# linto-ai/whisper-timestamped

Hardware: NVIDIA B200
Metric: audio-sec/s (RTF) large-v3 1h synthetic @1/2/4/8 B200; DTW GB/s vs HBM peak (higher is better)
Workload: dtype bf16x3 tensor-core GEMMs (float32-accurate), f32 elsewhere, f64 DTW accumulate

## Files before the change

include/wts.h:

```cpp
#ifndef WTS_H
#define WTS_H

#include <stdint.h>

#ifdef __cplusplus
extern "C" {
#endif

#define WTS_VERSION 102
#define WTS_SEG_NONPOSITIVE 1
#define WTS_SEG_PITCH16 2

typedef struct WtsSegDesc {
    int32_t window;
    int32_t row0;
    int32_t last_row;
    int32_t T;
    int32_t f0;
    int32_t F;
    int32_t max_dur;
    int32_t flags;
    int64_t cost_off;
    int64_t jumps_off;
    int64_t dir_off;
    int64_t bnd_off;
} WtsSegDesc;

int         wts_version(void);
const char* wts_last_error(void);

int64_t wts_dtw_dir_words(int32_t T, int32_t F);
int64_t wts_dtw_bnd_doubles(int32_t T, int32_t F);

int wts_attn_prep_batch(const float* d_qk, int32_t N, int32_t Tmax, int32_t Fmax,
                        const WtsSegDesc* d_segs, int32_t nseg, int32_t max_T, int32_t max_F,
                        float* d_cost, void* stream);

int wts_dtw_batch(const void* d_cost, int32_t cost_is_f64,
                  const WtsSegDesc* d_segs, int32_t nseg,
                  uint32_t* d_dir_ws, double* d_bnd_ws,
                  int32_t* d_jumps, int32_t* d_path, const int64_t* d_path_off,
                  int32_t* d_path_len, int32_t* d_status, void* stream);

int wts_dtw_batch_sized(const void* d_cost, int32_t cost_is_f64,
                  const WtsSegDesc* d_segs, int32_t nseg,
                  uint32_t* d_dir_ws, double* d_bnd_ws,
                  int32_t* d_jumps, int32_t* d_path, const int64_t* d_path_off,
                  int32_t* d_path_len, int32_t* d_status, int32_t max_T, int32_t max_F, int32_t all_flags,
                  void* stream);

int wts_disfluency_starts(const float* d_cost, const WtsSegDesc* d_segs, int32_t nseg, const int32_t* d_jumps,
                          int32_t* d_out, void* stream);



typedef struct WtsGemm {
    const void* a;  int64_t lda, a_plane, a_bo, a_bi;
    const void* b;  int64_t ldb, b_plane, b_bo, b_bi;
    int32_t M, N, K, batch_outer, batch_inner;
    float alpha;
    const float* bias;
    int32_t bias_on_m;
    int32_t act;
    const float* residual; int64_t ldr, r_bo, r_bi;
    float* out_f32;   int64_t ldc, c_bo, c_bi;
    void*  out_sb16;  int64_t ldo, o_plane, o_bo, o_bi;
    int32_t head_dim; int64_t head_stride;
    int32_t backend;
    int32_t a_is_f32, b_is_f32;
    const int32_t* row_mask;
} WtsGemm;

int wts_gemm(const WtsGemm* g, void* stream);

int wts_to_sb16(const float* d_x, int64_t n, void* d_hi, void* d_lo, void* stream);

int wts_layernorm(const float* d_x, int64_t ldx, const float* d_gamma, const float* d_beta, int32_t M,
                  int32_t D, void* d_out_sb16, int64_t ldo, int64_t o_plane, float* d_out_f32, int64_t ldf,
                  void* stream);

int wts_softmax_rows(const float* d_s, int64_t lds, int64_t rows, int32_t n, void* d_out_sb16, int64_t ldo,
                     int64_t o_plane, void* stream);

int wts_enc_attention(const void* d_qk, int64_t ld_qk, int64_t qk_plane, const void* d_vt, int64_t ld_vt,
                      int64_t vt_plane, int32_t B, int32_t H, int32_t D, int32_t n_ctx, void* d_out, int64_t ldo,
                      int64_t o_plane, void* stream);

int wts_frames(const float* d_audio, int64_t n_samples, int64_t n_total, int64_t n_frames, void* d_out,
               int64_t o_plane, void* stream);
int wts_power(const float* d_y, int64_t ldy, int64_t n_frames, void* d_out, int64_t ldo, int64_t o_plane,
              void* stream);
int wts_logmel_max(const float* d_m, int64_t n, float* d_max, void* stream);
int wts_logmel_finish(const float* d_m, int64_t n_frames, int32_t n_mels, const float* d_max, float* d_out_f32,
                      void* stream);

int wts_window_gather(const int64_t* d_mel_ptr, int32_t n_mels, const int32_t* d_seek, const int32_t* d_size,
                      int32_t B, void* d_out, int64_t o_plane, void* stream);

int wts_embed(const int32_t* d_tokens, const int32_t* d_positions, const float* d_emb, const float* d_pos,
              int32_t rows, int32_t D, float* d_out, void* stream);

int wts_gather_rows(const float* d_x, int64_t ldx, const int32_t* d_idx, int32_t rows, int32_t D, float* d_out,
                    void* stream);

int wts_decoder_attention(int32_t kind, const float* d_q, int64_t ldq, const float* d_k, const float* d_v,
                          int64_t seq_stride, int32_t ctx, const int32_t* d_row_seq, const int32_t* d_row_pos,
                          int32_t rows, int32_t H, void* d_out_sb16, int64_t ldo, int64_t o_plane,
                          float* d_qk_out, const int32_t* d_head_slot, int32_t n_slots, int32_t qk_rows,
                          const int32_t* d_qk_row, const int32_t* d_row_active, void* stream);

int wts_cross_kv_pack(const float* d_src, void* d_dst16, float* d_dst_align, const int32_t* d_head_slot,
                      int32_t n_slots, int32_t B, int32_t H, int32_t ctx, void* stream);
int wts_cross_attention_f16(const float* d_q, int64_t ldq, const void* d_k16, const void* d_v16,
                            const float* d_k_align, const int32_t* d_head_slot, int32_t n_slots, int32_t ctx,
                            const int32_t* d_row_seq, int32_t rows, int32_t H, void* d_out_sb16, int64_t ldo,
                            int64_t o_plane, float* d_qk_out, int32_t qk_rows, const int32_t* d_qk_row,
                            const int32_t* d_row_active, void* stream);

int wts_kv_append(const float* d_k, const float* d_v, int64_t ld, const int32_t* d_row_seq,
                  const int32_t* d_row_pos, int32_t rows, int32_t H, int32_t ctx, float* d_kc, float* d_vc,
                  int64_t seq_stride, void* stream);

typedef struct WtsDecodeCfg {
    int32_t n_vocab, eot, timestamp_begin, no_timestamps, max_initial_ts;
    int32_t sample_len, n_ctx, tokens_ld;
} WtsDecodeCfg;
int wts_decode_select(float* d_logits, int64_t ldl, const WtsDecodeCfg* cfg, const uint8_t* d_suppress,
                      const uint8_t* d_blank, int32_t* d_tokens, int32_t* d_n_tokens, const int32_t* d_n_prompt,
                      int32_t* d_done, float* d_logprobs, int32_t lp_ld, float* d_full_logprobs,
                      float* d_last_full, int32_t B, void* stream);

int wts_filtered_logprobs(const float* d_logits, int64_t ldl, const WtsDecodeCfg* cfg, const uint8_t* d_suppress,
                          const uint8_t* d_blank, int32_t* d_tokens, int32_t* d_n_tokens, const int32_t* d_n_prompt,
                          float* d_out, int32_t B, void* stream);

typedef struct WtsDecLayer {
    const float *ln1_g, *ln1_b, *w_qkv, *b_qkv, *w_o, *b_o;
    const float *ln2_g, *ln2_b, *w_cq, *b_cq, *w_co, *b_co;
    const float *ln3_g, *ln3_b, *w_fc1, *b_fc1, *w_fc2, *b_fc2;
    float *self_k, *self_v;
    const void *cross_k16, *cross_v16;
    const float* cross_k_align;
    const int32_t* head_slot;
    const void *sb_qkv, *sb_o, *sb_cq, *sb_co, *sb_fc1, *sb_fc2;
    int64_t pl_qkv, pl_o, pl_cq, pl_co, pl_fc1, pl_fc2;
} WtsDecLayer;

typedef struct WtsDecodeSteps {
    const WtsDecLayer* layers;
    const float *emb, *pos, *ln_g, *ln_b;
    int32_t *tokens, *n_tokens;
    const int32_t* n_prompt;
    int32_t* done;
    float *logprobs, *full, *last_full, *qk_buf;
    const uint8_t *suppress, *blank;
    float *x, *qkv, *att, *q, *mid, *logits;
    uint32_t* sync;
    uint64_t* prof;
    const void* emb_sb;
    int64_t emb_plane;
    int64_t use_mma;
    WtsDecodeCfg cfg;
    int32_t n_layer, D, H, n_ctx, n_audio_ctx, n_slots, cap, lp_ld, qk_rows, n_steps, max_rows, prof_cap;
} WtsDecodeSteps;

int wts_decode_steps(const WtsDecodeSteps* p, void* stream);

int wts_decode_step_kernels(const WtsDecodeSteps* p, const WtsDecLayer* h_layers, void* stream);

int wts_step_inputs(const int32_t* d_tokens, int32_t tokens_ld, const int32_t* d_n_tokens, const int32_t* d_n_prompt,
                    const int32_t* d_done, int32_t B, int32_t* d_tok, int32_t* d_pos, int32_t* d_qk_row,
                    int32_t* d_active, void* stream);

int wts_softmax_pick(const float* d_logits, int64_t ldl, int32_t n, int32_t index, float* d_out, int32_t rows,
                     void* stream);

int wts_logprob_gather(const float* d_logits, int64_t ldl, int32_t n, const int32_t* d_rows, const int32_t* d_tokens,
                       float* d_out, int32_t count, void* stream);

#ifdef __cplusplus
}
#endif
#endif
```

whisper-timestamped_b200/csrc/gemm.cu:

```cuda
#include <cuda_bf16.h>

#include "common.cuh"

namespace wts {

int gemm_tc_launch(const WtsGemm& g, cudaStream_t st);

__device__ __forceinline__ float ld_operand(const void* p, int64_t idx, int64_t plane, bool is_f32)
{
    if (is_f32) return reinterpret_cast<const float*>(p)[idx];
    const __nv_bfloat16* q = reinterpret_cast<const __nv_bfloat16*>(p);
    return __bfloat162float(q[idx]) + __bfloat162float(q[idx + plane]);
}

__device__ __forceinline__ float gelu_erf(float v) { return 0.5f * v * (1.0f + erff(v * 0.70710678118654752440f)); }

__device__ __forceinline__ void gemm_epilogue_store(const WtsGemm& g, int zo, int zi, int m, int n, float acc)
{
    float v = g.alpha * acc;
    if (g.bias) v += g.bias[g.bias_on_m ? m : n];
    if (g.act == 1) v = gelu_erf(v);
    if (g.residual) v += g.residual[(int64_t)zo * g.r_bo + (int64_t)zi * g.r_bi + (int64_t)m * g.ldr + n];
    if (g.out_f32) {
        const int64_t off = g.head_dim > 0 ? (int64_t)(n / g.head_dim) * g.head_stride + (int64_t)m * g.ldc + (n % g.head_dim)
                                           : (int64_t)m * g.ldc + n;
        g.out_f32[(int64_t)zo * g.c_bo + (int64_t)zi * g.c_bi + off] = v;
    }
    if (g.out_sb16) {
        const int64_t off = g.head_dim > 0 ? (int64_t)(n / g.head_dim) * g.head_stride + (int64_t)m * g.ldo + (n % g.head_dim)
                                           : (int64_t)m * g.ldo + n;
        __nv_bfloat16* o = reinterpret_cast<__nv_bfloat16*>(g.out_sb16) + (int64_t)zo * g.o_bo + (int64_t)zi * g.o_bi + off;
        const __nv_bfloat16 hi = __float2bfloat16_rn(v);
        o[0] = hi;
        o[g.o_plane] = __float2bfloat16_rn(v - __bfloat162float(hi));
    }
}

constexpr int ST = 64, SK = 16;
__global__ void __launch_bounds__(256)
gemm_simt_kernel(const WtsGemm g)
{
    __shared__ float As[SK][ST + 4];
    __shared__ float Bs[SK][ST + 4];
    const int z = blockIdx.z, zo = z / g.batch_inner, zi = z % g.batch_inner;
    const int m0 = blockIdx.y * ST, n0 = blockIdx.x * ST;
    const int tx = threadIdx.x & 15, ty = threadIdx.x >> 4;
    const int64_t abase = (int64_t)zo * g.a_bo + (int64_t)zi * g.a_bi;
    const int64_t bbase = (int64_t)zo * g.b_bo + (int64_t)zi * g.b_bi;
    float acc[4][4] = {};
    for (int k0 = 0; k0 < g.K; k0 += SK) {
#pragma unroll
        for (int i = 0; i < 4; ++i) {
            const int e = threadIdx.x + i * 256;
            const int r = e >> 4, kk = e & 15;
            const int m = m0 + r, n = n0 + r, k = k0 + kk;
            As[kk][r] = (m < g.M && k < g.K) ? ld_operand(g.a, abase + (int64_t)m * g.lda + k, g.a_plane, g.a_is_f32) : 0.f;
            Bs[kk][r] = (n < g.N && k < g.K) ? ld_operand(g.b, bbase + (int64_t)n * g.ldb + k, g.b_plane, g.b_is_f32) : 0.f;
        }
        __syncthreads();
#pragma unroll
        for (int kk = 0; kk < SK; ++kk) {
            float a[4], b[4];
#pragma unroll
            for (int i = 0; i < 4; ++i) { a[i] = As[kk][ty * 4 + i]; b[i] = Bs[kk][tx * 4 + i]; }
#pragma unroll
            for (int i = 0; i < 4; ++i)
#pragma unroll
                for (int j = 0; j < 4; ++j) acc[i][j] = fmaf(a[i], b[j], acc[i][j]);
        }
        __syncthreads();
    }
#pragma unroll
    for (int i = 0; i < 4; ++i)
#pragma unroll
        for (int j = 0; j < 4; ++j) {
            const int m = m0 + ty * 4 + i, n = n0 + tx * 4 + j;
            if (m < g.M && n < g.N) gemm_epilogue_store(g, zo, zi, m, n, acc[i][j]);
        }
}

}

using namespace wts;

extern "C" int wts_gemm(const WtsGemm* gp, void* stream)
{
    if (!gp) { set_error("wts_gemm: null descriptor"); return -2; }
    const WtsGemm g = *gp;
    if (g.M <= 0 || g.N <= 0 || g.batch_outer <= 0 || g.batch_inner <= 0) return 0;
    if (!g.a || !g.b || (!g.out_f32 && !g.out_sb16)) { set_error("wts_gemm: null operand/output"); return -2; }
    cudaStream_t st = (cudaStream_t)stream;
    if (g.backend == 0 && !g.a_is_f32 && !g.b_is_f32) return gemm_tc_launch(g, st);
    dim3 grid((g.N + ST - 1) / ST, (g.M + ST - 1) / ST, g.batch_outer * g.batch_inner);
    gemm_simt_kernel<<<grid, 256, 0, st>>>(g);
    WTS_LAUNCH_CHECK();
    return 0;
}
```

whisper-timestamped_b200/csrc/gemm_tc.cu:

```cuda
#include <cuda.h>
#include <cuda_bf16.h>
#include <cudaTypedefs.h>

#include <mutex>
#include <stdlib.h>

#include "common.cuh"

namespace wts {

constexpr int BM = 128, BK = 64;
constexpr int TILE_BYTES = BM * BK * 2;
constexpr int TC_THREADS = 192;
template <int BN> struct TcCfg {
    static constexpr int STAGES = 3;
    static constexpr int B_TILE = BN * BK * 2;
    static constexpr int STAGE_BYTES = 2 * TILE_BYTES + 2 * B_TILE;
    static constexpr int SMEM = STAGES * STAGE_BYTES + 256 + 1024;
    static constexpr int TMEM_COLS = BN < 32 ? 32 : BN;
};

__device__ __forceinline__ uint32_t smem_addr(const void* p) { return (uint32_t)__cvta_generic_to_shared(p); }

__device__ __forceinline__ void mbar_init(uint32_t bar, uint32_t count)
{
    asm volatile("mbarrier.init.shared::cta.b64 [%0], %1;" ::"r"(bar), "r"(count));
}
__device__ __forceinline__ void mbar_expect_tx(uint32_t bar, uint32_t bytes)
{
    asm volatile("mbarrier.arrive.expect_tx.shared::cta.b64 _, [%0], %1;" ::"r"(bar), "r"(bytes) : "memory");
}
__device__ __forceinline__ void mbar_wait(uint32_t bar, uint32_t parity)
{
    asm volatile(
        "{\n\t"
        ".reg .pred p;\n\t"
        "WAIT_LOOP:\n\t"
        "mbarrier.try_wait.parity.shared::cta.b64 p, [%0], %1;\n\t"
        "@p bra DONE;\n\t"
        "bra WAIT_LOOP;\n\t"
        "DONE:\n\t"
        "}\n" ::"r"(bar), "r"(parity) : "memory");
}
__device__ __forceinline__ void tma_load_5d(uint32_t dst, const CUtensorMap* tm, uint32_t bar, int c0, int c1, int c2,
                                            int c3, int c4)
{
    asm volatile(
        "cp.async.bulk.tensor.5d.shared::cluster.global.mbarrier::complete_tx::bytes [%0], [%1, {%3, %4, %5, %6, %7}], [%2];"
        ::"r"(dst), "l"(tm), "r"(bar), "r"(c0), "r"(c1), "r"(c2), "r"(c3), "r"(c4) : "memory");
}
__device__ __forceinline__ void umma_bf16(uint32_t tmem_c, uint64_t adesc, uint64_t bdesc, uint32_t idesc, uint32_t accumulate)
{
    asm volatile(
        "{\n\t"
        ".reg .pred p;\n\t"
        "setp.ne.b32 p, %4, 0;\n\t"
        "tcgen05.mma.cta_group::1.kind::f16 [%0], %1, %2, %3, p;\n\t"
        "}\n" ::"r"(tmem_c), "l"(adesc), "l"(bdesc), "r"(idesc), "r"(accumulate) : "memory");
}
__device__ __forceinline__ void umma_commit(uint32_t bar)
{
    asm volatile("tcgen05.commit.cta_group::1.mbarrier::arrive::one.shared::cluster.b64 [%0];" ::"r"(bar) : "memory");
}
__device__ __forceinline__ void tc_fence_before() { asm volatile("tcgen05.fence::before_thread_sync;" ::: "memory"); }
__device__ __forceinline__ void tc_fence_after() { asm volatile("tcgen05.fence::after_thread_sync;" ::: "memory"); }

__device__ __forceinline__ void tmem_ld32(uint32_t taddr, uint32_t (&v)[32])
{
    asm volatile(
        "tcgen05.ld.sync.aligned.32x32b.x32.b32 "
        "{%0, %1, %2, %3, %4, %5, %6, %7, %8, %9, %10, %11, %12, %13, %14, %15, "
        "%16, %17, %18, %19, %20, %21, %22, %23, %24, %25, %26, %27, %28, %29, %30, %31}, [%32];"
        : "=r"(v[0]), "=r"(v[1]), "=r"(v[2]), "=r"(v[3]), "=r"(v[4]), "=r"(v[5]), "=r"(v[6]), "=r"(v[7]), "=r"(v[8]),
          "=r"(v[9]), "=r"(v[10]), "=r"(v[11]), "=r"(v[12]), "=r"(v[13]), "=r"(v[14]), "=r"(v[15]), "=r"(v[16]),
          "=r"(v[17]), "=r"(v[18]), "=r"(v[19]), "=r"(v[20]), "=r"(v[21]), "=r"(v[22]), "=r"(v[23]), "=r"(v[24]),
          "=r"(v[25]), "=r"(v[26]), "=r"(v[27]), "=r"(v[28]), "=r"(v[29]), "=r"(v[30]), "=r"(v[31])
        : "r"(taddr) : "memory");
    asm volatile("tcgen05.wait::ld.sync.aligned;" ::: "memory");
}

__device__ __forceinline__ uint64_t umma_desc(uint32_t saddr)
{
    uint64_t d = 0;
    d |= (uint64_t)((saddr >> 4) & 0x3FFF);
    d |= (uint64_t)1 << 16;
    d |= (uint64_t)(1024 >> 4) << 32;
    d |= (uint64_t)1 << 46;
    d |= (uint64_t)2 << 61;
    return d;
}

__device__ __forceinline__ float gelu_erf_tc(float v) { return 0.5f * v * (1.0f + erff(v * 0.70710678118654752440f)); }

struct TcArgs {
    WtsGemm g;
    int a_has_bo, a_has_bi, b_has_bo, b_has_bi;
    int debug;
};

__device__ __forceinline__ void epilogue_chunk(const WtsGemm& g, float (&y)[32], int m, int nb, float bias_m, const float* res,
                                               float* of, __nv_bfloat16* ob)
{
#pragma unroll
    for (int j = 0; j < 32; ++j) {
        const int n = nb + j;
        float t = y[j];
        if (g.bias) t += g.bias_on_m ? bias_m : (n < g.N ? g.bias[n] : 0.f);
        if (g.act == 1) t = gelu_erf_tc(t);
        if (res && n < g.N) t += res[n];
        y[j] = t;
    }
    const bool full = nb + 32 <= g.N;
    if (of) {
        const int64_t off = g.head_dim > 0 ? (int64_t)(nb / g.head_dim) * g.head_stride + (int64_t)m * g.ldc + (nb % g.head_dim)
                                           : (int64_t)m * g.ldc + nb;
        float* dst = of + off;
        if (full && ((reinterpret_cast<uintptr_t>(dst) & 15) == 0)) {
#pragma unroll
            for (int j = 0; j < 32; j += 4) *reinterpret_cast<float4*>(dst + j) = make_float4(y[j], y[j + 1], y[j + 2], y[j + 3]);
        } else {
#pragma unroll
            for (int j = 0; j < 32; ++j) if (nb + j < g.N) dst[j] = y[j];
        }
    }
    if (ob) {
        const int64_t off = g.head_dim > 0 ? (int64_t)(nb / g.head_dim) * g.head_stride + (int64_t)m * g.ldo + (nb % g.head_dim)
                                           : (int64_t)m * g.ldo + nb;
        __nv_bfloat16* dh = ob + off;
        __nv_bfloat16* dl = dh + g.o_plane;
        __align__(16) __nv_bfloat16 hi[32];
        __align__(16) __nv_bfloat16 lo[32];
#pragma unroll
        for (int j = 0; j < 32; ++j) {
            hi[j] = __float2bfloat16_rn(y[j]);
            lo[j] = __float2bfloat16_rn(y[j] - __bfloat162float(hi[j]));
        }
        if (full && ((reinterpret_cast<uintptr_t>(dh) & 15) == 0) && ((reinterpret_cast<uintptr_t>(dl) & 15) == 0)) {
#pragma unroll
            for (int j = 0; j < 4; ++j) {
                reinterpret_cast<uint4*>(dh)[j] = reinterpret_cast<const uint4*>(hi)[j];
                reinterpret_cast<uint4*>(dl)[j] = reinterpret_cast<const uint4*>(lo)[j];
            }
        } else {
#pragma unroll
            for (int j = 0; j < 32; ++j) if (nb + j < g.N) { dh[j] = hi[j]; dl[j] = lo[j]; }
        }
    }
}

template <int BN>
__global__ void __launch_bounds__(TC_THREADS, 1)
gemm_tc_kernel(const __grid_constant__ CUtensorMap tmA, const __grid_constant__ CUtensorMap tmB, const TcArgs args)
{
    using Cfg = TcCfg<BN>;
    constexpr int STAGES = Cfg::STAGES, STAGE_BYTES = Cfg::STAGE_BYTES, B_TILE = Cfg::B_TILE, TMEM_COLS = Cfg::TMEM_COLS;
    extern __shared__ unsigned char smem_raw[];
    const WtsGemm& g = args.g;
    const uint32_t base = (smem_addr(smem_raw) + 1023u) & ~1023u;
    const uint32_t bar_base = base + STAGES * STAGE_BYTES;
    const int warp = threadIdx.x >> 5, lane = threadIdx.x & 31;
    const int m0 = blockIdx.y * BM, n0 = blockIdx.x * BN;
    const int z = blockIdx.z, zo = z / g.batch_inner, zi = z - zo * g.batch_inner;
    const int nkb = (g.K + BK - 1) / BK;
    constexpr int kb0 = 0;

    if (warp == 0 && lane == 0) {
        asm volatile("prefetch.tensormap [%0];" ::"l"(&tmA) : "memory");
        asm volatile("prefetch.tensormap [%0];" ::"l"(&tmB) : "memory");
    }
    if (warp == 1) {
        if (lane == 0) {
            for (int s = 0; s < STAGES; ++s) { mbar_init(bar_base + 8 * s, 1); mbar_init(bar_base + 64 + 8 * s, 1); }
            mbar_init(bar_base + 128, 1);
            asm volatile("fence.mbarrier_init.release.cluster;" ::: "memory");
        }
        __syncwarp();
        asm volatile("tcgen05.alloc.cta_group::1.sync.aligned.shared::cta.b32 [%0], %1;" ::"r"(bar_base + 136), "r"(TMEM_COLS) : "memory");
        asm volatile("tcgen05.relinquish_alloc_permit.cta_group::1.sync.aligned;" ::: "memory");
    }
    tc_fence_before();
    __syncthreads();
    tc_fence_after();
    uint32_t tmem_base;
    asm volatile("ld.shared.u32 %0, [%1];" : "=r"(tmem_base) : "r"(bar_base + 136));

    if (warp == 0) {
        if (lane == 0) {
            const int azo = args.a_has_bo ? zo : 0, azi = args.a_has_bi ? zi : 0;
            const int bzo = args.b_has_bo ? zo : 0, bzi = args.b_has_bi ? zi : 0;
            for (int kb = 0; kb < (args.debug == 2 ? 0 : nkb); ++kb) {
                const int s = kb % STAGES, u = kb / STAGES;
                mbar_wait(bar_base + 64 + 8 * s, (u & 1) ^ 1);
                const uint32_t full = bar_base + 8 * s;
                mbar_expect_tx(full, STAGE_BYTES);
                const uint32_t st = base + s * STAGE_BYTES;
                const int kc = (kb0 + kb) * BK;
                tma_load_5d(st, &tmA, full, kc, m0, azi, azo, 0);
                tma_load_5d(st + TILE_BYTES, &tmA, full, kc, m0, azi, azo, 1);
                tma_load_5d(st + 2 * TILE_BYTES, &tmB, full, kc, n0, bzi, bzo, 0);
                tma_load_5d(st + 2 * TILE_BYTES + B_TILE, &tmB, full, kc, n0, bzi, bzo, 1);
            }
        }
    } else if (warp == 1) {
        if (lane == 0) {
            const uint32_t idesc = (1u << 4) | (1u << 7) | (1u << 10) | ((uint32_t)(BN >> 3) << 17) | ((uint32_t)(BM >> 4) << 24);
            for (int kb = 0; kb < nkb; ++kb) {
                const int s = kb % STAGES, u = kb / STAGES;
                if (args.debug != 2) mbar_wait(bar_base + 8 * s, u & 1);
                tc_fence_after();
                if (args.debug == 1) {
                    asm volatile("mbarrier.arrive.shared::cta.b64 _, [%0];" ::"r"(bar_base + 64 + 8 * s) : "memory");
                    continue;
                }
                const uint32_t st = base + s * STAGE_BYTES;
                const uint64_t a_hi = umma_desc(st), a_lo = umma_desc(st + TILE_BYTES);
                const uint64_t b_hi = umma_desc(st + 2 * TILE_BYTES), b_lo = umma_desc(st + 2 * TILE_BYTES + B_TILE);
#pragma unroll
                for (int k = 0; k < BK / 16; ++k) {
                    const uint64_t adv = (uint64_t)(k * 2);
                    umma_bf16(tmem_base, a_hi + adv, b_hi + adv, idesc, (kb | k) ? 1u : 0u);
                    if (args.debug == 3) continue;
                    umma_bf16(tmem_base, a_lo + adv, b_hi + adv, idesc, 1u);
                    umma_bf16(tmem_base, a_hi + adv, b_lo + adv, idesc, 1u);
                }
                umma_commit(bar_base + 64 + 8 * s);
            }
            umma_commit(bar_base + 128);
        }
    } else {
        const int q = warp & 3;
        const int m = m0 + 32 * q + lane;
        mbar_wait(bar_base + 128, 0);
        tc_fence_after();
        const bool row_ok = m < g.M;
        const float* res = g.residual ? g.residual + (int64_t)zo * g.r_bo + (int64_t)zi * g.r_bi + (int64_t)m * g.ldr : nullptr;
        float* of = g.out_f32 ? g.out_f32 + (int64_t)zo * g.c_bo + (int64_t)zi * g.c_bi : nullptr;
        __nv_bfloat16* ob = g.out_sb16 ? reinterpret_cast<__nv_bfloat16*>(g.out_sb16) + (int64_t)zo * g.o_bo + (int64_t)zi * g.o_bi : nullptr;
        const float bias_m = (g.bias && g.bias_on_m && row_ok) ? g.bias[m] : 0.f;
#pragma unroll 1
        for (int c = 0; c < BN / 32; ++c) {
            uint32_t v[32];
            tmem_ld32(tmem_base + ((uint32_t)(32 * q) << 16) + (uint32_t)(32 * c), v);
            const int nb = n0 + 32 * c;
            if (!row_ok || nb >= g.N) continue;
            float y[32];
#pragma unroll
            for (int j = 0; j < 32; ++j) y[j] = g.alpha * __uint_as_float(v[j]);
            epilogue_chunk(g, y, m, nb, bias_m, res, of, ob);
        }
    }
    tc_fence_before();
    __syncthreads();
    if (warp == 1) {
        tc_fence_after();
        asm volatile("tcgen05.dealloc.cta_group::1.sync.aligned.b32 %0, %1;" ::"r"(tmem_base), "r"(TMEM_COLS) : "memory");
    }
}

constexpr int P_THREADS = 320;
constexpr int P_STAGES = 3;
constexpr int P_STAGE_BYTES = 4 * TILE_BYTES;
constexpr int P_SMEM = P_STAGES * P_STAGE_BYTES + 256 + 1024;

__global__ void __launch_bounds__(P_THREADS, 1)
gemm_tc_persist_kernel(const __grid_constant__ CUtensorMap tmA, const __grid_constant__ CUtensorMap tmB, const TcArgs args)
{
    extern __shared__ unsigned char smem_raw[];
    const WtsGemm& g = args.g;
    const uint32_t base = (smem_addr(smem_raw) + 1023u) & ~1023u;
    const uint32_t bar_base = base + P_STAGES * P_STAGE_BYTES;
    const int warp = threadIdx.x >> 5, lane = threadIdx.x & 31;
    const int tiles_n = (g.N + BM - 1) / BM, tiles_m = (g.M + BM - 1) / BM;
    const int n_tiles = tiles_n * tiles_m * g.batch_outer * g.batch_inner;
    const int nkb = (g.K + BK - 1) / BK;

    if (warp == 0 && lane == 0) {
        asm volatile("prefetch.tensormap [%0];" ::"l"(&tmA) : "memory");
        asm volatile("prefetch.tensormap [%0];" ::"l"(&tmB) : "memory");
    }
    if (warp == 1) {
        if (lane == 0) {
            for (int s = 0; s < P_STAGES; ++s) { mbar_init(bar_base + 8 * s, 1); mbar_init(bar_base + 32 + 8 * s, 1); }
            for (int b = 0; b < 2; ++b) { mbar_init(bar_base + 64 + 8 * b, 1); mbar_init(bar_base + 80 + 8 * b, 256); }
            asm volatile("fence.mbarrier_init.release.cluster;" ::: "memory");
        }
        __syncwarp();
        asm volatile("tcgen05.alloc.cta_group::1.sync.aligned.shared::cta.b32 [%0], %1;" ::"r"(bar_base + 96), "r"(256) : "memory");
        asm volatile("tcgen05.relinquish_alloc_permit.cta_group::1.sync.aligned;" ::: "memory");
    }
    tc_fence_before();
    __syncthreads();
    tc_fence_after();
    uint32_t tmem_base;
    asm volatile("ld.shared.u32 %0, [%1];" : "=r"(tmem_base) : "r"(bar_base + 96));

    if (warp == 0) {
        if (lane == 0) {
            int it = 0;
            for (int t = blockIdx.x; t < n_tiles; t += gridDim.x) {
                const int nt = t % tiles_n, mt = (t / tiles_n) % tiles_m, z = t / (tiles_n * tiles_m);
                const int zo = z / g.batch_inner, zi = z - zo * g.batch_inner;
                const int azo = args.a_has_bo ? zo : 0, azi = args.a_has_bi ? zi : 0;
                const int bzo = args.b_has_bo ? zo : 0, bzi = args.b_has_bi ? zi : 0;
                const int m0 = mt * BM, n0 = nt * BM;
                for (int kb = 0; kb < nkb; ++kb, ++it) {
                    const int s = it % P_STAGES, u = it / P_STAGES;
                    mbar_wait(bar_base + 32 + 8 * s, (u & 1) ^ 1);
                    const uint32_t full = bar_base + 8 * s;
                    mbar_expect_tx(full, P_STAGE_BYTES);
                    const uint32_t st = base + s * P_STAGE_BYTES;
                    const int kc = kb * BK;
                    tma_load_5d(st, &tmA, full, kc, m0, azi, azo, 0);
                    tma_load_5d(st + TILE_BYTES, &tmA, full, kc, m0, azi, azo, 1);
                    tma_load_5d(st + 2 * TILE_BYTES, &tmB, full, kc, n0, bzi, bzo, 0);
                    tma_load_5d(st + 3 * TILE_BYTES, &tmB, full, kc, n0, bzi, bzo, 1);
                }
            }
        }
    } else if (warp == 1) {
        if (lane == 0) {
            const uint32_t idesc = (1u << 4) | (1u << 7) | (1u << 10) | ((uint32_t)(BM >> 3) << 17) | ((uint32_t)(BM >> 4) << 24);
            int it = 0, lt = 0;
            for (int t = blockIdx.x; t < n_tiles; t += gridDim.x, ++lt) {
                const int buf = lt & 1, ut = lt >> 1;
                mbar_wait(bar_base + 80 + 8 * buf, (ut & 1) ^ 1);
                tc_fence_after();
                const uint32_t acc = tmem_base + (uint32_t)(buf * BM);
                for (int kb = 0; kb < nkb; ++kb, ++it) {
                    const int s = it % P_STAGES, u = it / P_STAGES;
                    mbar_wait(bar_base + 8 * s, u & 1);
                    tc_fence_after();
                    const uint32_t st = base + s * P_STAGE_BYTES;
                    const uint64_t a_hi = umma_desc(st), a_lo = umma_desc(st + TILE_BYTES);
                    const uint64_t b_hi = umma_desc(st + 2 * TILE_BYTES), b_lo = umma_desc(st + 3 * TILE_BYTES);
#pragma unroll
                    for (int k = 0; k < BK / 16; ++k) {
                        const uint64_t adv = (uint64_t)(k * 2);
                        umma_bf16(acc, a_hi + adv, b_hi + adv, idesc, (kb | k) ? 1u : 0u);
                        umma_bf16(acc, a_lo + adv, b_hi + adv, idesc, 1u);
                        umma_bf16(acc, a_hi + adv, b_lo + adv, idesc, 1u);
                    }
                    umma_commit(bar_base + 32 + 8 * s);
                }
                umma_commit(bar_base + 64 + 8 * buf);
            }
        }
    } else {
        const int q = warp & 3, half = (warp - 2) >> 2;
        int lt = 0;
        for (int t = blockIdx.x; t < n_tiles; t += gridDim.x, ++lt) {
            const int nt = t % tiles_n, mt = (t / tiles_n) % tiles_m, z = t / (tiles_n * tiles_m);
            const int zo = z / g.batch_inner, zi = z - zo * g.batch_inner;
            const int m0 = mt * BM, n0 = nt * BM;
            const int buf = lt & 1, ut = lt >> 1;
            const int m = m0 + 32 * q + lane;
            const bool row_ok = m < g.M;
            const float* res = g.residual ? g.residual + (int64_t)zo * g.r_bo + (int64_t)zi * g.r_bi + (int64_t)m * g.ldr : nullptr;
            float* of = g.out_f32 ? g.out_f32 + (int64_t)zo * g.c_bo + (int64_t)zi * g.c_bi : nullptr;
            __nv_bfloat16* ob = g.out_sb16 ? reinterpret_cast<__nv_bfloat16*>(g.out_sb16) + (int64_t)zo * g.o_bo + (int64_t)zi * g.o_bi : nullptr;
            const float bias_m = (g.bias && g.bias_on_m && row_ok) ? g.bias[m] : 0.f;
            mbar_wait(bar_base + 64 + 8 * buf, ut & 1);
            tc_fence_after();
            uint32_t v0[32], v1[32];
            const uint32_t taddr = tmem_base + ((uint32_t)(32 * q) << 16) + (uint32_t)(buf * BM + 64 * half);
            tmem_ld32(taddr, v0);
            tmem_ld32(taddr + 32, v1);
            tc_fence_before();
            asm volatile("mbarrier.arrive.shared::cta.b64 _, [%0];" ::"r"(bar_base + 80 + 8 * buf) : "memory");
            if (!row_ok) continue;
            float y[32];
            int nb = n0 + 64 * half;
            if (nb < g.N) {
#pragma unroll
                for (int j = 0; j < 32; ++j) y[j] = g.alpha * __uint_as_float(v0[j]);
                epilogue_chunk(g, y, m, nb, bias_m, res, of, ob);
            }
            nb += 32;
            if (nb < g.N) {
#pragma unroll
                for (int j = 0; j < 32; ++j) y[j] = g.alpha * __uint_as_float(v1[j]);
                epilogue_chunk(g, y, m, nb, bias_m, res, of, ob);
            }
        }
    }
    tc_fence_before();
    __syncthreads();
    if (warp == 1) {
        tc_fence_after();
        asm volatile("tcgen05.dealloc.cta_group::1.sync.aligned.b32 %0, %1;" ::"r"(tmem_base), "r"(256) : "memory");
    }
}

struct SkArgs {
    WtsGemm g;
    int split_k;
    int bn;
    int stages, stage_bytes;
    int debug;
};

constexpr int SK_SMEM = 3 * 65536 + 256 + 1024 + 1024;

__device__ __forceinline__ void sk_finish(const WtsGemm& g, float t, float resid, int m, int n, float bias_n, float* of,
                                          __nv_bfloat16* ob)
{
    if (g.bias) t += g.bias_on_m ? g.bias[m] : bias_n;
    if (g.act == 1) t = gelu_erf_tc(t);
    t += resid;
    if (of) of[(int64_t)m * g.ldc + n] = t;
    if (ob) {
        const __nv_bfloat16 hi = __float2bfloat16_rn(t);
        ob[(int64_t)m * g.ldo + n] = hi;
        ob[(int64_t)m * g.ldo + n + g.o_plane] = __float2bfloat16_rn(t - __bfloat162float(hi));
    }
}

__device__ __forceinline__ void cluster_sync_all()
{
    asm volatile("barrier.cluster.arrive.release.aligned;" ::: "memory");
    asm volatile("barrier.cluster.wait.acquire.aligned;" ::: "memory");
}

template <int SMAX, int RB>
__device__ __forceinline__ void sk_reduce_rows(const WtsGemm& g, const uint32_t (&peer)[8], int S, const int* list, int rank,
                                               int n_rows, int n, float bias_n, float* of, __nv_bfloat16* ob)
{
#pragma unroll 1
    for (int kb = rank; kb < n_rows; kb += RB * S) {
        float x[RB][SMAX], r[RB];
        int mm[RB];
#pragma unroll
        for (int i = 0; i < RB; ++i) {
            const int k = kb + i * S;
            const bool ok = k < n_rows;
            const int m = ok ? list[k] : 0;
            mm[i] = ok ? m : -1;
            r[i] = (ok && g.residual) ? g.residual[(int64_t)m * g.ldr + n] : 0.f;
#pragma unroll
            for (int s = 0; s < SMAX; ++s) {
                x[i][s] = 0.f;
                if (s < S && ok)
                    asm volatile("ld.shared::cluster.f32 %0, [%1];" : "=f"(x[i][s]) : "r"(peer[s] + (uint32_t)(m * BM * 4)));
            }
        }
#pragma unroll
        for (int i = 0; i < RB; ++i) {
            if (mm[i] >= 0) {
                float t = 0.f;
#pragma unroll
                for (int s = 0; s < SMAX; ++s) t += x[i][s];
                sk_finish(g, t, r[i], mm[i], n, bias_n, of, ob);
            }
        }
    }
}

__global__ void __launch_bounds__(TC_THREADS, 1)
gemm_skinny_kernel(const __grid_constant__ CUtensorMap tmW, const __grid_constant__ CUtensorMap tmX, const SkArgs args)
{
    extern __shared__ unsigned char smem_raw[];
    const WtsGemm& g = args.g;
    const uint32_t base = (smem_addr(smem_raw) + 1023u) & ~1023u;
    const uint32_t bar_base = base + 3 * 65536;
    const int warp = threadIdx.x >> 5, lane = threadIdx.x & 31;
    const int n0 = blockIdx.x * BM;
    const int S = args.split_k;
    const int nkb_all = (g.K + BK - 1) / BK;
    const int kb0 = (int)((int64_t)blockIdx.y * nkb_all / S);
    const int kb1 = (int)((int64_t)(blockIdx.y + 1) * nkb_all / S);
    const int nkb = args.debug == 4 ? 0 : kb1 - kb0;
    const int STAGES = args.stages, STAGE_BYTES = args.stage_bytes;
    const int X_TILE = args.bn * BK * 2;
    pdl_launch();
    if (args.debug == 5) { pdl_wait(); return; }

    if (warp == 0 && lane == 0) {
        asm volatile("prefetch.tensormap [%0];" ::"l"(&tmW) : "memory");
        asm volatile("prefetch.tensormap [%0];" ::"l"(&tmX) : "memory");
    }
    if (warp == 1) {
        if (lane == 0) {
            for (int s = 0; s < STAGES; ++s) { mbar_init(bar_base + 8 * s, 1); mbar_init(bar_base + 64 + 8 * s, 1); }
            mbar_init(bar_base + 128, 1);
            asm volatile("fence.mbarrier_init.release.cluster;" ::: "memory");
        }
        __syncwarp();
        asm volatile("tcgen05.alloc.cta_group::1.sync.aligned.shared::cta.b32 [%0], %1;" ::"r"(bar_base + 136), "r"(128) : "memory");
        asm volatile("tcgen05.relinquish_alloc_permit.cta_group::1.sync.aligned;" ::: "memory");
    }
    tc_fence_before();
    __syncthreads();
    tc_fence_after();
    uint32_t tmem_base;
    asm volatile("ld.shared.u32 %0, [%1];" : "=r"(tmem_base) : "r"(bar_base + 136));
    pdl_wait();

    int* rows_list = reinterpret_cast<int*>(smem_raw + (bar_base - smem_addr(smem_raw)) + 256);
    if (warp >= 2) {
        const int t = threadIdx.x - 64;
        const bool act = t < g.M && (g.row_mask == nullptr || g.row_mask[t] != 0);
        const unsigned bal = __ballot_sync(0xffffffffu, act);
        int* wcount = rows_list + 132;
        if (lane == 0) wcount[warp - 2] = __popc(bal);
        asm volatile("bar.sync 1, 128;" ::: "memory");
        int off = 0;
        for (int w2 = 0; w2 < warp - 2; ++w2) off += wcount[w2];
        if (act) rows_list[off + __popc(bal & ((1u << lane) - 1u))] = t;
        if (t == 0) rows_list[128] = wcount[0] + wcount[1] + wcount[2] + wcount[3];
        asm volatile("bar.sync 1, 128;" ::: "memory");
    }

    const int q = warp & 3;
    const int nl = 32 * q + lane;
    const int n = n0 + nl;
    const bool n_ok = n < g.N;
    float* of = g.out_f32;
    __nv_bfloat16* ob = reinterpret_cast<__nv_bfloat16*>(g.out_sb16);

    if (warp == 0) {
        if (lane == 0) {
            for (int kb = 0; kb < (args.debug == 2 ? 0 : nkb); ++kb) {
                const int s = kb % STAGES, u = kb / STAGES;
                mbar_wait(bar_base + 64 + 8 * s, (u & 1) ^ 1);
                const uint32_t full = bar_base + 8 * s;
                mbar_expect_tx(full, STAGE_BYTES);
                const uint32_t st = base + s * STAGE_BYTES;
                const int kc = (kb0 + kb) * BK;
                tma_load_5d(st, &tmW, full, kc, n0, 0, 0, 0);
                tma_load_5d(st + TILE_BYTES, &tmW, full, kc, n0, 0, 0, 1);
                tma_load_5d(st + 2 * TILE_BYTES, &tmX, full, kc, 0, 0, 0, 0);
                tma_load_5d(st + 2 * TILE_BYTES + X_TILE, &tmX, full, kc, 0, 0, 0, 1);
            }
        }
    } else if (warp == 1) {
        if (lane == 0) {
            const uint32_t idesc = (1u << 4) | (1u << 7) | (1u << 10) | ((uint32_t)(args.bn >> 3) << 17) | ((uint32_t)(BM >> 4) << 24);
            for (int kb = 0; kb < nkb; ++kb) {
                const int s = kb % STAGES, u = kb / STAGES;
                if (args.debug != 2) mbar_wait(bar_base + 8 * s, u & 1);
                tc_fence_after();
                if (args.debug == 1) {
                    asm volatile("mbarrier.arrive.shared::cta.b64 _, [%0];" ::"r"(bar_base + 64 + 8 * s) : "memory");
                    continue;
                }
                const uint32_t st = base + s * STAGE_BYTES;
                const uint64_t w_hi = umma_desc(st), w_lo = umma_desc(st + TILE_BYTES);
                const uint64_t x_hi = umma_desc(st + 2 * TILE_BYTES), x_lo = umma_desc(st + 2 * TILE_BYTES + X_TILE);
#pragma unroll
                for (int k = 0; k < BK / 16; ++k) {
                    const uint64_t adv = (uint64_t)(k * 2);
                    umma_bf16(tmem_base, w_hi + adv, x_hi + adv, idesc, (kb | k) ? 1u : 0u);
                    umma_bf16(tmem_base, w_lo + adv, x_hi + adv, idesc, 1u);
                    umma_bf16(tmem_base, w_hi + adv, x_lo + adv, idesc, 1u);
                }
                umma_commit(bar_base + 64 + 8 * s);
            }
            umma_commit(bar_base + 128);
        }
    } else {
        const int nchunk = (g.M + 31) / 32;
        const float bias_n = (g.bias && !g.bias_on_m && n_ok) ? g.bias[n] : 0.f;
        mbar_wait(bar_base + 128, 0);
        tc_fence_after();
        float* part = reinterpret_cast<float*>(smem_raw + (base - smem_addr(smem_raw)));
#pragma unroll 1
        for (int c = 0; c < nchunk; ++c) {
            uint32_t v[32];
            tmem_ld32(tmem_base + ((uint32_t)(32 * q) << 16) + (uint32_t)(32 * c), v);
            if (S == 1) {
                if (!n_ok) continue;
                float r[32];
#pragma unroll
                for (int j = 0; j < 32; ++j) {
                    const int m = 32 * c + j;
                    r[j] = (g.residual && m < g.M) ? g.residual[(int64_t)m * g.ldr + n] : 0.f;
                }
#pragma unroll
                for (int j = 0; j < 32; ++j) {
                    const int m = 32 * c + j;
                    if (m < g.M && (g.row_mask == nullptr || g.row_mask[m] != 0))
                        sk_finish(g, g.alpha * __uint_as_float(v[j]), r[j], m, n, bias_n, of, ob);
                }
            } else {
#pragma unroll
                for (int j = 0; j < 32; ++j) {
                    const int m = 32 * c + j;
                    if (m < g.M) part[m * BM + nl] = g.alpha * __uint_as_float(v[j]);
                }
            }
        }
    }
    if (S > 1) {
        __syncwarp();
        cluster_sync_all();
        if (warp >= 2 && n_ok) {
            uint32_t rank;
            asm volatile("mov.u32 %0, %%cluster_ctarank;" : "=r"(rank));
            const int n_rows = rows_list[128];
            const float bias_n = (g.bias && !g.bias_on_m) ? g.bias[n] : 0.f;
            uint32_t peer[8];
#pragma unroll
            for (int s = 0; s < 8; ++s) {
                peer[s] = 0;
                if (s < S) asm volatile("mapa.shared::cluster.u32 %0, %1, %2;" : "=r"(peer[s]) : "r"(base + 4u * nl), "r"(s));
            }
            if (S <= 4) sk_reduce_rows<4, 12>(g, peer, S, rows_list, (int)rank, n_rows, n, bias_n, of, ob);
            else        sk_reduce_rows<8, 6>(g, peer, S, rows_list, (int)rank, n_rows, n, bias_n, of, ob);
        }
        __syncwarp();
        cluster_sync_all();
    }
    tc_fence_before();
    __syncthreads();
    if (warp == 1) {
        tc_fence_after();
        asm volatile("tcgen05.dealloc.cta_group::1.sync.aligned.b32 %0, %1;" ::"r"(tmem_base), "r"(128) : "memory");
    }
}

static PFN_cuTensorMapEncodeTiled_v12000 get_encode()
{
    static PFN_cuTensorMapEncodeTiled_v12000 fn = nullptr;
    static std::once_flag once;
    std::call_once(once, [] {
        void* p = nullptr;
        cudaDriverEntryPointQueryResult qres;
        if (cudaGetDriverEntryPoint("cuTensorMapEncodeTiled", &p, cudaEnableDefault, &qres) == cudaSuccess &&
            qres == cudaDriverEntryPointSuccess)
            fn = reinterpret_cast<PFN_cuTensorMapEncodeTiled_v12000>(p);
    });
    return fn;
}

static int make_map(CUtensorMap* tm, const void* ptr, int64_t K, int64_t rows, int64_t ld, int64_t plane, int64_t n_bi,
                    int64_t s_bi, int64_t n_bo, int64_t s_bo, int box_rows, const char* which)
{
    auto enc = get_encode();
    if (!enc) { set_error("wts_gemm: cuTensorMapEncodeTiled entry point not available"); return -4; }
    if ((reinterpret_cast<uintptr_t>(ptr) & 15) || (ld & 7) || (plane & 7) || (s_bi & 7) || (s_bo & 7)) {
        set_error("wts_gemm(tc): operand %s not 16-byte aligned (ptr=%p ld=%lld plane=%lld bi=%lld bo=%lld)", which, ptr,
                  (long long)ld, (long long)plane, (long long)s_bi, (long long)s_bo);
        return -5;
    }
    const int64_t e_bi = s_bi ? n_bi : 1, e_bo = s_bo ? n_bo : 1;
    cuuint64_t dims[5] = {(cuuint64_t)K, (cuuint64_t)rows, (cuuint64_t)e_bi, (cuuint64_t)e_bo, 2};
    const cuuint64_t row_b = (cuuint64_t)ld * 2;
    cuuint64_t strides[4] = {row_b, (cuuint64_t)(s_bi ? s_bi * 2 : row_b), (cuuint64_t)(s_bo ? s_bo * 2 : row_b),
                             (cuuint64_t)plane * 2};
    cuuint32_t box[5] = {BK, (cuuint32_t)box_rows, 1, 1, 1};
    cuuint32_t estr[5] = {1, 1, 1, 1, 1};
    CUresult r = enc(tm, CU_TENSOR_MAP_DATA_TYPE_BFLOAT16, 5, const_cast<void*>(ptr), dims, strides, box, estr,
                     CU_TENSOR_MAP_INTERLEAVE_NONE, CU_TENSOR_MAP_SWIZZLE_128B, CU_TENSOR_MAP_L2_PROMOTION_L2_256B,
                     CU_TENSOR_MAP_FLOAT_OOB_FILL_NONE);
    if (r != CUDA_SUCCESS) {
        set_error("wts_gemm(tc): cuTensorMapEncodeTiled(%s) failed with %d (K=%lld rows=%lld ld=%lld plane=%lld)", which, (int)r,
                  (long long)K, (long long)rows, (long long)ld, (long long)plane);
        return -6;
    }
    return 0;
}

static int launch_big(const WtsGemm& g, cudaStream_t st)
{
    constexpr int BN = 128;
    static bool attr_set = false;
    if (!attr_set) {
        WTS_CUDA_CHECK(cudaFuncSetAttribute(gemm_tc_kernel<BN>, cudaFuncAttributeMaxDynamicSharedMemorySize, TcCfg<BN>::SMEM));
        attr_set = true;
    }
    alignas(64) CUtensorMap tmA, tmB;
    int rc = make_map(&tmA, g.a, g.K, g.M, g.lda, g.a_plane, g.batch_inner, g.a_bi, g.batch_outer, g.a_bo, BM, "A");
    if (rc) return rc;
    rc = make_map(&tmB, g.b, g.K, g.N, g.ldb, g.b_plane, g.batch_inner, g.b_bi, g.batch_outer, g.b_bo, BN, "B");
    if (rc) return rc;
    TcArgs args;
    args.g = g;
    args.a_has_bo = g.a_bo != 0; args.a_has_bi = g.a_bi != 0;
    args.b_has_bo = g.b_bo != 0; args.b_has_bi = g.b_bi != 0;
    { const char* e = getenv("WTS_GEMM_DEBUG"); args.debug = e ? atoi(e) : 0; }
    static const int persist = []{ const char* e = getenv("WTS_GEMM_PERSIST"); return e ? atoi(e) : 1; }();
    const int64_t n_tiles = (int64_t)((g.N + BN - 1) / BN) * ((g.M + BM - 1) / BM) * g.batch_outer * g.batch_inner;
    if (persist && args.debug == 0 && n_tiles > 1) {
        static bool pattr = false;
        static int n_sm = 148;
        if (!pattr) {
            WTS_CUDA_CHECK(cudaFuncSetAttribute(gemm_tc_persist_kernel, cudaFuncAttributeMaxDynamicSharedMemorySize, P_SMEM));
            int dev = 0;
            WTS_CUDA_CHECK(cudaGetDevice(&dev));
            WTS_CUDA_CHECK(cudaDeviceGetAttribute(&n_sm, cudaDevAttrMultiProcessorCount, dev));
            pattr = true;
        }
        const int64_t rounds = (n_tiles + n_sm - 1) / n_sm;
        const int ctas = (int)((n_tiles + rounds - 1) / rounds);
        gemm_tc_persist_kernel<<<ctas, P_THREADS, P_SMEM, st>>>(tmA, tmB, args);
        WTS_LAUNCH_CHECK();
        return 0;
    }
    dim3 grid((g.N + BN - 1) / BN, (g.M + BM - 1) / BM, g.batch_outer * g.batch_inner);
    gemm_tc_kernel<BN><<<grid, TC_THREADS, TcCfg<BN>::SMEM, st>>>(tmA, tmB, args);
    WTS_LAUNCH_CHECK();
    return 0;
}

static int launch_skinny(const WtsGemm& g, cudaStream_t st, int split_k)
{
    static bool attr_set = false;
    if (!attr_set) {
        WTS_CUDA_CHECK(cudaFuncSetAttribute(gemm_skinny_kernel, cudaFuncAttributeMaxDynamicSharedMemorySize, SK_SMEM));
        attr_set = true;
    }
    SkArgs args;
    args.g = g;
    args.bn = ((g.M + 15) / 16) * 16;
    args.stage_bytes = 2 * TILE_BYTES + 2 * args.bn * BK * 2;
    args.stages = (3 * 65536) / args.stage_bytes;
    if (args.stages > 8) args.stages = 8;
    args.split_k = split_k;
    { const char* e = getenv("WTS_GEMM_DEBUG"); args.debug = e ? atoi(e) : 0; }
    alignas(64) CUtensorMap tmW, tmX;
    int rc = make_map(&tmW, g.b, g.K, g.N, g.ldb, g.b_plane, 1, 0, 1, 0, BM, "B(weights)");
    if (rc) return rc;
    rc = make_map(&tmX, g.a, g.K, g.M, g.lda, g.a_plane, 1, 0, 1, 0, args.bn, "A(rows)");
    if (rc) return rc;
    cudaLaunchConfig_t cfg = {};
    cfg.gridDim = dim3((g.N + BM - 1) / BM, split_k, 1);
    cfg.blockDim = dim3(TC_THREADS, 1, 1);
    cfg.dynamicSmemBytes = SK_SMEM;
    cfg.stream = st;
    cudaLaunchAttribute attr[2];
    attr[0].id = cudaLaunchAttributeClusterDimension;
    attr[0].val.clusterDim.x = 1;
    attr[0].val.clusterDim.y = split_k;
    attr[0].val.clusterDim.z = 1;
    attr[1].id = cudaLaunchAttributeProgrammaticStreamSerialization;
    attr[1].val.programmaticStreamSerializationAllowed = 1;
    cfg.attrs = attr;
    cfg.numAttrs = pdl_enabled() ? 2 : 1;
    WTS_CUDA_CHECK(cudaLaunchKernelEx(&cfg, gemm_skinny_kernel, tmW, tmX, args));
    return 0;
}

int gemm_tc_launch(const WtsGemm& g, cudaStream_t st)
{
    static const int skinny = []{ const char* e = getenv("WTS_SKINNY_GEMM"); return e ? atoi(e) : 1; }();
    static const int splitk = []{ const char* e = getenv("WTS_SPLITK"); return e ? atoi(e) : 1; }();
    if (skinny && g.M <= BM && g.batch_outer * g.batch_inner == 1 && g.head_dim == 0) {
        const int tiles = (g.N + BM - 1) / BM, nkb = (g.K + BK - 1) / BK;
        int split = 1;
        if (splitk && tiles <= 74) {
            split = 148 / tiles;
            if (split > 8) split = 8;
            if (split > nkb) split = nkb;
            if (split < 1) split = 1;
        }
        return launch_skinny(g, st, split);
    }
    return launch_big(g, st);
}

}
```

whisper-timestamped_b200/csrc/ops.cu:

```cuda
#include "decode_common.cuh"

namespace wts {

__global__ void to_sb16_kernel(const float* __restrict__ x, int64_t n, __nv_bfloat16* __restrict__ hi,
                               __nv_bfloat16* __restrict__ lo)
{
    for (int64_t i = blockIdx.x * (int64_t)blockDim.x + threadIdx.x; i < n; i += (int64_t)gridDim.x * blockDim.x) {
        __nv_bfloat16 h, l;
        split_bf16(x[i], h, l);
        hi[i] = h;
        lo[i] = l;
    }
}

constexpr int LN_THREADS = 128, LN_MAXV = 16;
__global__ void __launch_bounds__(LN_THREADS)
layernorm_kernel(const float* x, int64_t ldx, const float* gamma,
                 const float* beta, int M, int D, __nv_bfloat16* o, int64_t ldo,
                 int64_t o_plane, float* of, int64_t ldf)
{
    pdl_launch();
    pdl_wait();
    __shared__ float red[32];
    const int row = blockIdx.x;
    const float* xr = x + (int64_t)row * ldx;
    float v[LN_MAXV];
    float s = 0.f;
#pragma unroll
    for (int k = 0; k < LN_MAXV; ++k) {
        const int c = threadIdx.x + LN_THREADS * k;
        v[k] = c < D ? xr[c] : 0.f;
        s += v[k];
    }
    const float mean = block_reduce_sum(s, red) / (float)D;
    float q = 0.f;
#pragma unroll
    for (int k = 0; k < LN_MAXV; ++k) {
        const int c = threadIdx.x + LN_THREADS * k;
        const float d = c < D ? v[k] - mean : 0.f;
        q += d * d;
    }
    const float rstd = 1.0f / sqrtf(block_reduce_sum(q, red) / (float)D + 1e-5f);
#pragma unroll
    for (int k = 0; k < LN_MAXV; ++k) {
        const int c = threadIdx.x + LN_THREADS * k;
        if (c < D) {
            const float y = (v[k] - mean) * rstd * gamma[c] + beta[c];
            if (o) {
                __nv_bfloat16 h, l;
                split_bf16(y, h, l);
                o[(int64_t)row * ldo + c] = h;
                o[(int64_t)row * ldo + c + o_plane] = l;
            }
            if (of) of[(int64_t)row * ldf + c] = y;
        }
    }
}

__global__ void __launch_bounds__(128)
softmax_rows_kernel(const float* __restrict__ s, int64_t lds, int64_t rows, int n,
                    __nv_bfloat16* __restrict__ o, int64_t ldo, int64_t o_plane)
{
    const int64_t row = (int64_t)blockIdx.x * 4 + (threadIdx.x >> 5);
    const int lane = threadIdx.x & 31;
    if (row >= rows) return;
    const float* sr = s + row * lds;
    float v[64];
    float mx = -CUDART_INF_F;
#pragma unroll
    for (int k = 0; k < 64; ++k) {
        const int c = lane + 32 * k;
        v[k] = c < n ? sr[c] : -CUDART_INF_F;
        mx = fmaxf(mx, v[k]);
    }
    mx = warp_max(mx);
    float sum = 0.f;
#pragma unroll
    for (int k = 0; k < 64; ++k) {
        v[k] = expf(v[k] - mx);
        sum += v[k];
    }
    sum = warp_sum(sum);
    const float inv = 1.0f / sum;
#pragma unroll
    for (int k = 0; k < 64; ++k) {
        const int c = lane + 32 * k;
        if (c < n) {
            __nv_bfloat16 h, l;
            split_bf16(v[k] * inv, h, l);
            o[row * ldo + c] = h;
            o[row * ldo + c + o_plane] = l;
        }
    }
}

__global__ void frames_kernel(const float* __restrict__ audio, int64_t n_samples, int64_t n_total,
                              int64_t n_frames, float* __restrict__ out)
{
    const int64_t t = blockIdx.x;
    if (t >= n_frames) return;
    for (int n = threadIdx.x; n < 400; n += blockDim.x) {
        int64_t i = t * 160 - 200 + n;
        if (i < 0) i = -i;
        if (i >= n_total) i = 2 * (n_total - 1) - i;
        const float x = (i >= 0 && i < n_samples) ? audio[i] : 0.f;
        const float w = 0.5f - 0.5f * cospif((float)n / 200.0f);
        out[t * 400 + n] = x * w;
    }
}

__global__ void power_kernel(const float* __restrict__ y, int64_t ldy, int64_t n_frames, float* __restrict__ p,
                             int64_t ldp)
{
    const int64_t i = blockIdx.x * (int64_t)blockDim.x + threadIdx.x;
    if (i >= n_frames * 208) return;
    const int64_t t = i / 208;
    const int k = (int)(i - t * 208);
    const float re = y[t * ldy + k], im = y[t * ldy + 208 + k];
    p[t * ldp + k] = re * re + im * im;
}

__device__ __forceinline__ float mel_log10(float m) { return log10f(fmaxf(m, 1e-10f)); }

__global__ void logmel_max_kernel(const float* __restrict__ m, int64_t n, float* __restrict__ out)
{
    __shared__ float red[32];
    float mx = -CUDART_INF_F;
    for (int64_t i = blockIdx.x * (int64_t)blockDim.x + threadIdx.x; i < n; i += (int64_t)gridDim.x * blockDim.x)
        mx = fmaxf(mx, mel_log10(m[i]));
    mx = block_reduce_max(mx, red);
    if (threadIdx.x == 0) {
        int key = __float_as_int(mx);
        key = key >= 0 ? key : key ^ 0x7fffffff;
        atomicMax(reinterpret_cast<int*>(out), key);
    }
}

__global__ void logmel_finish_kernel(const float* __restrict__ m, int64_t n, const float* __restrict__ mxkey,
                                     float* __restrict__ out)
{
    int key = *reinterpret_cast<const int*>(mxkey);
    key = key >= 0 ? key : key ^ 0x7fffffff;
    const float gmax = __int_as_float(key);
    for (int64_t i = blockIdx.x * (int64_t)blockDim.x + threadIdx.x; i < n; i += (int64_t)gridDim.x * blockDim.x) {
        float x = mel_log10(m[i]);
        x = fmaxf(x, gmax - 8.0f);
        out[i] = (x + 4.0f) / 4.0f;
    }
}

__global__ void window_gather_kernel(const int64_t* __restrict__ mel_ptr, int n_mels,
                                     const int32_t* __restrict__ seek, const int32_t* __restrict__ size, int B,
                                     __nv_bfloat16* __restrict__ out, int64_t o_plane)
{
    const int b = blockIdx.y;
    const float* mel = reinterpret_cast<const float*>(mel_ptr[b]);
    const int64_t i = blockIdx.x * (int64_t)blockDim.x + threadIdx.x;
    const int64_t per = (int64_t)3002 * n_mels;
    if (i >= per) return;
    const int r = (int)(i / n_mels), c = (int)(i - (int64_t)r * n_mels);
    float v = 0.f;
    const int t = r - 1;
    if (t >= 0 && t < size[b]) v = mel[((int64_t)seek[b] + t) * n_mels + c];
    __nv_bfloat16 h, l;
    split_bf16(v, h, l);
    out[b * per + i] = h;
    out[b * per + i + o_plane] = l;
}

__global__ void embed_kernel(const int32_t* tokens, const int32_t* positions,
                             const float* emb, const float* pos, int rows, int D,
                             float* out)
{
    pdl_launch();
    pdl_wait();
    const int r = blockIdx.x;
    if (r >= rows) return;
    const float* e = emb + (int64_t)tokens[r] * D;
    const float* p = pos + (int64_t)positions[r] * D;
    for (int c = threadIdx.x; c < D; c += blockDim.x) out[(int64_t)r * D + c] = e[c] + p[c];
}

__global__ void gather_rows_kernel(const float* __restrict__ x, int64_t ldx, const int32_t* __restrict__ idx,
                                   int rows, int D, float* __restrict__ out)
{
    const int r = blockIdx.x;
    if (r >= rows) return;
    const float* s = x + (int64_t)idx[r] * ldx;
    for (int c = threadIdx.x; c < D; c += blockDim.x) out[(int64_t)r * D + c] = s[c];
}

constexpr int DA_THREADS = 128;
__global__ void __launch_bounds__(DA_THREADS)
decoder_attention_kernel(const int kind, const float* q, int64_t ldq, const float* kc,
                         const float* vc, int64_t seq_stride, int ctx,
                         const int32_t* row_seq, const int32_t* row_pos, int H,
                         __nv_bfloat16* o, int64_t ldo, int64_t o_plane, float* qk_out,
                         const int32_t* head_slot, int n_slots, int qk_rows,
                         const int32_t* qk_row, const int32_t* row_active)
{
    pdl_launch();
    pdl_wait();
    extern __shared__ float sm[];
    float* sc = sm;
    float* qs = sm + ctx;
    float* red = qs + 64;
    float* part = red + 32;
    const int r = blockIdx.x, h = blockIdx.y;
    if (row_active != nullptr && !row_active[r]) return;
    const int seq = row_seq[r];
    const int nk = kind == 1 ? ctx : row_pos[r] + 1;
    const float* K = kc + (int64_t)seq * seq_stride + (int64_t)h * ctx * 64;
    const float* V = vc + (int64_t)seq * seq_stride + (int64_t)h * ctx * 64;
    if (kind == 2) {
        const float* src = q + (int64_t)r * ldq + h * 64;
        const int64_t at = (int64_t)(nk - 1) * 64 + (threadIdx.x & 63);
        if (threadIdx.x < 64) const_cast<float*>(K)[at] = src[(int64_t)H * 64 + threadIdx.x];
        else                  const_cast<float*>(V)[at] = src[(int64_t)2 * H * 64 + (threadIdx.x & 63)];
    }
    if (threadIdx.x < 64) qs[threadIdx.x] = q[(int64_t)r * ldq + h * 64 + threadIdx.x];
    __syncthreads();
    float mx = -CUDART_INF_F;
    for (int j = threadIdx.x; j < nk; j += DA_THREADS) {
        const float4* kr = reinterpret_cast<const float4*>(K + (int64_t)j * 64);
        float acc = 0.f;
#pragma unroll
        for (int c = 0; c < 16; ++c) {
            const float4 kv = kr[c];
            acc += qs[4 * c] * kv.x + qs[4 * c + 1] * kv.y + qs[4 * c + 2] * kv.z + qs[4 * c + 3] * kv.w;
        }
        sc[j] = acc;
        mx = fmaxf(mx, acc);
    }
    __syncthreads();
    if (kind == 1 && qk_out != nullptr) {
        const int slot = head_slot[h];
        const int qr = qk_row[r];
        if (slot >= 0 && qr >= 0) {
            float* dst = qk_out + (((int64_t)seq * n_slots + slot) * qk_rows + qr) * (int64_t)ctx;
            for (int j = threadIdx.x; j < nk; j += DA_THREADS) dst[j] = sc[j];
        }
    }
    mx = block_reduce_max(mx, red);
    float sum = 0.f;
    for (int j = threadIdx.x; j < nk; j += DA_THREADS) {
        const float e = expf(sc[j] - mx);
        sc[j] = e;
        sum += e;
    }
    sum = block_reduce_sum(sum, red);
    const float inv = 1.0f / sum;
    const int c = threadIdx.x & 63, g = threadIdx.x >> 6;
    float acc = 0.f;
    for (int j = g; j < nk; j += 2) acc += sc[j] * V[(int64_t)j * 64 + c];
    part[g * 64 + c] = acc;
    __syncthreads();
    if (threadIdx.x < 64) {
        const float y = (part[threadIdx.x] + part[64 + threadIdx.x]) * inv;
        __nv_bfloat16 hi, lo;
        split_bf16(y, hi, lo);
        o[(int64_t)r * ldo + h * 64 + threadIdx.x] = hi;
        o[(int64_t)r * ldo + h * 64 + threadIdx.x + o_plane] = lo;
    }
}


__global__ void cross_kv_pack_kernel(const float* __restrict__ src, __half* __restrict__ dst16,
                                     float* __restrict__ dst_align, const int32_t* __restrict__ head_slot,
                                     int n_slots, int H, int ctx)
{
    const int bh = blockIdx.x;
    const int b = bh / H, h = bh - b * H;
    const float* s = src + (int64_t)bh * ctx * 64;
    __half* d = dst16 + (int64_t)bh * ctx * 64;
    const int slot = dst_align ? head_slot[h] : -1;
    float* da = slot >= 0 ? dst_align + ((int64_t)b * n_slots + slot) * ctx * 64 : nullptr;
    for (int i = threadIdx.x; i < ctx * 64; i += blockDim.x) {
        const float v = s[i];
        d[i] = __float2half_rn(v);
        if (da) da[i] = v;
    }
}

__global__ void __launch_bounds__(CA_THREADS)
cross_attention_f16_kernel(const float* q, int64_t ldq, const __half* k16,
                           const __half* v16, const float* k_align,
                           const int32_t* head_slot, int n_slots, int ctx,
                           const int32_t* row_seq, int H, __nv_bfloat16* o, int64_t ldo,
                           int64_t o_plane, float* qk_out, int qk_rows, const int32_t* qk_row,
                           const int32_t* row_active)
{
    pdl_launch();
    pdl_wait();
    __shared__ CaScratch sc;
    const int r = blockIdx.x, h = blockIdx.y;
    if (row_active != nullptr && !row_active[r]) return;
    const int seq = row_seq[r];
    const int slot = head_slot[h];
    const int c8 = threadIdx.x & 7;
    float qf[8];
    {
        const float4* qp = reinterpret_cast<const float4*>(q + (int64_t)r * ldq + h * 64 + c8 * 8);
        const float4 a = qp[0], b = qp[1];
        qf[0] = a.x; qf[1] = a.y; qf[2] = a.z; qf[3] = a.w; qf[4] = b.x; qf[5] = b.y; qf[6] = b.z; qf[7] = b.w;
    }
    const __half* V = v16 + ((int64_t)seq * H + h) * ctx * 64;
    float* qk_dst = nullptr;
    const float* kal = nullptr;
    if (slot >= 0) {
        kal = k_align + ((int64_t)seq * n_slots + slot) * ctx * 64;
        if (qk_out != nullptr) {
            const int qr = qk_row[r];
            if (qr >= 0) qk_dst = qk_out + (((int64_t)seq * n_slots + slot) * qk_rows + qr) * (int64_t)ctx;
        }
    }
    const float y = ca_row_head<4>(qf, k16 + ((int64_t)seq * H + h) * ctx * 64, V, kal, qk_dst, ctx, sc);
    if (threadIdx.x < 64) {
        __nv_bfloat16 hi, lo;
        split_bf16(y, hi, lo);
        o[(int64_t)r * ldo + h * 64 + threadIdx.x] = hi;
        o[(int64_t)r * ldo + h * 64 + threadIdx.x + o_plane] = lo;
    }
}

__global__ void kv_append_kernel(const float* k, const float* v, int64_t ld,
                                 const int32_t* row_seq, const int32_t* row_pos, int H,
                                 int ctx, float* kc, float* vc, int64_t seq_stride)
{
    pdl_launch();
    pdl_wait();
    const int r = blockIdx.x;
    const int seq = row_seq[r], pos = row_pos[r];
    for (int c = threadIdx.x; c < H * 64; c += blockDim.x) {
        const int h = c >> 6, d = c & 63;
        const int64_t dst = (int64_t)seq * seq_stride + ((int64_t)h * ctx + pos) * 64 + d;
        kc[dst] = k[(int64_t)r * ld + c];
        vc[dst] = v[(int64_t)r * ld + c];
    }
}

constexpr int DS_THREADS = 1024;
__global__ void __launch_bounds__(DS_THREADS)
decode_select_kernel(float* logits, int64_t ldl, const WtsDecodeCfg cfg,
                     const uint8_t* suppress, const uint8_t* blank,
                     int32_t* tokens, int32_t* n_tokens,
                     const int32_t* n_prompt, int32_t* done,
                     float* logprobs, int lp_ld, float* full, float* last_full)
{
    pdl_launch();
    pdl_wait();
    __shared__ SelectScratch S;
    const int b = blockIdx.x;
    if (done[b]) return;
    select_row<false>(logits + (int64_t)b * ldl, cfg, suppress, blank, tokens + (int64_t)b * cfg.tokens_ld, n_tokens + b,
                      n_prompt[b], done + b, logprobs + (int64_t)b * lp_ld,
                      full != nullptr ? full + (int64_t)b * lp_ld * cfg.n_vocab : nullptr,
                      last_full != nullptr ? last_full + (int64_t)b * cfg.n_vocab : nullptr, S);
}

__global__ void __launch_bounds__(DS_THREADS)
filtered_logprobs_kernel(const float* logits, int64_t ldl, const WtsDecodeCfg cfg, const uint8_t* suppress, const uint8_t* blank,
                         int32_t* tokens, int32_t* n_tokens, const int32_t* n_prompt, float* out)
{
    __shared__ SelectScratch S;
    const int b = blockIdx.x;
    select_row<false>(logits + (int64_t)b * ldl, cfg, suppress, blank, tokens + (int64_t)b * cfg.tokens_ld, n_tokens + b,
                      n_prompt[b], nullptr, nullptr, out + (int64_t)b * cfg.n_vocab, nullptr, S, true);
}

__global__ void step_inputs_kernel(const int32_t* tokens, int ld, const int32_t* n_tokens,
                                   const int32_t* n_prompt, const int32_t* done, int B,
                                   int32_t* tok, int32_t* pos, int32_t* qk_row,
                                   int32_t* active)
{
    pdl_launch();
    pdl_wait();
    const int b = blockIdx.x * blockDim.x + threadIdx.x;
    if (b >= B) return;
    const int nt = n_tokens[b];
    tok[b] = tokens[(int64_t)b * ld + nt - 1];
    pos[b] = nt - 1;
    qk_row[b] = done[b] ? -1 : nt - n_prompt[b];
    if (active) active[b] = done[b] ? 0 : 1;
}

__global__ void softmax_pick_kernel(const float* __restrict__ logits, int64_t ldl, int n, int index,
                                    float* __restrict__ out)
{
    __shared__ float red[32];
    const float* x = logits + (int64_t)blockIdx.x * ldl;
    float mx = -CUDART_INF_F;
    for (int v = threadIdx.x; v < n; v += blockDim.x) mx = fmaxf(mx, x[v]);
    mx = block_reduce_max(mx, red);
    float s = 0.f;
    for (int v = threadIdx.x; v < n; v += blockDim.x) s += expf(x[v] - mx);
    s = block_reduce_sum(s, red);
    if (threadIdx.x == 0) out[blockIdx.x] = expf(x[index] - mx) / s;
}

__global__ void logprob_gather_kernel(const float* logits, int64_t ldl, int n, const int32_t* rows, const int32_t* tokens,
                                      float* out)
{
    __shared__ float red[32];
    const float* x = logits + (int64_t)rows[blockIdx.x] * ldl;
    float mx = -CUDART_INF_F;
    for (int v = threadIdx.x; v < n; v += blockDim.x) mx = fmaxf(mx, x[v]);
    mx = block_reduce_max(mx, red);
    float s = 0.f;
    for (int v = threadIdx.x; v < n; v += blockDim.x) s += expf(x[v] - mx);
    s = block_reduce_sum(s, red);
    if (threadIdx.x == 0) out[blockIdx.x] = (x[tokens[blockIdx.x]] - mx) - logf(s);
}

}

using namespace wts;

static inline int grid_for(int64_t n, int block, int cap = 148 * 16)
{
    int64_t g = (n + block - 1) / block;
    return (int)(g < 1 ? 1 : (g > cap ? cap : g));
}

extern "C" int wts_to_sb16(const float* d_x, int64_t n, void* d_hi, void* d_lo, void* stream)
{
    if (n <= 0) return 0;
    to_sb16_kernel<<<grid_for(n, 256), 256, 0, (cudaStream_t)stream>>>(d_x, n, (__nv_bfloat16*)d_hi, (__nv_bfloat16*)d_lo);
    WTS_LAUNCH_CHECK();
    return 0;
}

extern "C" int wts_layernorm(const float* d_x, int64_t ldx, const float* d_gamma, const float* d_beta, int32_t M,
                             int32_t D, void* d_out_sb16, int64_t ldo, int64_t o_plane, float* d_out_f32,
                             int64_t ldf, void* stream)
{
    if (M <= 0) return 0;
    if (D > LN_THREADS * LN_MAXV) { set_error("wts_layernorm: D=%d > %d", D, LN_THREADS * LN_MAXV); return -2; }
    WTS_CUDA_CHECK(launch_pdl(layernorm_kernel, dim3(M), dim3(LN_THREADS), 0, (cudaStream_t)stream, d_x, ldx, d_gamma, d_beta, M, D,
                                                                   (__nv_bfloat16*)d_out_sb16, ldo, o_plane, d_out_f32, ldf));
    WTS_LAUNCH_CHECK();
    return 0;
}

extern "C" int wts_softmax_rows(const float* d_s, int64_t lds, int64_t rows, int32_t n, void* d_out_sb16,
                                int64_t ldo, int64_t o_plane, void* stream)
{
    if (rows <= 0) return 0;
    if (n > 2048) { set_error("wts_softmax_rows: n=%d > 2048", n); return -2; }
    softmax_rows_kernel<<<(unsigned)((rows + 3) / 4), 128, 0, (cudaStream_t)stream>>>(d_s, lds, rows, n,
                                                                                     (__nv_bfloat16*)d_out_sb16, ldo, o_plane);
    WTS_LAUNCH_CHECK();
    return 0;
}

extern "C" int wts_frames(const float* d_audio, int64_t n_samples, int64_t n_total, int64_t n_frames, void* d_out,
                          int64_t o_plane, void* stream)
{
    (void)o_plane;
    if (n_frames <= 0) return 0;
    frames_kernel<<<(unsigned)n_frames, 128, 0, (cudaStream_t)stream>>>(d_audio, n_samples, n_total, n_frames, (float*)d_out);
    WTS_LAUNCH_CHECK();
    return 0;
}

extern "C" int wts_power(const float* d_y, int64_t ldy, int64_t n_frames, void* d_out, int64_t ldo, int64_t o_plane,
                         void* stream)
{
    (void)o_plane;
    if (n_frames <= 0) return 0;
    power_kernel<<<(unsigned)((n_frames * 208 + 255) / 256), 256, 0, (cudaStream_t)stream>>>(d_y, ldy, n_frames, (float*)d_out, ldo);
    WTS_LAUNCH_CHECK();
    return 0;
}

extern "C" int wts_logmel_max(const float* d_m, int64_t n, float* d_max, void* stream)
{
    logmel_max_kernel<<<grid_for(n, 256, 1024), 256, 0, (cudaStream_t)stream>>>(d_m, n, d_max);
    WTS_LAUNCH_CHECK();
    return 0;
}

extern "C" int wts_logmel_finish(const float* d_m, int64_t n_frames, int32_t n_mels, const float* d_max,
                                 float* d_out_f32, void* stream)
{
    const int64_t n = n_frames * n_mels;
    logmel_finish_kernel<<<grid_for(n, 256), 256, 0, (cudaStream_t)stream>>>(d_m, n, d_max, d_out_f32);
    WTS_LAUNCH_CHECK();
    return 0;
}

extern "C" int wts_window_gather(const int64_t* d_mel_ptr, int32_t n_mels, const int32_t* d_seek,
                                 const int32_t* d_size, int32_t B, void* d_out, int64_t o_plane, void* stream)
{
    if (B <= 0) return 0;
    dim3 grid((unsigned)(((int64_t)3002 * n_mels + 255) / 256), B);
    window_gather_kernel<<<grid, 256, 0, (cudaStream_t)stream>>>(d_mel_ptr, n_mels, d_seek, d_size, B,
                                                                 (__nv_bfloat16*)d_out, o_plane);
    WTS_LAUNCH_CHECK();
    return 0;
}

extern "C" int wts_embed(const int32_t* d_tokens, const int32_t* d_positions, const float* d_emb, const float* d_pos,
                         int32_t rows, int32_t D, float* d_out, void* stream)
{
    if (rows <= 0) return 0;
    WTS_CUDA_CHECK(launch_pdl(embed_kernel, dim3(rows), dim3(256), 0, (cudaStream_t)stream, d_tokens, d_positions, d_emb, d_pos, rows, D, d_out));
    WTS_LAUNCH_CHECK();
    return 0;
}

extern "C" int wts_gather_rows(const float* d_x, int64_t ldx, const int32_t* d_idx, int32_t rows, int32_t D,
                               float* d_out, void* stream)
{
    if (rows <= 0) return 0;
    gather_rows_kernel<<<rows, 256, 0, (cudaStream_t)stream>>>(d_x, ldx, d_idx, rows, D, d_out);
    WTS_LAUNCH_CHECK();
    return 0;
}

extern "C" int wts_decoder_attention(int32_t kind, const float* d_q, int64_t ldq, const float* d_k, const float* d_v,
                                     int64_t seq_stride, int32_t ctx, const int32_t* d_row_seq,
                                     const int32_t* d_row_pos, int32_t rows, int32_t H, void* d_out_sb16, int64_t ldo,
                                     int64_t o_plane, float* d_qk_out, const int32_t* d_head_slot, int32_t n_slots,
                                     int32_t qk_rows, const int32_t* d_qk_row, const int32_t* d_row_active, void* stream)
{
    if (rows <= 0) return 0;
    const size_t smem = ((size_t)ctx + 64 + 32 + 128) * sizeof(float);
    dim3 grid(rows, H);
    WTS_CUDA_CHECK(launch_pdl(decoder_attention_kernel, grid, dim3(DA_THREADS), smem, (cudaStream_t)stream, 
        kind, d_q, ldq, d_k, d_v, seq_stride, ctx, d_row_seq, d_row_pos, H, (__nv_bfloat16*)d_out_sb16, ldo, o_plane,
        d_qk_out, d_head_slot, n_slots, qk_rows, d_qk_row, d_row_active));
    WTS_LAUNCH_CHECK();
    return 0;
}


extern "C" int wts_cross_kv_pack(const float* d_src, void* d_dst16, float* d_dst_align, const int32_t* d_head_slot,
                                 int32_t n_slots, int32_t B, int32_t H, int32_t ctx, void* stream)
{
    if (B <= 0) return 0;
    cross_kv_pack_kernel<<<B * H, 256, 0, (cudaStream_t)stream>>>(d_src, (__half*)d_dst16, d_dst_align, d_head_slot,
                                                                 n_slots, H, ctx);
    WTS_LAUNCH_CHECK();
    return 0;
}

extern "C" int wts_cross_attention_f16(const float* d_q, int64_t ldq, const void* d_k16, const void* d_v16,
                                       const float* d_k_align, const int32_t* d_head_slot, int32_t n_slots,
                                       int32_t ctx, const int32_t* d_row_seq, int32_t rows, int32_t H,
                                       void* d_out_sb16, int64_t ldo, int64_t o_plane, float* d_qk_out,
                                       int32_t qk_rows, const int32_t* d_qk_row, const int32_t* d_row_active,
                                       void* stream)
{
    if (rows <= 0) return 0;
    if ((ldq & 3) || (reinterpret_cast<uintptr_t>(d_q) & 15)) { set_error("wts_cross_attention_f16: q must be 16-byte aligned"); return -2; }
    dim3 grid(rows, H);
    WTS_CUDA_CHECK(launch_pdl(cross_attention_f16_kernel, grid, dim3(CA_THREADS), 0, (cudaStream_t)stream, 
        d_q, ldq, (const __half*)d_k16, (const __half*)d_v16, d_k_align, d_head_slot, n_slots, ctx, d_row_seq, H,
        (__nv_bfloat16*)d_out_sb16, ldo, o_plane, d_qk_out, qk_rows, d_qk_row, d_row_active));
    WTS_LAUNCH_CHECK();
    return 0;
}

extern "C" int wts_kv_append(const float* d_k, const float* d_v, int64_t ld, const int32_t* d_row_seq,
                             const int32_t* d_row_pos, int32_t rows, int32_t H, int32_t ctx, float* d_kc, float* d_vc,
                             int64_t seq_stride, void* stream)
{
    if (rows <= 0) return 0;
    WTS_CUDA_CHECK(launch_pdl(kv_append_kernel, dim3(rows), dim3(256), 0, (cudaStream_t)stream, d_k, d_v, ld, d_row_seq, d_row_pos, H, ctx, d_kc, d_vc, seq_stride));
    WTS_LAUNCH_CHECK();
    return 0;
}

extern "C" int wts_decode_select(float* d_logits, int64_t ldl, const WtsDecodeCfg* cfg, const uint8_t* d_suppress,
                                 const uint8_t* d_blank, int32_t* d_tokens, int32_t* d_n_tokens,
                                 const int32_t* d_n_prompt, int32_t* d_done, float* d_logprobs, int32_t lp_ld,
                                 float* d_full_logprobs, float* d_last_full, int32_t B, void* stream)
{
    if (B <= 0) return 0;
    WTS_CUDA_CHECK(launch_pdl(decode_select_kernel, dim3(B), dim3(DS_THREADS), 0, (cudaStream_t)stream, d_logits, ldl, *cfg, d_suppress, d_blank, d_tokens,
                                                                    d_n_tokens, d_n_prompt, d_done, d_logprobs, lp_ld,
                                                                    d_full_logprobs, d_last_full));
    WTS_LAUNCH_CHECK();
    return 0;
}

extern "C" int wts_filtered_logprobs(const float* d_logits, int64_t ldl, const WtsDecodeCfg* cfg, const uint8_t* d_suppress,
                                     const uint8_t* d_blank, int32_t* d_tokens, int32_t* d_n_tokens, const int32_t* d_n_prompt,
                                     float* d_out, int32_t B, void* stream)
{
    if (B <= 0) return 0;
    if (!d_logits || !cfg || !d_suppress || !d_blank || !d_tokens || !d_n_tokens || !d_n_prompt || !d_out) {
        set_error("wts_filtered_logprobs: null pointer");
        return -2;
    }
    filtered_logprobs_kernel<<<B, DS_THREADS, 0, (cudaStream_t)stream>>>(d_logits, ldl, *cfg, d_suppress, d_blank, d_tokens,
                                                                         d_n_tokens, d_n_prompt, d_out);
    WTS_LAUNCH_CHECK();
    return 0;
}

extern "C" int wts_step_inputs(const int32_t* d_tokens, int32_t tokens_ld, const int32_t* d_n_tokens,
                               const int32_t* d_n_prompt, const int32_t* d_done, int32_t B, int32_t* d_tok,
                               int32_t* d_pos, int32_t* d_qk_row, int32_t* d_active, void* stream)
{
    if (B <= 0) return 0;
    WTS_CUDA_CHECK(launch_pdl(step_inputs_kernel, dim3((B + 127) / 128), dim3(128), 0, (cudaStream_t)stream, d_tokens, tokens_ld, d_n_tokens, d_n_prompt,
                                                                         d_done, B, d_tok, d_pos, d_qk_row, d_active));
    WTS_LAUNCH_CHECK();
    return 0;
}

extern "C" int wts_softmax_pick(const float* d_logits, int64_t ldl, int32_t n, int32_t index, float* d_out,
                                int32_t rows, void* stream)
{
    if (rows <= 0) return 0;
    softmax_pick_kernel<<<rows, 512, 0, (cudaStream_t)stream>>>(d_logits, ldl, n, index, d_out);
    WTS_LAUNCH_CHECK();
    return 0;
}

extern "C" int wts_logprob_gather(const float* d_logits, int64_t ldl, int32_t n, const int32_t* d_rows,
                                  const int32_t* d_tokens, float* d_out, int32_t count, void* stream)
{
    if (count <= 0) return 0;
    if (!d_logits || !d_rows || !d_tokens || !d_out) { set_error("wts_logprob_gather: null pointer"); return -2; }
    logprob_gather_kernel<<<count, 512, 0, (cudaStream_t)stream>>>(d_logits, ldl, n, d_rows, d_tokens, d_out);
    WTS_LAUNCH_CHECK();
    return 0;
}
```

whisper-timestamped_b200/whisper_timestamped/_native.py:

```python
import ctypes
import os

import numpy as np
import torch

_HERE = os.path.dirname(os.path.abspath(__file__))
LIB_PATH = os.path.join(_HERE, "libwts.so")


class WtsError(RuntimeError):
    pass


class SegDesc(ctypes.Structure):
    _fields_ = [
        ("window", ctypes.c_int32), ("row0", ctypes.c_int32), ("last_row", ctypes.c_int32),
        ("T", ctypes.c_int32), ("f0", ctypes.c_int32), ("F", ctypes.c_int32),
        ("max_dur", ctypes.c_int32), ("flags", ctypes.c_int32),
        ("cost_off", ctypes.c_int64), ("jumps_off", ctypes.c_int64),
        ("dir_off", ctypes.c_int64), ("bnd_off", ctypes.c_int64),
    ]


SEG_DTYPE = np.dtype([
    ("window", "<i4"), ("row0", "<i4"), ("last_row", "<i4"), ("T", "<i4"), ("f0", "<i4"),
    ("F", "<i4"), ("max_dur", "<i4"), ("flags", "<i4"), ("cost_off", "<i8"), ("jumps_off", "<i8"),
    ("dir_off", "<i8"), ("bnd_off", "<i8")])
assert SEG_DTYPE.itemsize == ctypes.sizeof(SegDesc) == 64


class Gemm(ctypes.Structure):
    _fields_ = [
        ("a", ctypes.c_void_p), ("lda", ctypes.c_int64), ("a_plane", ctypes.c_int64), ("a_bo", ctypes.c_int64), ("a_bi", ctypes.c_int64),
        ("b", ctypes.c_void_p), ("ldb", ctypes.c_int64), ("b_plane", ctypes.c_int64), ("b_bo", ctypes.c_int64), ("b_bi", ctypes.c_int64),
        ("M", ctypes.c_int32), ("N", ctypes.c_int32), ("K", ctypes.c_int32), ("batch_outer", ctypes.c_int32), ("batch_inner", ctypes.c_int32),
        ("alpha", ctypes.c_float),
        ("bias", ctypes.c_void_p), ("bias_on_m", ctypes.c_int32), ("act", ctypes.c_int32),
        ("residual", ctypes.c_void_p), ("ldr", ctypes.c_int64), ("r_bo", ctypes.c_int64), ("r_bi", ctypes.c_int64),
        ("out_f32", ctypes.c_void_p), ("ldc", ctypes.c_int64), ("c_bo", ctypes.c_int64), ("c_bi", ctypes.c_int64),
        ("out_sb16", ctypes.c_void_p), ("ldo", ctypes.c_int64), ("o_plane", ctypes.c_int64), ("o_bo", ctypes.c_int64), ("o_bi", ctypes.c_int64),
        ("head_dim", ctypes.c_int32), ("head_stride", ctypes.c_int64),
        ("backend", ctypes.c_int32), ("a_is_f32", ctypes.c_int32), ("b_is_f32", ctypes.c_int32),
        ("row_mask", ctypes.c_void_p),
    ]


class DecodeCfg(ctypes.Structure):
    _fields_ = [("n_vocab", ctypes.c_int32), ("eot", ctypes.c_int32), ("timestamp_begin", ctypes.c_int32),
                ("no_timestamps", ctypes.c_int32), ("max_initial_ts", ctypes.c_int32), ("sample_len", ctypes.c_int32),
                ("n_ctx", ctypes.c_int32), ("tokens_ld", ctypes.c_int32)]


class DecLayer(ctypes.Structure):
    _fields_ = [(n, ctypes.c_void_p) for n in (
        "ln1_g", "ln1_b", "w_qkv", "b_qkv", "w_o", "b_o",
        "ln2_g", "ln2_b", "w_cq", "b_cq", "w_co", "b_co",
        "ln3_g", "ln3_b", "w_fc1", "b_fc1", "w_fc2", "b_fc2",
        "self_k", "self_v", "cross_k16", "cross_v16", "cross_k_align", "head_slot",
        "sb_qkv", "sb_o", "sb_cq", "sb_co", "sb_fc1", "sb_fc2")] + [(n, ctypes.c_int64) for n in (
        "pl_qkv", "pl_o", "pl_cq", "pl_co", "pl_fc1", "pl_fc2")]


class DecodeSteps(ctypes.Structure):
    _fields_ = [(n, ctypes.c_void_p) for n in (
        "layers", "emb", "pos", "ln_g", "ln_b", "tokens", "n_tokens", "n_prompt", "done",
        "logprobs", "full", "last_full", "qk_buf", "suppress", "blank",
        "x", "qkv", "att", "q", "mid", "logits", "sync", "prof", "emb_sb")] + [("emb_plane", ctypes.c_int64),
                                                                              ("use_mma", ctypes.c_int64), ("cfg", DecodeCfg)] + [(n, ctypes.c_int32) for n in (
        "n_layer", "D", "H", "n_ctx", "n_audio_ctx", "n_slots", "cap", "lp_ld", "qk_rows", "n_steps", "max_rows",
        "prof_cap")]


def _load():
    if not os.path.exists(LIB_PATH):
        raise ImportError(
            f"{LIB_PATH} not found: build it with `python whisper-timestamped_b200/build.py` "
            "(the product has no CPU fallback)")
    lib = ctypes.CDLL(LIB_PATH)
    lib.wts_version.restype = ctypes.c_int
    lib.wts_last_error.restype = ctypes.c_char_p
    lib.wts_dtw_dir_words.restype = ctypes.c_int64
    lib.wts_dtw_dir_words.argtypes = [ctypes.c_int32, ctypes.c_int32]
    lib.wts_dtw_bnd_doubles.restype = ctypes.c_int64
    lib.wts_dtw_bnd_doubles.argtypes = [ctypes.c_int32, ctypes.c_int32]
    vp, i32 = ctypes.c_void_p, ctypes.c_int32
    lib.wts_attn_prep_batch.restype = ctypes.c_int
    lib.wts_attn_prep_batch.argtypes = [vp, i32, i32, i32, vp, i32, i32, i32, vp, vp]
    lib.wts_dtw_batch.restype = ctypes.c_int
    lib.wts_dtw_batch.argtypes = [vp, i32, vp, i32, vp, vp, vp, vp, vp, vp, vp, vp]
    lib.wts_dtw_batch_sized.restype = ctypes.c_int
    lib.wts_dtw_batch_sized.argtypes = [vp, i32, vp, i32, vp, vp, vp, vp, vp, vp, vp, i32, i32, i32, vp]
    lib.wts_disfluency_starts.restype = ctypes.c_int
    lib.wts_disfluency_starts.argtypes = [vp, vp, i32, vp, vp, vp]
    i64, f32p = ctypes.c_int64, vp
    lib.wts_gemm.restype = ctypes.c_int
    lib.wts_gemm.argtypes = [ctypes.POINTER(Gemm), vp]
    lib.wts_to_sb16.argtypes = [vp, i64, vp, vp, vp]
    lib.wts_layernorm.argtypes = [vp, i64, vp, vp, i32, i32, vp, i64, i64, vp, i64, vp]
    lib.wts_softmax_rows.argtypes = [vp, i64, i64, i32, vp, i64, i64, vp]
    lib.wts_frames.argtypes = [vp, i64, i64, i64, vp, i64, vp]
    lib.wts_power.argtypes = [vp, i64, i64, vp, i64, i64, vp]
    lib.wts_logmel_max.argtypes = [vp, i64, vp, vp]
    lib.wts_logmel_finish.argtypes = [vp, i64, i32, vp, vp, vp]
    lib.wts_window_gather.argtypes = [vp, i32, vp, vp, i32, vp, i64, vp]
    lib.wts_embed.argtypes = [vp, vp, vp, vp, i32, i32, vp, vp]
    lib.wts_gather_rows.argtypes = [vp, i64, vp, i32, i32, vp, vp]
    lib.wts_decoder_attention.argtypes = [i32, vp, i64, vp, vp, i64, i32, vp, vp, i32, i32, vp, i64, i64, vp, vp, i32,
                                          i32, vp, vp, vp]
    lib.wts_cross_kv_pack.argtypes = [vp, vp, vp, vp, i32, i32, i32, i32, vp]
    lib.wts_cross_attention_f16.argtypes = [vp, i64, vp, vp, vp, vp, i32, i32, vp, i32, i32, vp, i64, i64, vp, i32, vp, vp, vp]
    lib.wts_enc_attention.argtypes = [vp, i64, i64, vp, i64, i64, i32, i32, i32, i32, vp, i64, i64, vp]
    lib.wts_enc_attention.restype = ctypes.c_int
    lib.wts_kv_append.argtypes = [vp, vp, i64, vp, vp, i32, i32, i32, vp, vp, i64, vp]
    lib.wts_decode_select.argtypes = [vp, i64, ctypes.POINTER(DecodeCfg), vp, vp, vp, vp, vp, vp, vp, i32, vp, vp, i32, vp]
    lib.wts_filtered_logprobs.argtypes = [vp, i64, ctypes.POINTER(DecodeCfg), vp, vp, vp, vp, vp, vp, i32, vp]
    lib.wts_filtered_logprobs.restype = ctypes.c_int
    lib.wts_decode_steps.argtypes = [ctypes.POINTER(DecodeSteps), vp]
    lib.wts_decode_steps.restype = ctypes.c_int
    lib.wts_decode_step_kernels.argtypes = [ctypes.POINTER(DecodeSteps), vp, vp]
    lib.wts_decode_step_kernels.restype = ctypes.c_int
    lib.wts_step_inputs.argtypes = [vp, i32, vp, vp, vp, i32, vp, vp, vp, vp, vp]
    lib.wts_softmax_pick.argtypes = [vp, i64, i32, i32, vp, i32, vp]
    lib.wts_logprob_gather.argtypes = [vp, i64, i32, vp, vp, vp, i32, vp]
    for name in ("wts_to_sb16", "wts_layernorm", "wts_softmax_rows", "wts_frames", "wts_power", "wts_logmel_max",
                 "wts_logmel_finish", "wts_window_gather", "wts_embed", "wts_gather_rows", "wts_decoder_attention",
                 "wts_kv_append", "wts_decode_select", "wts_step_inputs", "wts_softmax_pick", "wts_logprob_gather", "wts_cross_kv_pack",
                 "wts_cross_attention_f16"):
        getattr(lib, name).restype = ctypes.c_int
    return lib


lib = _load()

EXPORTED_SYMBOLS = [
    "wts_version", "wts_last_error", "wts_dtw_dir_words", "wts_dtw_bnd_doubles",
    "wts_attn_prep_batch", "wts_dtw_batch", "wts_dtw_batch_sized", "wts_disfluency_starts", "wts_gemm", "wts_to_sb16", "wts_layernorm", "wts_softmax_rows",
    "wts_frames", "wts_power", "wts_logmel_max", "wts_logmel_finish", "wts_window_gather", "wts_embed",
    "wts_gather_rows", "wts_decoder_attention", "wts_kv_append", "wts_decode_select", "wts_filtered_logprobs", "wts_decode_steps", "wts_decode_step_kernels", "wts_step_inputs",
    "wts_softmax_pick", "wts_logprob_gather", "wts_cross_kv_pack", "wts_cross_attention_f16", "wts_enc_attention",
]


def check(rc: int, what: str):
    if rc != 0:
        raise WtsError(f"{what} failed ({rc}): {lib.wts_last_error().decode(errors='replace')}")


def ptr(t):
    if t is None:
        return None
    assert t.is_contiguous(), "libwts needs contiguous buffers"
    return ctypes.c_void_p(t.data_ptr())


def stream_ptr(device=None):
    return ctypes.c_void_p(torch.cuda.current_stream(device).cuda_stream)


def require_cuda(t, name):
    if not t.is_cuda:
        raise WtsError(f"{name} must live on a CUDA device: libwts has no CPU path")
```

whisper-timestamped_b200/whisper_timestamped/engine.py:

```python
import ctypes
import os

import numpy as np
import torch

from . import _native as nat
from .alignment import attn_prep, dtw, plan_segments, split_jumps
from .model import SB16
from .windows import N_FRAMES, WindowRecord

N_SAMPLES = 480000
N_CTX_AUDIO = 1500
KPAD = 1504


def _i32(x, dev):
    return torch.as_tensor(np.asarray(x, dtype=np.int32)).to(dev)


class CudaEngine:
    def __init__(self, model, max_batch=None, gemm_backend=None, keep_full_logprobs=False, small_batch_rows=None):
        self.m = model
        self.dev = model.device
        self.w = model.w
        self.dims = model.dims
        self.max_batch = max_batch or int(os.environ.get("WTS_MAX_BATCH", "64"))
        self.backend = int(os.environ.get("WTS_GEMM_BACKEND", "0")) if gemm_backend is None else gemm_backend
        self.conv_backend = int(os.environ.get("WTS_CONV_BACKEND", str(self.backend)))
        self.fused_attention = os.environ.get("WTS_FUSED_ATTN", "1") != "0"
        self.keep_full_logprobs = keep_full_logprobs
        self.qk_buffers = []
        self.window_index = []
        self.full_logprobs = []
        self.launches = 0
        self.use_graph = os.environ.get("WTS_CUDA_GRAPH", "1") != "0"
        self.small_batch_rows = min(32, int(os.environ.get("WTS_SMALL_BATCH_ROWS", "8")) if small_batch_rows is None
                                    else int(small_batch_rows))
        self.small_batch_steps = 0
        self.small_batch_mode = os.environ.get("WTS_SMALL_BATCH_MODE", "lean")
        self.small_batch_mma = os.environ.get("WTS_SMALL_BATCH_MMA", "1") != "0"
        self._graphs = {}
        self.profile = False
        self._events = []

    class _Phase:
        def __init__(self, eng, name):
            self.eng, self.name = eng, name

        def __enter__(self):
            if self.eng.profile:
                self.a = torch.cuda.Event(enable_timing=True)
                self.b = torch.cuda.Event(enable_timing=True)
                self.a.record(torch.cuda.current_stream(self.eng.dev))

        def __exit__(self, *exc):
            if self.eng.profile:
                self.b.record(torch.cuda.current_stream(self.eng.dev))
                self.eng._events.append((self.name, self.a, self.b))

    def phase(self, name):
        return CudaEngine._Phase(self, name)

    def stage_ms(self, reset=True):
        torch.cuda.synchronize(self.dev)
        out = {}
        self.batch_ms = [(B, steps, self._events[i][1].elapsed_time(self._events[i][2]))
                         for (B, steps, i) in getattr(self, "batch_log", [])]
        self.batch_log = []
        for name, a, b in self._events:
            out[name] = out.get(name, 0.0) + a.elapsed_time(b)
        if reset:
            self._events = []
        return out

    def _st(self):
        return nat.stream_ptr(self.dev)

    def gemm(self, a, b, M, N, K, *, lda=None, ldb=None, a_plane=None, b_plane=None, a_off=0, b_off=0,
             batch=(1, 1), a_b=(0, 0), b_b=(0, 0), alpha=1.0, bias=None, bias_on_m=False, act=0,
             residual=None, ldr=0, r_b=(0, 0), out_f32=None, ldc=0, c_b=(0, 0), c_off=0,
             out_sb=None, ldo=0, o_plane=0, o_b=(0, 0), o_off=0, head_dim=0, head_stride=0,
             a_f32=False, b_f32=False, backend=None, row_mask=None):
        g = nat.Gemm()
        if a_f32:
            g.a, g.lda, g.a_plane = a.data_ptr() + 4 * a_off, lda, 0
        else:
            g.a, g.lda, g.a_plane = a.ptr + 2 * a_off, lda or a.ld, a_plane if a_plane is not None else a.plane
        if b_f32:
            g.b, g.ldb, g.b_plane = b.data_ptr() + 4 * b_off, ldb, 0
        else:
            g.b, g.ldb, g.b_plane = b.ptr + 2 * b_off, ldb or b.ld, b_plane if b_plane is not None else b.plane
        g.a_bo, g.a_bi = a_b
        g.b_bo, g.b_bi = b_b
        g.M, g.N, g.K = M, N, K
        g.batch_outer, g.batch_inner = batch
        g.alpha = alpha
        g.bias = bias.data_ptr() if bias is not None else None
        g.bias_on_m = 1 if bias_on_m else 0
        g.act = act
        if residual is not None:
            g.residual, g.ldr = residual.data_ptr(), ldr
            g.r_bo, g.r_bi = r_b
        if out_f32 is not None:
            g.out_f32, g.ldc = out_f32.data_ptr() + 4 * c_off, ldc
            g.c_bo, g.c_bi = c_b
        if out_sb is not None:
            g.out_sb16, g.ldo, g.o_plane = out_sb.ptr + 2 * o_off, ldo or out_sb.ld, o_plane or out_sb.plane
            g.o_bo, g.o_bi = o_b
        g.head_dim, g.head_stride = head_dim, head_stride
        g.backend = self.backend if backend is None else backend
        g.a_is_f32, g.b_is_f32 = int(a_f32), int(b_f32)
        g.row_mask = row_mask.data_ptr() if row_mask is not None else None
        if a_f32 or b_f32:
            g.backend = 1
        nat.check(nat.lib.wts_gemm(ctypes.byref(g), self._st()), "wts_gemm")
        self.launches += 1

    def layernorm(self, x, gamma, beta, M, D, out_sb=None, out_f32=None):
        nat.check(nat.lib.wts_layernorm(x.data_ptr(), D, gamma.data_ptr(), beta.data_ptr(), M, D,
                                        out_sb.ptr if out_sb is not None else None,
                                        out_sb.ld if out_sb is not None else 0,
                                        out_sb.plane if out_sb is not None else 0,
                                        out_f32.data_ptr() if out_f32 is not None else None, D, self._st()),
                  "wts_layernorm")
        self.launches += 1

    def load_audio(self, audio):
        if isinstance(audio, str):
            import wave
            with wave.open(audio, "rb") as wv:
                if wv.getframerate() != 16000 or wv.getnchannels() != 1 or wv.getsampwidth() != 2:
                    raise RuntimeError("only 16 kHz mono s16 .wav files can be read here (no ffmpeg in this environment)")
                data = wv.readframes(wv.getnframes())
            audio = np.frombuffer(data, np.int16).astype(np.float32) / 32768.0
        if isinstance(audio, np.ndarray):
            audio = torch.from_numpy(np.ascontiguousarray(audio, dtype=np.float32))
        assert isinstance(audio, torch.Tensor), f"Got unexpected audio of type {type(audio)}"
        audio = audio.float()
        if audio.device != self.dev:
            audio = (audio.pin_memory() if audio.device.type == "cpu" else audio).to(self.dev, non_blocking=True)
        return audio.contiguous()

    def log_mel(self, audio, pad_30s=True):
        with self.phase("mel"):
            return self._log_mel(audio, N_SAMPLES if pad_30s else 0)

    def _log_mel(self, audio, padding=N_SAMPLES):
        dev, st = self.dev, self._st()
        n = int(audio.numel())
        total = n + padding
        nf = total // 160
        C = self.dims.n_mels
        frames = torch.empty((nf, 400), dtype=torch.float32, device=dev)
        nat.check(nat.lib.wts_frames(audio.data_ptr(), n, total, nf, frames.data_ptr(), 0, st), "wts_frames")
        y = torch.empty((nf, 416), dtype=torch.float32, device=dev)
        self.gemm(frames, self.w.dft, nf, 416, 400, lda=400, ldb=400, a_f32=True, b_f32=True, out_f32=y, ldc=416)
        p = torch.empty((nf, 208), dtype=torch.float32, device=dev)
        nat.check(nat.lib.wts_power(y.data_ptr(), 416, nf, p.data_ptr(), 208, 0, st), "wts_power")
        mel = torch.empty((nf, C), dtype=torch.float32, device=dev)
        self.gemm(p, self.w.melfb, nf, C, 208, lda=208, ldb=208, a_f32=True, b_f32=True, out_f32=mel, ldc=C)
        key = torch.full((1,), -2 ** 31, dtype=torch.int32, device=dev)
        nat.check(nat.lib.wts_logmel_max(mel.data_ptr(), nf * C, key.data_ptr(), st), "wts_logmel_max")
        out = torch.empty((nf, C), dtype=torch.float32, device=dev)
        nat.check(nat.lib.wts_logmel_finish(mel.data_ptr(), nf, C, key.data_ptr(), out.data_ptr(), st), "wts_logmel_finish")
        self.launches += 6
        return out

    def mel_frames(self, mel):
        return int(mel.shape[0])

    def encode(self, jobs):
        d, dev, st, w = self.dims, self.dev, self._st(), self.w
        B, C, D, H = len(jobs), d.n_mels, d.n_audio_state, d.n_audio_head
        ptrs = torch.as_tensor(np.array([j["mel"].data_ptr() for j in jobs], dtype=np.int64)).to(dev)
        seek = _i32([j["seek"] for j in jobs], dev)
        size = _i32([j["segment_size"] for j in jobs], dev)
        x0 = SB16(B * 3002, C, dev)
        nat.check(nat.lib.wts_window_gather(ptrs.data_ptr(), C, seek.data_ptr(), size.data_ptr(), B, x0.ptr, x0.plane, st),
                  "wts_window_gather")
        h1 = SB16(B * 3001, D, dev)
        self.gemm(x0, w.conv1, 3000, D, 3 * C, lda=C, batch=(B, 1), a_b=(3002 * C, 0), bias=w.conv1_b, act=1,
                  out_sb=h1, ldo=D, o_b=(3001 * D, 0), o_off=D, backend=self.conv_backend)
        x = torch.empty((B * 1500, D), dtype=torch.float32, device=dev)
        self.gemm(h1, w.conv2, 1500, D, 3 * D, lda=2 * D, batch=(B, 1), a_b=(3001 * D, 0), bias=w.conv2_b, act=1,
                  residual=w.enc_pos, ldr=D, r_b=(0, 0), out_f32=x, ldc=D, c_b=(1500 * D, 0), backend=self.conv_backend)
        R = B * 1500
        hs = SB16(R, D, dev)
        qk = SB16(R, 2 * D, dev)
        vt = SB16(B * D, KPAD, dev)
        fused = self.backend == 0 and self.fused_attention
        if not fused:
            S = torch.empty((B * H * 1500, KPAD), dtype=torch.float32, device=dev)
            P = SB16(B * H * 1500, KPAD, dev)
        att = SB16(R, D, dev)
        mid = SB16(R, 4 * D, dev)
        for blk in w.enc:
            a = blk.attn
            self.layernorm(x, a.ln_g, a.ln_b, R, D, out_sb=hs)
            self.gemm(hs, a.qk, R, 2 * D, D, bias=a.qk_b, out_sb=qk)
            self.gemm(a.v, hs, D, 1500, D, batch=(B, 1), b_b=(1500 * D, 0), bias=a.v_b, bias_on_m=True,
                      out_sb=vt, ldo=KPAD, o_b=(D * KPAD, 0))
            if fused:
                nat.check(nat.lib.wts_enc_attention(qk.ptr, 2 * D, qk.plane, vt.ptr, KPAD, vt.plane, B, H, D, 1500,
                                                    att.ptr, D, att.plane, st), "wts_enc_attention")
                self.launches += 1
            else:
                self.gemm(qk, qk, 1500, 1500, 64, lda=2 * D, ldb=2 * D, b_off=D, batch=(B, H),
                          a_b=(1500 * 2 * D, 64), b_b=(1500 * 2 * D, 64), out_f32=S, ldc=KPAD,
                          c_b=(H * 1500 * KPAD, 1500 * KPAD))
                nat.check(nat.lib.wts_softmax_rows(S.data_ptr(), KPAD, B * H * 1500, 1500, P.ptr, KPAD, P.plane, st),
                          "wts_softmax_rows")
                self.launches += 1
                self.gemm(P, vt, 1500, 64, 1500, lda=KPAD, ldb=KPAD, batch=(B, H),
                          a_b=(H * 1500 * KPAD, 1500 * KPAD), b_b=(D * KPAD, 64 * KPAD), out_sb=att, ldo=D,
                          o_b=(1500 * D, 64))
            self.gemm(att, a.out, R, D, D, bias=a.out_b, residual=x, ldr=D, out_f32=x, ldc=D)
            self.layernorm(x, blk.mlp_ln_g, blk.mlp_ln_b, R, D, out_sb=hs)
            self.gemm(hs, blk.fc1, R, 4 * D, D, bias=blk.fc1_b, act=1, out_sb=mid)
            self.gemm(mid, blk.fc2, R, D, 4 * D, bias=blk.fc2_b, residual=x, ldr=D, out_f32=x, ldc=D)
        xa = SB16(R, D, dev)
        self.layernorm(x, w.ln_post_g, w.ln_post_b, R, D, out_sb=xa)
        return xa

    def _decoder_rows(self, st8, x, R, row_seq, row_pos, qk_row, qk_buf, active=None):
        d, w, st = self.dims, self.w, self._st()
        D, H, L = d.n_text_state, d.n_text_head, d.n_text_layer
        hs, qkv, att, q, mid = st8["hs"], st8["qkv"], st8["att"], st8["q"], st8["mid"]
        n_slots = len(self.m.heads)
        for li, blk in enumerate(w.dec):
            a, c = blk.attn, blk.cross
            self.layernorm(x, a.ln_g, a.ln_b, R, D, out_sb=hs)
            self.gemm(hs, a.qkv, R, 3 * D, D, bias=a.qkv_b, out_f32=qkv, ldc=3 * D, row_mask=active)
            fused_append = active is not None
            if not fused_append:
                nat.check(nat.lib.wts_kv_append(qkv.data_ptr() + 4 * D, qkv.data_ptr() + 8 * D, 3 * D, row_seq.data_ptr(),
                                                row_pos.data_ptr(), R, H, d.n_text_ctx, st8["sk"][li].data_ptr(),
                                                st8["sv"][li].data_ptr(), H * d.n_text_ctx * 64, st), "wts_kv_append")
                self.launches += 1
            nat.check(nat.lib.wts_decoder_attention(2 if fused_append else 0, qkv.data_ptr(), 3 * D, st8["sk"][li].data_ptr(),
                                                    st8["sv"][li].data_ptr(), H * d.n_text_ctx * 64, d.n_text_ctx,
                                                    row_seq.data_ptr(), row_pos.data_ptr(), R, H, att.ptr, att.ld,
                                                    att.plane, None, None, 0, 0, None,
                                                    active.data_ptr() if active is not None else None, st),
                      "wts_decoder_attention")
            self.gemm(att, a.out, R, D, D, bias=a.out_b, residual=x, ldr=D, out_f32=x, ldc=D, row_mask=active)
            self.layernorm(x, c.ln_g, c.ln_b, R, D, out_sb=hs)
            self.gemm(hs, c.q, R, D, D, bias=c.q_b, out_f32=q, ldc=D, row_mask=active)
            nat.check(nat.lib.wts_cross_attention_f16(q.data_ptr(), D, st8["ck"][li].data_ptr(), st8["cv"][li].data_ptr(),
                                                      st8["ckal"][li].data_ptr(), w.head_slot[li].data_ptr(), n_slots,
                                                      N_CTX_AUDIO, row_seq.data_ptr(), R, H, att.ptr, att.ld, att.plane,
                                                      qk_buf.data_ptr(), qk_buf.shape[2], qk_row.data_ptr(),
                                                      active.data_ptr() if active is not None else None, st),
                      "wts_cross_attention_f16")
            self.gemm(att, c.out, R, D, D, bias=c.out_b, residual=x, ldr=D, out_f32=x, ldc=D, row_mask=active)
            self.layernorm(x, blk.mlp_ln_g, blk.mlp_ln_b, R, D, out_sb=hs)
            self.gemm(hs, blk.fc1, R, 4 * D, D, bias=blk.fc1_b, act=1, out_sb=mid, row_mask=active)
            self.gemm(mid, blk.fc2, R, D, 4 * D, bias=blk.fc2_b, residual=x, ldr=D, out_f32=x, ldc=D, row_mask=active)
            self.launches += 2

    def _alloc_decoder_state(self, B, R):
        d, dev = self.dims, self.dev
        D, H, L = d.n_text_state, d.n_text_head, d.n_text_layer
        f32 = dict(dtype=torch.float32, device=dev)
        return dict(
            hs=SB16(R, D, dev), att=SB16(R, D, dev), mid=SB16(R, 4 * D, dev),
            qkv=torch.empty((R, 3 * D), **f32), q=torch.empty((R, D), **f32),
            sk=[torch.zeros((B, H, d.n_text_ctx, 64), **f32) for _ in range(L)],
            sv=[torch.zeros((B, H, d.n_text_ctx, 64), **f32) for _ in range(L)],
            ck=[torch.empty((B, H, N_CTX_AUDIO, 64), dtype=torch.float16, device=dev) for _ in range(L)],
            cv=[torch.empty((B, H, N_CTX_AUDIO, 64), dtype=torch.float16, device=dev) for _ in range(L)],
            ckal=[torch.empty((B, max(1, len(self.m.heads)), N_CTX_AUDIO, 64), **f32) for _ in range(L)],
            kvtmp=torch.empty((B, H, N_CTX_AUDIO, 64), **f32))

    def _cross_kv(self, xa, st8, B):
        d = self.dims
        D, H = d.n_text_state, d.n_text_head
        for li, blk in enumerate(self.w.dec):
            c = blk.cross
            tmp = st8["kvtmp"]
            n_slots = len(self.m.heads)
            for (wt, bias, dst, al) in ((c.k, None, st8["ck"][li], st8["ckal"][li]), (c.v, c.v_b, st8["cv"][li], None)):
                self.gemm(xa, wt, 1500, D, D, batch=(B, 1), a_b=(1500 * D, 0), bias=bias, out_f32=tmp, ldc=64,
                          c_b=(H * 1500 * 64, 0), head_dim=64, head_stride=1500 * 64)
                nat.check(nat.lib.wts_cross_kv_pack(tmp.data_ptr(), dst.data_ptr(), al.data_ptr() if al is not None else None,
                                                    self.w.head_slot[li].data_ptr(), n_slots, B, H, N_CTX_AUDIO, self._st()),
                          "wts_cross_kv_pack")
                self.launches += 1

    def _final_logits(self, x_rows, n_rows, logits):
        d, w = self.dims, self.w
        D, V = d.n_text_state, d.n_vocab
        hs = SB16(n_rows, D, self.dev)
        self.layernorm(x_rows, w.ln_g, w.ln_b, n_rows, D, out_sb=hs)
        self.gemm(hs, w.emb_sb, n_rows, V, D, out_f32=logits, ldc=V)

    def decode_windows(self, jobs, setup):
        if getattr(setup, "beam_size", None) is not None or setup.temperature > 0:
            return [self._decode_strategy(job, setup) for job in jobs]
        out = []
        for i in range(0, len(jobs), self.max_batch):
            out.extend(self._decode_batch(jobs[i:i + self.max_batch], setup))
        return out

    def _decoder_session(self, setup, need):
        d, dev = self.dims, self.dev
        tok = setup.tokenizer
        V, D, n_ctx = d.n_vocab, d.n_text_state, d.n_text_ctx
        ses = getattr(self, "_session", None)
        cap = 4
        while cap < need:
            cap *= 2
        cap = min(cap, max(self.max_batch, need))
        if ses is not None and ses["cap"] >= need:
            cap = ses["cap"]
        key = (cap, setup.sample_len, tok.eot, tok.timestamp_begin, tok.no_timestamps, setup.max_initial_timestamp_index,
               self.keep_full_logprobs, self.small_batch_rows)
        if ses is not None and ses["key"] == key:
            return ses
        self._session = ses = None
        qk_rows = setup.sample_len + 1
        n_slots = len(self.m.heads)
        i32 = dict(dtype=torch.int32, device=dev)
        ses = dict(key=key, cap=cap, qk_rows=qk_rows, graph=None, per_step=0)
        ses["st8"] = self._alloc_decoder_state(cap, cap)
        ses["st8"]["hs_fin"] = SB16(cap, D, dev)
        ses["tokens"] = torch.zeros((cap, n_ctx + 1), **i32)
        ses["n_tokens"] = torch.ones(cap, **i32)
        ses["n_prompt"] = torch.ones(cap, **i32)
        ses["done"] = torch.ones(cap, **i32)
        ses["logprobs"] = torch.zeros((cap, qk_rows), dtype=torch.float32, device=dev)
        ses["full"] = torch.empty((cap, qk_rows, V), dtype=torch.float32, device=dev) if self.keep_full_logprobs else None
        ses["qk_buf"] = torch.zeros((cap, max(1, n_slots), qk_rows, N_CTX_AUDIO), dtype=torch.float32, device=dev)
        ses["s_tok"] = torch.zeros(cap, **i32)
        ses["s_pos"] = torch.zeros(cap, **i32)
        ses["s_qkr"] = torch.zeros(cap, **i32)
        ses["s_act"] = torch.zeros(cap, **i32)
        ses["seq_ids"] = _i32(list(range(cap)), dev)
        ses["logits"] = torch.empty((cap, V), dtype=torch.float32, device=dev)
        ses["xs"] = torch.empty((cap, D), dtype=torch.float32, device=dev)
        ses["last_full"] = torch.zeros((cap, V), dtype=torch.float32, device=dev)
        ses["suppress"] = torch.zeros(V, dtype=torch.uint8, device=dev)
        ses["blank"] = torch.zeros(V, dtype=torch.uint8, device=dev)
        ses["cfg"] = nat.DecodeCfg(n_vocab=V, eot=tok.eot, timestamp_begin=tok.timestamp_begin,
                                   no_timestamps=tok.no_timestamps,
                                   max_initial_ts=-1 if setup.max_initial_timestamp_index is None else setup.max_initial_timestamp_index,
                                   sample_len=setup.sample_len, n_ctx=n_ctx, tokens_ld=n_ctx + 1)
        ses["steps"] = self._steps_descriptor(ses) if self.small_batch_rows > 0 else None
        self._session = ses
        return ses

    def _steps_descriptor(self, ses):
        d, w, dev = self.dims, self.w, self.dev
        D, H, L, V = d.n_text_state, d.n_text_head, d.n_text_layer, d.n_vocab
        if D % 128 != 0 or D > 1280 or D != 64 * H:
            return None
        st8, cap = ses["st8"], ses["cap"]
        layers = (nat.DecLayer * L)()
        for li, blk in enumerate(w.dec):
            a, c, y = blk.attn, blk.cross, layers[li]
            y.ln1_g, y.ln1_b, y.w_qkv, y.b_qkv = a.ln_g.data_ptr(), a.ln_b.data_ptr(), a.qkv_f32.data_ptr(), a.qkv_b.data_ptr()
            y.w_o, y.b_o = a.out_f32.data_ptr(), a.out_b.data_ptr()
            y.ln2_g, y.ln2_b, y.w_cq, y.b_cq = c.ln_g.data_ptr(), c.ln_b.data_ptr(), c.q_f32.data_ptr(), c.q_b.data_ptr()
            y.w_co, y.b_co = c.out_f32.data_ptr(), c.out_b.data_ptr()
            y.ln3_g, y.ln3_b = blk.mlp_ln_g.data_ptr(), blk.mlp_ln_b.data_ptr()
            y.w_fc1, y.b_fc1, y.w_fc2, y.b_fc2 = blk.fc1_f32.data_ptr(), blk.fc1_b.data_ptr(), blk.fc2_f32.data_ptr(), blk.fc2_b.data_ptr()
            y.self_k, y.self_v = st8["sk"][li].data_ptr(), st8["sv"][li].data_ptr()
            y.cross_k16, y.cross_v16 = st8["ck"][li].data_ptr(), st8["cv"][li].data_ptr()
            y.cross_k_align, y.head_slot = st8["ckal"][li].data_ptr(), w.head_slot[li].data_ptr()
            for name, sb in (("qkv", a.qkv), ("o", a.out), ("cq", c.q), ("co", c.out), ("fc1", blk.fc1), ("fc2", blk.fc2)):
                assert sb.ld == sb.cols
                setattr(y, "sb_" + name, sb.ptr)
                setattr(y, "pl_" + name, sb.plane)
        raw = np.frombuffer(bytes(layers), dtype=np.uint8).copy()
        f32 = dict(dtype=torch.float32, device=dev)
        keep = dict(layers=torch.from_numpy(raw).to(dev), x=torch.zeros((cap, D), **f32), qkv=torch.zeros((cap, 3 * D), **f32),
                    att=torch.zeros((cap, D), **f32), q=torch.zeros((cap, D), **f32), mid=torch.zeros((cap, 4 * D), **f32),
                    sync=torch.zeros(64, dtype=torch.int32, device=dev))
        p = nat.DecodeSteps()
        p.layers = keep["layers"].data_ptr()
        p.emb, p.pos, p.ln_g, p.ln_b = w.emb.data_ptr(), w.dec_pos.data_ptr(), w.ln_g.data_ptr(), w.ln_b.data_ptr()
        p.tokens, p.n_tokens, p.n_prompt, p.done = (ses[k].data_ptr() for k in ("tokens", "n_tokens", "n_prompt", "done"))
        p.logprobs, p.qk_buf = ses["logprobs"].data_ptr(), ses["qk_buf"].data_ptr()
        p.full = ses["full"].data_ptr() if ses["full"] is not None else None
        p.last_full = ses["last_full"].data_ptr()
        p.suppress, p.blank = ses["suppress"].data_ptr(), ses["blank"].data_ptr()
        p.x, p.qkv, p.att, p.q, p.mid = (keep[k].data_ptr() for k in ("x", "qkv", "att", "q", "mid"))
        p.logits, p.sync = ses["logits"].data_ptr(), keep["sync"].data_ptr()
        p.emb_sb, p.emb_plane = w.emb_sb.ptr, w.emb_sb.plane
        p.use_mma = 1 if self.small_batch_mma else 0
        p.cfg = ses["cfg"]
        p.n_layer, p.D, p.H, p.n_ctx, p.n_audio_ctx = L, D, H, d.n_text_ctx, N_CTX_AUDIO
        p.n_slots, p.cap, p.lp_ld, p.qk_rows = max(1, len(self.m.heads)), cap, ses["qk_rows"], ses["qk_rows"]
        return dict(args=p, keep=keep, host_layers=layers, graphs={})

    def _lean_graph(self, ses, n_active):
        sd = ses["steps"]
        rows = 4 if n_active <= 4 else 8 if n_active <= 8 else 16 if n_active <= 16 else 32
        key = (rows, bool(self.small_batch_mma))
        if key in sd["graphs"]:
            return sd["graphs"][key]
        dev = self.dev
        p = sd["args"]

        def launch():
            p.max_rows, p.n_steps, p.use_mma = rows, 1, int(key[1])
            nat.check(nat.lib.wts_decode_step_kernels(ctypes.byref(p), ctypes.byref(sd["host_layers"]), self._st()),
                      "wts_decode_step_kernels")
        saved = {k: ses[k].clone() for k in ("tokens", "n_tokens", "done", "logprobs")}
        launch()
        torch.cuda.synchronize(dev)
        for k, v in saved.items():
            ses[k].copy_(v)
        graph = torch.cuda.CUDAGraph()
        cap_stream = torch.cuda.Stream(device=dev)
        cap_stream.wait_stream(torch.cuda.current_stream(dev))
        with torch.cuda.stream(cap_stream):
            with torch.cuda.graph(graph, stream=cap_stream):
                launch()
        torch.cuda.current_stream(dev).wait_stream(cap_stream)
        sd["graphs"][key] = graph
        return graph

    def _step_graph(self, ses):
        if ses["graph"] is not None:
            return ses["graph"]
        dev = self.dev
        saved = {k: ses[k].clone() for k in ("tokens", "n_tokens", "done", "logprobs")}
        self._step(ses)
        torch.cuda.synchronize(dev)
        for k, v in saved.items():
            ses[k].copy_(v)
        graph = torch.cuda.CUDAGraph()
        cap_stream = torch.cuda.Stream(device=dev)
        cap_stream.wait_stream(torch.cuda.current_stream(dev))
        l0 = self.launches
        with torch.cuda.stream(cap_stream):
            with torch.cuda.graph(graph, stream=cap_stream):
                self._step(ses)
        ses["per_step"] = self.launches - l0
        self.launches = l0
        torch.cuda.current_stream(dev).wait_stream(cap_stream)
        ses["graph"] = graph
        return graph

    def _run_steps(self, ses, n_steps, n_active):
        sd = ses["steps"]
        p = sd["args"]
        p.n_steps, p.max_rows = int(n_steps), int(n_active)
        nat.check(nat.lib.wts_decode_steps(ctypes.byref(p), self._st()), "wts_decode_steps")
        self.launches += 1

    def _select(self, ses, logits, rows):
        d = self.dims
        nat.check(nat.lib.wts_decode_select(logits.data_ptr(), d.n_vocab, ctypes.byref(ses["cfg"]), ses["suppress"].data_ptr(),
                                            ses["blank"].data_ptr(), ses["tokens"].data_ptr(), ses["n_tokens"].data_ptr(),
                                            ses["n_prompt"].data_ptr(), ses["done"].data_ptr(), ses["logprobs"].data_ptr(),
                                            ses["qk_rows"], ses["full"].data_ptr() if ses["full"] is not None else None,
                                            ses["last_full"].data_ptr(), rows, self._st()), "wts_decode_select")
        self.launches += 1

    def _step(self, ses):
        self._step_logits(ses)
        self._select(ses, ses["logits"], ses["cap"])
        self.launches += 1

    def _step_logits(self, ses):
        d, w, st = self.dims, self.w, self._st()
        cap, D = ses["cap"], d.n_text_state
        nat.check(nat.lib.wts_step_inputs(ses["tokens"].data_ptr(), d.n_text_ctx + 1, ses["n_tokens"].data_ptr(),
                                          ses["n_prompt"].data_ptr(), ses["done"].data_ptr(), cap, ses["s_tok"].data_ptr(),
                                          ses["s_pos"].data_ptr(), ses["s_qkr"].data_ptr(), ses["s_act"].data_ptr(), st),
                  "wts_step_inputs")
        nat.check(nat.lib.wts_embed(ses["s_tok"].data_ptr(), ses["s_pos"].data_ptr(), w.emb.data_ptr(), w.dec_pos.data_ptr(),
                                    cap, D, ses["xs"].data_ptr(), st), "wts_embed")
        self._decoder_rows(ses["st8"], ses["xs"], cap, ses["seq_ids"], ses["s_pos"], ses["s_qkr"], ses["qk_buf"],
                           active=ses["s_act"])
        self._final_logits_static(ses["xs"], cap, ses["logits"], ses["st8"], active=ses["s_act"])
        self.launches += 1

    @torch.no_grad()
    def _decode_batch(self, jobs, setup):
        d, dev, st, w = self.dims, self.dev, self._st(), self.w
        tok = setup.tokenizer
        B = len(jobs)
        D, V = d.n_text_state, d.n_vocab
        n_ctx = d.n_text_ctx
        sample_len = setup.sample_len
        ses = self._decoder_session(setup, B)
        cap, qk_rows = ses["cap"], ses["qk_rows"]
        assert B <= cap
        st8 = ses["st8"]
        with self.phase("encoder"):
            xa = self.encode(jobs)
        prompts = [list(j["prompt"]) for j in jobs]
        P = [len(p) for p in prompts]
        R0 = sum(P)
        with self.phase("cross_kv"):
            self._cross_kv(xa, st8, B)
        del xa

        tokens_h = np.zeros((cap, n_ctx + 1), dtype=np.int32)
        for b, p in enumerate(prompts):
            tokens_h[b, :len(p)] = p
        ses["tokens"].copy_(torch.from_numpy(tokens_h), non_blocking=False)
        nt = np.ones(cap, dtype=np.int32)
        nt[:B] = P
        ses["n_tokens"].copy_(torch.from_numpy(nt))
        ses["n_prompt"].copy_(torch.from_numpy(nt))
        dn = np.ones(cap, dtype=np.int32)
        dn[:B] = 0
        ses["done"].copy_(torch.from_numpy(dn))
        ses["logprobs"].zero_()
        ses["suppress"].zero_()
        ses["suppress"][torch.as_tensor(list(setup.suppress_tokens), dtype=torch.long, device=dev)] = 1
        ses["blank"].zero_()
        if setup.blank_tokens:
            ses["blank"][torch.as_tensor(list(setup.blank_tokens), dtype=torch.long, device=dev)] = 1
        qk_buf = ses["qk_buf"]

        row_seq = _i32([b for b, p in enumerate(prompts) for _ in p], dev)
        row_pos = _i32([i for p in prompts for i in range(len(p))], dev)
        row_tok = _i32([t for p in prompts for t in p], dev)
        qk_row = _i32([0 if i == len(p) - 1 else -1 for p in prompts for i in range(len(p))], dev)
        f32 = dict(dtype=torch.float32, device=dev)
        pre = dict(st8)
        pre.update(hs=SB16(R0, D, dev), att=SB16(R0, D, dev), mid=SB16(R0, 4 * D, dev),
                   qkv=torch.empty((R0, 3 * D), **f32), q=torch.empty((R0, D), **f32))
        x = torch.empty((R0, D), **f32)
        ph = self.phase("prefill")
        ph.__enter__()
        nat.check(nat.lib.wts_embed(row_tok.data_ptr(), row_pos.data_ptr(), w.emb.data_ptr(), w.dec_pos.data_ptr(), R0, D,
                                    x.data_ptr(), st), "wts_embed")
        self._decoder_rows(pre, x, R0, row_seq, row_pos, qk_row, qk_buf)
        ends = np.cumsum(P) - 1
        sot_rows = [int(ends[b] - P[b] + 1 + prompts[b].index(tok.sot)) for b in range(B)]
        sel = _i32(list(ends) + sot_rows, dev)
        xr = torch.empty((2 * B, D), **f32)
        nat.check(nat.lib.wts_gather_rows(x.data_ptr(), D, sel.data_ptr(), 2 * B, D, xr.data_ptr(), st), "wts_gather_rows")
        logits2 = torch.empty((2 * B, V), **f32)
        self._final_logits(xr, 2 * B, logits2)
        no_speech = torch.zeros(B, **f32)
        if tok.no_speech is not None:
            nat.check(nat.lib.wts_softmax_pick(logits2.data_ptr() + 4 * B * V, V, V, tok.no_speech, no_speech.data_ptr(), B, st),
                      "wts_softmax_pick")
        self._select(ses, logits2, B)
        ph.__exit__()
        del pre, x, xr

        max_steps = sample_len - 1
        steps_done = 0
        ph = self.phase("decode_steps")
        ph.__enter__()
        done = ses["done"]
        n_active = B
        while steps_done < max_steps and n_active > 0:
            left = max_steps - steps_done
            if ses["steps"] is not None and n_active <= self.small_batch_rows and self.small_batch_mode == "lean":
                chunk = min(8, left)
                graph = self._lean_graph(ses, n_active)
                for _ in range(chunk):
                    graph.replay()
                self.launches += chunk * (8 * d.n_text_layer + 3)
                self.small_batch_steps += chunk
            elif ses["steps"] is not None and n_active <= self.small_batch_rows:
                chunk = min(32, left)
                self._run_steps(ses, chunk, n_active)
                self.small_batch_steps += chunk
            else:
                chunk = min(8, left)
                graph = self._step_graph(ses) if (self.use_graph and max_steps > 4) else None
                for _ in range(chunk):
                    if graph is not None:
                        graph.replay()
                        self.launches += ses["per_step"]
                    else:
                        self._step(ses)
            steps_done += chunk
            n_active = int((done == 0).sum().item())
        if ses["steps"] is not None:
            flags = ses["steps"]["keep"]["sync"].cpu().numpy()
            if flags[1] != 0:
                raise nat.WtsError("wts_decode_steps: grid barrier timed out (results invalid)")
        ph.__exit__()
        self.decode_steps_run = getattr(self, "decode_steps_run", 0) + steps_done
        if self.profile:
            self.batch_log = getattr(self, "batch_log", [])
            self.batch_log.append((B, steps_done, len(self._events) - 1))
        torch.cuda.synchronize(dev)
        tokens_h = ses["tokens"][:B].cpu().numpy()
        n_tok_h = ses["n_tokens"][:B].cpu().numpy()
        done_h = ses["done"][:B].cpu().numpy()
        lp_h = ses["logprobs"][:B].cpu().numpy()
        ns_h = no_speech.cpu().numpy()
        max_rows = int(max(1, (n_tok_h - np.asarray(P)).max() + 1))
        buf_idx = len(self.qk_buffers)
        self.qk_buffers.append(qk_buf[:B, :, :max_rows].clone())
        full = ses["full"]
        if full is not None:
            self.full_logprobs.append(full[:B, :max_rows].clone())
            full = self.full_logprobs[-1]
        limit_rows = [b for b in range(B) if int(done_h[b]) == 2]
        last_full_h = {}
        if limit_rows:
            lf = ses["last_full"][torch.as_tensor(limit_rows, device=dev)].cpu()
            last_full_h = {b: lf[i] for i, b in enumerate(limit_rows)}
        records = []
        for b, job in enumerate(jobs):
            n = int(n_tok_h[b] - P[b])
            ended = int(done_h[b]) == 1
            rows = n + 1 if ended else n
            sampled = tokens_h[b, P[b]:P[b] + n].tolist()
            gid = len(self.window_index)
            self.window_index.append((buf_idx, b))
            last_lp = None
            if b in last_full_h:
                last_lp = (lambda t, row=last_full_h[b]: float(row[t]))
            elif full is not None:
                last_lp = (lambda t, bb=b, rr=rows - 1, ff=full: float(ff[bb, rr, t].item()))
            records.append(WindowRecord(seek=job["seek"], segment_size=job["segment_size"], prompt=prompts[b],
                                        tokens=sampled, logprobs=lp_h[b, :rows].copy(), ended_by_eot=ended,
                                        no_speech_prob=float(ns_h[b]), qk_window=gid, temperature=0.0,
                                        language=tok.language, last_row_logprobs=last_lp))
        return records

    @torch.no_grad()
    def decode_stream(self, jobs, setup, feed):
        d, dev, st, w = self.dims, self.dev, self._st(), self.w
        tok = setup.tokenizer
        assert not self.keep_full_logprobs, "decode_stream keeps no per-row log-prob tables"
        D, V, n_ctx = d.n_text_state, d.n_vocab, d.n_text_ctx
        queue = list(jobs)
        if not queue:
            return
        ses = self._decoder_session(setup, min(self.max_batch, len(queue)))
        cap, st8, qk_buf = ses["cap"], ses["st8"], ses["qk_buf"]
        f32 = dict(dtype=torch.float32, device=dev)
        ses["done"].fill_(1)
        ses["suppress"].zero_()
        ses["suppress"][torch.as_tensor(list(setup.suppress_tokens), dtype=torch.long, device=dev)] = 1
        ses["blank"].zero_()
        if setup.blank_tokens:
            ses["blank"][torch.as_tensor(list(setup.blank_tokens), dtype=torch.long, device=dev)] = 1
        slot_job = [None] * cap
        slot_info = [None] * cap
        free = list(range(cap))
        max_steps = setup.sample_len - 1

        def admit(batch):
            n = len(batch)
            slots = [b for b, _ in batch]
            d_slots = torch.as_tensor(slots, dtype=torch.long, device=dev)
            with self.phase("encoder"):
                xa = self.encode([j for _, j in batch])
            with self.phase("cross_kv"):
                if slots == list(range(n)):
                    self._cross_kv(xa, st8, n)
                else:
                    tmp = self._alloc_cross_state(n)
                    self._cross_kv(xa, tmp, n)
                    for li in range(d.n_text_layer):
                        for name in ("ck", "cv", "ckal"):
                            st8[name][li].index_copy_(0, d_slots, tmp[name][li])
                    del tmp
                del xa
            prompts = [list(j["prompt"]) for _, j in batch]
            P = [len(p) for p in prompts]
            R0 = sum(P)
            th = np.zeros((n, n_ctx + 1), dtype=np.int32)
            for k, p in enumerate(prompts):
                th[k, :len(p)] = p
            ses["tokens"].index_copy_(0, d_slots, torch.from_numpy(th).to(dev))
            nt = torch.as_tensor(P, dtype=torch.int32, device=dev)
            ses["n_tokens"].index_copy_(0, d_slots, nt)
            ses["n_prompt"].index_copy_(0, d_slots, nt)
            ses["logprobs"].index_fill_(0, d_slots, 0.0)
            with self.phase("prefill"):
                row_seq = _i32([b for b, p in zip(slots, prompts) for _ in p], dev)
                row_pos = _i32([i for p in prompts for i in range(len(p))], dev)
                row_tok = _i32([t for p in prompts for t in p], dev)
                qk_row = _i32([0 if i == len(p) - 1 else -1 for p in prompts for i in range(len(p))], dev)
                pre = dict(st8)
                pre.update(hs=SB16(R0, D, dev), att=SB16(R0, D, dev), mid=SB16(R0, 4 * D, dev),
                           qkv=torch.empty((R0, 3 * D), **f32), q=torch.empty((R0, D), **f32))
                x = torch.empty((R0, D), **f32)
                nat.check(nat.lib.wts_embed(row_tok.data_ptr(), row_pos.data_ptr(), w.emb.data_ptr(), w.dec_pos.data_ptr(), R0, D,
                                            x.data_ptr(), st), "wts_embed")
                self._decoder_rows(pre, x, R0, row_seq, row_pos, qk_row, qk_buf)
                ends = np.cumsum(P) - 1
                sot_rows = [int(ends[k] - P[k] + 1 + prompts[k].index(tok.sot)) for k in range(n)]
                sel = _i32(list(ends) + sot_rows, dev)
                xr = torch.empty((2 * n, D), **f32)
                nat.check(nat.lib.wts_gather_rows(x.data_ptr(), D, sel.data_ptr(), 2 * n, D, xr.data_ptr(), st), "wts_gather_rows")
                logits2 = torch.empty((2 * n, V), **f32)
                self._final_logits(xr, 2 * n, logits2)
                no_speech = torch.zeros(n, **f32)
                if tok.no_speech is not None:
                    nat.check(nat.lib.wts_softmax_pick(logits2.data_ptr() + 4 * n * V, V, V, tok.no_speech, no_speech.data_ptr(), n, st),
                              "wts_softmax_pick")
                ses["logits"].index_copy_(0, d_slots, logits2[:n])
                saved = ses["done"].clone()
                ses["done"].fill_(1)
                ses["done"].index_fill_(0, d_slots, 0)
                self._select(ses, ses["logits"], cap)
                mask = torch.zeros(cap, dtype=torch.bool, device=dev)
                mask[d_slots] = True
                ses["done"].copy_(torch.where(mask, ses["done"], saved))
                self.launches += 4
            ns = no_speech.cpu().numpy()
            for k, (b, job) in enumerate(batch):
                slot_job[b] = job
                slot_info[b] = (prompts[k], float(ns[k]))

        def collect(finished, done_h):
            d_f = torch.as_tensor(finished, dtype=torch.long, device=dev)
            tokens_h = ses["tokens"].index_select(0, d_f).cpu().numpy()
            n_tok_h = ses["n_tokens"].index_select(0, d_f).cpu().numpy()
            lp_h = ses["logprobs"].index_select(0, d_f).cpu().numpy()
            limit = [k for k, b in enumerate(finished) if int(done_h[b]) == 2]
            last_rows = {}
            if limit:
                lf = ses["last_full"].index_select(0, d_f[torch.as_tensor(limit, device=dev)]).cpu()
                last_rows = {k: lf[i] for i, k in enumerate(limit)}
            out = []
            n_rows = [int(n_tok_h[k]) - len(slot_info[b][0]) + (1 if int(done_h[b]) == 1 else 0) for k, b in enumerate(finished)]
            buf_idx = len(self.qk_buffers)
            self.qk_buffers.append(qk_buf.index_select(0, d_f)[:, :, :max(1, max(n_rows))].contiguous())
            for k, b in enumerate(finished):
                prompt, ns = slot_info[b]
                job = slot_job[b]
                n = int(n_tok_h[k]) - len(prompt)
                ended = int(done_h[b]) == 1
                rows = n + 1 if ended else n
                gid = len(self.window_index)
                self.window_index.append((buf_idx, k))
                last_lp = (lambda t, row=last_rows[k]: float(row[t])) if k in last_rows else None
                out.append((job, WindowRecord(seek=job["seek"], segment_size=job["segment_size"], prompt=prompt,
                                              tokens=tokens_h[k, len(prompt):len(prompt) + n].tolist(), logprobs=lp_h[k, :rows].copy(),
                                              ended_by_eot=ended, no_speech_prob=ns, qk_window=gid, temperature=0.0,
                                              language=tok.language, last_row_logprobs=last_lp)))
                slot_job[b] = slot_info[b] = None
            return out

        done = ses["done"]
        while queue or any(j is not None for j in slot_job):
            if queue and free:
                batch = []
                while queue and free:
                    batch.append((free.pop(0), queue.pop(0)))
                admit(batch)
            ph = self.phase("decode_steps")
            ph.__enter__()
            n_active = int((done == 0).sum().item())
            if n_active > 0:
                chunk = 8
                if ses["steps"] is not None and n_active <= self.small_batch_rows and self.small_batch_mode == "lean":
                    graph = self._lean_graph(ses, n_active)
                    for _ in range(chunk):
                        graph.replay()
                    self.launches += chunk * (8 * d.n_text_layer + 3)
                    self.small_batch_steps += chunk
                else:
                    graph = self._step_graph(ses) if (self.use_graph and max_steps > 4) else None
                    for _ in range(chunk):
                        if graph is not None:
                            graph.replay()
                            self.launches += ses["per_step"]
                        else:
                            self._step(ses)
                self.decode_steps_run = getattr(self, "decode_steps_run", 0) + chunk
            ph.__exit__()
            done_h = done.cpu().numpy()
            finished = [b for b in range(cap) if slot_job[b] is not None and int(done_h[b]) != 0]
            if finished:
                for job, rec in collect(finished, done_h):
                    nxt = feed(job, rec)
                    if nxt is not None:
                        queue.append(nxt)
                free.extend(finished)
                free.sort()

    def _alloc_cross_state(self, B):
        d, dev = self.dims, self.dev
        H, L = d.n_text_head, d.n_text_layer
        return dict(
            ck=[torch.empty((B, H, N_CTX_AUDIO, 64), dtype=torch.float16, device=dev) for _ in range(L)],
            cv=[torch.empty((B, H, N_CTX_AUDIO, 64), dtype=torch.float16, device=dev) for _ in range(L)],
            ckal=[torch.empty((B, max(1, len(self.m.heads)), N_CTX_AUDIO, 64), dtype=torch.float32, device=dev) for _ in range(L)],
            kvtmp=torch.empty((B, H, N_CTX_AUDIO, 64), dtype=torch.float32, device=dev))

    @torch.no_grad()
    def _decode_strategy(self, job, setup):
        d, dev, st, w = self.dims, self.dev, self._st(), self.w
        tok = setup.tokenizer
        G = setup.n_group
        beam = setup.beam_size
        T = float(setup.temperature)
        ses = self._decoder_session(setup, G)
        cap, st8 = ses["cap"], ses["st8"]
        D, V, L, n_ctx = d.n_text_state, d.n_vocab, d.n_text_layer, d.n_text_ctx
        f32 = dict(dtype=torch.float32, device=dev)
        with self.phase("encoder"):
            xa = self.encode([job])
        with self.phase("cross_kv"):
            self._cross_kv(xa, st8, 1)
            for li in range(L):
                for name in ("ck", "cv", "ckal"):
                    t = st8[name][li]
                    if G > 1:
                        t[1:G].copy_(t[0:1].expand(G - 1, *t.shape[1:]))
        del xa
        prompt = list(job["prompt"])
        P = len(prompt)
        tokens_h = np.zeros((cap, n_ctx + 1), dtype=np.int32)
        tokens_h[:G, :P] = prompt
        ses["tokens"].copy_(torch.from_numpy(tokens_h))
        nt = np.ones(cap, dtype=np.int32)
        nt[:G] = P
        ses["n_tokens"].copy_(torch.from_numpy(nt))
        ses["n_prompt"].copy_(torch.from_numpy(nt))
        dn = np.ones(cap, dtype=np.int32)
        dn[:G] = 0
        ses["done"].copy_(torch.from_numpy(dn))
        ses["suppress"].zero_()
        ses["suppress"][torch.as_tensor(list(setup.suppress_tokens), dtype=torch.long, device=dev)] = 1
        ses["blank"].zero_()
        if setup.blank_tokens:
            ses["blank"][torch.as_tensor(list(setup.blank_tokens), dtype=torch.long, device=dev)] = 1
        with self.phase("prefill"):
            row_seq = _i32([0] * P, dev)
            row_pos = _i32(list(range(P)), dev)
            row_tok = _i32(prompt, dev)
            qk_row = _i32([-1] * P, dev)
            pre = dict(st8)
            pre.update(hs=SB16(P, D, dev), att=SB16(P, D, dev), mid=SB16(P, 4 * D, dev),
                       qkv=torch.empty((P, 3 * D), **f32), q=torch.empty((P, D), **f32))
            x = torch.empty((P, D), **f32)
            nat.check(nat.lib.wts_embed(row_tok.data_ptr(), row_pos.data_ptr(), w.emb.data_ptr(), w.dec_pos.data_ptr(), P, D,
                                        x.data_ptr(), st), "wts_embed")
            self._decoder_rows(pre, x, P, row_seq, row_pos, qk_row, ses["qk_buf"])
            sel = _i32([P - 1, prompt.index(tok.sot)], dev)
            xr = torch.empty((2, D), **f32)
            nat.check(nat.lib.wts_gather_rows(x.data_ptr(), D, sel.data_ptr(), 2, D, xr.data_ptr(), st), "wts_gather_rows")
            logits2 = torch.empty((2, V), **f32)
            self._final_logits(xr, 2, logits2)
            no_speech = torch.zeros(1, **f32)
            if tok.no_speech is not None:
                nat.check(nat.lib.wts_softmax_pick(logits2.data_ptr() + 4 * V, V, V, tok.no_speech, no_speech.data_ptr(), 1, st),
                          "wts_softmax_pick")
            for li in range(L):
                for name in ("sk", "sv"):
                    t = st8[name][li]
                    if G > 1:
                        t[1:G, :, :P].copy_(t[0:1, :, :P].expand(G - 1, t.shape[1], P, t.shape[3]))
            ses["logits"][:G].copy_(logits2[0:1].expand(G, V))
            self.launches += 6
        del pre, x, xr
        lp_dev = torch.empty((cap, V), **f32)
        seqs = [list(prompt) for _ in range(G)]
        sum_lp = torch.zeros(G, dtype=torch.float32)
        finished = {}
        max_candidates = round(beam * (setup.patience or 1.0)) if beam else 0
        ph = self.phase("decode_steps")
        ph.__enter__()
        for i in range(setup.sample_len):
            nat.check(nat.lib.wts_filtered_logprobs(ses["logits"].data_ptr(), V, ctypes.byref(ses["cfg"]), ses["suppress"].data_ptr(),
                                                    ses["blank"].data_ptr(), ses["tokens"].data_ptr(), ses["n_tokens"].data_ptr(),
                                                    ses["n_prompt"].data_ptr(), lp_dev.data_ptr(), G, st), "wts_filtered_logprobs")
            self.launches += 1
            source = list(range(G))
            if beam:
                vals, idxs = torch.topk(lp_dev[:G], beam + 1, dim=-1)
                vals, idxs = vals.cpu(), idxs.cpu()
                scores, sources = {}, {}
                for j in range(G):
                    prefix = seqs[j]
                    for logprob, token in zip(vals[j], idxs[j]):
                        sequence = tuple(prefix + [int(token)])
                        scores[sequence] = (sum_lp[j] + logprob).item()
                        sources[sequence] = j
                new_seqs, source, newly_finished = [], [], {}
                for sequence in sorted(scores, key=scores.get, reverse=True):
                    if sequence[-1] == tok.eot:
                        newly_finished[sequence] = scores[sequence]
                    else:
                        sum_lp[len(new_seqs)] = scores[sequence]
                        new_seqs.append(list(sequence))
                        source.append(sources[sequence])
                        if len(new_seqs) == beam:
                            break
                for seq in sorted(newly_finished, key=newly_finished.get, reverse=True):
                    if len(finished) >= max_candidates:
                        break
                    finished[seq] = newly_finished[seq]
                seqs = new_seqs
                completed = len(finished) >= max_candidates
            else:
                lp = lp_dev[:G].cpu()
                nxt = torch.distributions.Categorical(logits=lp / T).sample()
                last = torch.tensor([s_[-1] for s_ in seqs])
                sum_lp += lp[torch.arange(G), nxt] * (last != tok.eot)
                nxt[last == tok.eot] = tok.eot
                for s_, t_ in zip(seqs, nxt.tolist()):
                    s_.append(t_)
                completed = bool((nxt == tok.eot).all())
            cur = len(seqs[0])
            if completed or cur > n_ctx:
                break
            if i + 1 == setup.sample_len:
                break
            if source != list(range(G)):
                src = torch.as_tensor(source, dtype=torch.long, device=dev)
                for li in range(L):
                    for name in ("sk", "sv"):
                        t = st8[name][li]
                        t[:G, :, :cur - 1] = t[src, :, :cur - 1]
            th = np.zeros((G, n_ctx + 1), dtype=np.int32)
            for r, s_ in enumerate(seqs):
                th[r, :cur] = s_
            ses["tokens"][:G].copy_(torch.from_numpy(th))
            ses["n_tokens"][:G].fill_(cur)
            self._step_logits(ses)
        ph.__exit__()
        if beam:
            if len(finished) < beam:
                for j in list(np.argsort(sum_lp.numpy()))[::-1]:
                    finished[tuple(seqs[j] + [tok.eot])] = sum_lp[j].item()
                    if len(finished) >= beam:
                        break
            cands = [list(k) for k in finished.keys()]
            cand_lp = list(finished.values())
        else:
            cands = [s_ + [tok.eot] for s_ in seqs]
            cand_lp = sum_lp.tolist()
        cut = []
        for c in cands:
            body = c[P:]
            cut.append(body[:body.index(tok.eot)])
        lp_len = [len(c) for c in cut]
        if setup.length_penalty is None:
            score = [lp / n if n else (float("-inf") if lp < 0 else float("inf")) for lp, n in zip(cand_lp, lp_len)]
        else:
            score = [lp / (((5 + n) / 6) ** setup.length_penalty) for lp, n in zip(cand_lp, lp_len)]
        best = int(np.argmax(score))
        torch.cuda.synchronize(dev)
        return WindowRecord(seek=job["seek"], segment_size=job["segment_size"], prompt=prompt, tokens=cut[best], logprobs=None,
                            ended_by_eot=True, no_speech_prob=float(no_speech.cpu()[0]), qk_window=-1, temperature=T,
                            language=tok.language, sum_logprob=float(cand_lp[best]))

    def _final_logits_static(self, x_rows, n_rows, logits, st8, active=None):
        d, w = self.dims, self.w
        hs = st8["hs_fin"]
        self.layernorm(x_rows, w.ln_g, w.ln_b, n_rows, d.n_text_state, out_sb=hs)
        self.gemm(hs, w.emb_sb, n_rows, d.n_vocab, d.n_text_state, out_f32=logits, ldc=d.n_vocab, row_mask=active)

    @torch.no_grad()
    def teacher_forced(self, mel, tokens_in, i_start, pairs):
        d, dev, st, w = self.dims, self.dev, self._st(), self.w
        tokens_in = [int(t) for t in tokens_in]
        R, D, V = len(tokens_in), d.n_text_state, d.n_vocab
        assert 0 < R <= d.n_text_ctx, f"{R} tokens do not fit the decoder context ({d.n_text_ctx})"
        size = min(N_FRAMES, int(mel.shape[0]))
        with self.phase("encoder"):
            xa = self.encode([dict(mel=mel, seek=0, segment_size=size)])
        st8 = getattr(self, "_tf_state", None)
        if st8 is None:
            st8 = self._tf_state = self._alloc_decoder_state(1, d.n_text_ctx)
        with self.phase("cross_kv"):
            self._cross_kv(xa, st8, 1)
        del xa
        rows = R - (i_start - 1)
        qk_buf = torch.zeros((1, max(1, len(self.m.heads)), rows, N_CTX_AUDIO), dtype=torch.float32, device=dev)
        row_seq = _i32([0] * R, dev)
        row_pos = _i32(list(range(R)), dev)
        row_tok = _i32(tokens_in, dev)
        qk_row = _i32([p - (i_start - 1) if p >= i_start - 1 else -1 for p in range(R)], dev)
        x = torch.empty((R, D), dtype=torch.float32, device=dev)
        with self.phase("prefill"):
            nat.check(nat.lib.wts_embed(row_tok.data_ptr(), row_pos.data_ptr(), w.emb.data_ptr(), w.dec_pos.data_ptr(), R, D,
                                        x.data_ptr(), st), "wts_embed")
            self.launches += 1
            self._decoder_rows(st8, x, R, row_seq, row_pos, qk_row, qk_buf)
            vals = np.zeros(0, dtype=np.float32)
            if pairs:
                steps = sorted({int(s_) for (s_, _) in pairs})
                index = {s_: i for i, s_ in enumerate(steps)}
                sel = _i32(steps, dev)
                xr = torch.empty((len(steps), D), dtype=torch.float32, device=dev)
                nat.check(nat.lib.wts_gather_rows(x.data_ptr(), D, sel.data_ptr(), len(steps), D, xr.data_ptr(), st),
                          "wts_gather_rows")
                logits = torch.empty((len(steps), V), dtype=torch.float32, device=dev)
                self._final_logits(xr, len(steps), logits)
                d_rows = _i32([index[int(s_)] for (s_, _) in pairs], dev)
                d_tok = _i32([int(t_) for (_, t_) in pairs], dev)
                out = torch.empty(len(pairs), dtype=torch.float32, device=dev)
                nat.check(nat.lib.wts_logprob_gather(logits.data_ptr(), V, V, d_rows.data_ptr(), d_tok.data_ptr(),
                                                     out.data_ptr(), len(pairs), st), "wts_logprob_gather")
                self.launches += 2
                vals = out.cpu().numpy()
        buf_idx = len(self.qk_buffers)
        self.qk_buffers.append(qk_buf)
        gid = len(self.window_index)
        self.window_index.append((buf_idx, 0))
        return gid, vals

    @torch.no_grad()
    def detect_language(self, mel, tokenizer):
        d, dev, st, w = self.dims, self.dev, self._st(), self.w
        size = min(N_FRAMES, int(mel.shape[0]))
        job = dict(mel=mel, seek=0, segment_size=size)
        xa = self.encode([job])
        st8 = self._alloc_decoder_state(1, 1)
        self._cross_kv(xa, st8, 1)
        qk_buf = torch.zeros((1, max(1, len(self.m.heads)), 1, N_CTX_AUDIO), dtype=torch.float32, device=dev)
        x = torch.empty((1, d.n_text_state), dtype=torch.float32, device=dev)
        one = _i32([0], dev)
        t = _i32([tokenizer.sot], dev)
        nat.check(nat.lib.wts_embed(t.data_ptr(), one.data_ptr(), w.emb.data_ptr(), w.dec_pos.data_ptr(), 1, d.n_text_state,
                                    x.data_ptr(), st), "wts_embed")
        self._decoder_rows(st8, x, 1, one, one, _i32([-1], dev), qk_buf)
        logits = torch.empty((1, d.n_vocab), dtype=torch.float32, device=dev)
        self._final_logits(x, 1, logits)
        lg = logits[0].cpu()
        ids = list(tokenizer.all_language_tokens)
        probs = torch.softmax(lg[ids].float(), dim=-1).tolist()
        language_probs = dict(zip(tokenizer.all_language_codes, probs))
        return max(language_probs, key=language_probs.get), language_probs

    def align(self, items, disfluencies=False):
        out = [None] * len(items)
        lefts = [None] * len(items)
        groups = {}
        for i, it in enumerate(items):
            buf, b = self.window_index[it["window"]]
            groups.setdefault(buf, []).append((i, b, it))
        queued = []
        for buf, lst in groups.items():
            plan = plan_segments([(b, it["row0"], it["last_row"], it["T"], it["f0"], it["F"], it["max_dur"])
                                  for (_, b, it) in lst], nonpositive=True)
            qk = self.qk_buffers[buf]
            with self.phase("align_prep"):
                cost = attn_prep(qk, plan)
            with self.phase("align_dtw"):
                res = dtw(cost, plan)
            self.launches += 3
            dl = None
            if disfluencies:
                from .alignment import disfluency_starts
                dl = disfluency_starts(cost, plan, res["jumps"])
                self.launches += 1
            queued.append((lst, plan, res["jumps"], dl))
        for lst, plan, d_jumps, dl in queued:
            jumps = split_jumps(d_jumps.cpu().numpy(), plan)
            for (i, _, _), j in zip(lst, jumps):
                out[i] = j
            if dl is not None:
                for (i, _, _), l_ in zip(lst, split_jumps(dl.cpu().numpy(), plan)):
                    lefts[i] = l_[:-1]
        return (out, lefts) if disfluencies else out

    def release(self):
        self.qk_buffers.clear()
        self.window_index.clear()
        self.full_logprobs.clear()
```

whisper-timestamped_b200/whisper_timestamped/model.py:

```python
import math
import os
from types import SimpleNamespace

import torch

from . import _native as nat
from . import model_zoo as zoo


class SB16:

    def __init__(self, rows, cols, device, ld=None):
        self.rows, self.cols = rows, cols
        self.ld = ld or cols
        self.t = torch.zeros((2, rows, self.ld), dtype=torch.bfloat16, device=device)

    @property
    def plane(self):
        return self.rows * self.ld

    @property
    def ptr(self):
        return self.t.data_ptr()

    @staticmethod
    def from_f32(x: torch.Tensor):
        x = x.contiguous().float()
        assert x.dim() == 2 and x.is_cuda
        out = SB16(x.shape[0], x.shape[1], x.device)
        nat.check(nat.lib.wts_to_sb16(nat.ptr(x), x.numel(), out.t[0].data_ptr(), out.t[1].data_ptr(),
                                      nat.stream_ptr(x.device)), "wts_to_sb16")
        return out

    def to_f32(self):
        return self.t[0].float() + self.t[1].float()


class WhisperB200:

    def __init__(self, dims: zoo.ModelDimensions, state_dict, device, name=None, alignment_heads=None):
        if not torch.cuda.is_available():
            raise nat.WtsError("whisper_timestamped (B200 drop-in) needs a CUDA device: there is no CPU fallback")
        self.dims = dims
        self.name = name
        self.device = torch.device(device if device is not None else "cuda")
        self.heads = list(alignment_heads) if alignment_heads is not None else zoo.default_alignment_heads(dims)
        mask = torch.zeros(dims.n_text_layer, dims.n_text_head, dtype=torch.bool)
        for l, h in self.heads:
            mask[l, h] = True
        self.alignment_heads = mask.to_sparse()
        self.heads = sorted(self.heads)
        self._engine = None
        self.w = self._prepare(state_dict)

    @property
    def is_multilingual(self):
        return self.dims.n_vocab >= 51865

    @property
    def num_languages(self):
        return self.dims.n_vocab - 51765 - int(self.is_multilingual)

    def engine(self):
        if self._engine is None:
            from .engine import CudaEngine
            self._engine = CudaEngine(self)
        return self._engine

    def transcribe(self, audio, **opts):
        from .transcribe import transcribe_timestamped
        return transcribe_timestamped(self, audio, **opts)

    def _prepare(self, sd):
        dev = self.device
        d = self.dims

        def g(name):
            return sd[name].to(dev, dtype=torch.float32).contiguous()

        def lin(wt):
            return SB16.from_f32(wt)

        w = SimpleNamespace()
        C, da = d.n_mels, d.n_audio_state
        w.conv1 = lin(g("encoder.conv1.weight").permute(0, 2, 1).reshape(da, 3 * C))
        w.conv1_b = g("encoder.conv1.bias")
        w.conv2 = lin(g("encoder.conv2.weight").permute(0, 2, 1).reshape(da, 3 * da))
        w.conv2_b = g("encoder.conv2.bias")
        w.enc_pos = g("encoder.positional_embedding")

        def attn_block(prefix, dm, n_head, cross, keep_f32=False):
            scale = (dm // n_head) ** -0.25
            b = SimpleNamespace()
            b.ln_g, b.ln_b = g(prefix + "_ln.weight"), g(prefix + "_ln.bias")
            q, qb = g(prefix + ".query.weight") * scale, g(prefix + ".query.bias") * scale
            k = g(prefix + ".key.weight") * scale
            v, vb = g(prefix + ".value.weight"), g(prefix + ".value.bias")
            zeros = torch.zeros_like(qb)
            out_w = g(prefix + ".out.weight")
            if cross:
                b.q, b.q_b = lin(q), qb
                b.k = lin(k)
                b.v, b.v_b = lin(v), vb
                b.q_f32 = q.contiguous()
            else:
                qkv = torch.cat([q, k, v], 0).contiguous()
                b.qkv = lin(qkv)
                b.qkv_b = torch.cat([qb, zeros, vb]).contiguous()
                if keep_f32:
                    b.qkv_f32 = qkv
                else:
                    b.qk = lin(torch.cat([q, k], 0))
                    b.qk_b = torch.cat([qb, zeros]).contiguous()
                    b.v, b.v_b = lin(v), vb
            b.out, b.out_b = lin(out_w), g(prefix + ".out.bias")
            if keep_f32:
                b.out_f32 = out_w
            return b

        def block(prefix, dm, n_head, cross):
            blk = SimpleNamespace()
            blk.attn = attn_block(prefix + ".attn", dm, n_head, False, keep_f32=cross)
            blk.cross = attn_block(prefix + ".cross_attn", dm, n_head, True, keep_f32=True) if cross else None
            blk.mlp_ln_g, blk.mlp_ln_b = g(prefix + ".mlp_ln.weight"), g(prefix + ".mlp_ln.bias")
            fc1, fc2 = g(prefix + ".mlp.0.weight"), g(prefix + ".mlp.2.weight")
            blk.fc1, blk.fc1_b = lin(fc1), g(prefix + ".mlp.0.bias")
            blk.fc2, blk.fc2_b = lin(fc2), g(prefix + ".mlp.2.bias")
            if cross:
                blk.fc1_f32, blk.fc2_f32 = fc1, fc2
            return blk

        w.enc = [block(f"encoder.blocks.{i}", da, d.n_audio_head, False) for i in range(d.n_audio_layer)]
        w.ln_post_g, w.ln_post_b = g("encoder.ln_post.weight"), g("encoder.ln_post.bias")
        dt = d.n_text_state
        w.emb = g("decoder.token_embedding.weight")
        w.emb_sb = lin(w.emb)
        w.dec_pos = g("decoder.positional_embedding")
        w.dec = [block(f"decoder.blocks.{i}", dt, d.n_text_head, True) for i in range(d.n_text_layer)]
        w.ln_g, w.ln_b = g("decoder.ln.weight"), g("decoder.ln.bias")
        slots = torch.full((d.n_text_layer, d.n_text_head), -1, dtype=torch.int32)
        for s, (l, h) in enumerate(self.heads):
            slots[l, h] = s
        w.head_slot = slots.to(dev)
        n = torch.arange(400, dtype=torch.float64)
        k = torch.arange(201, dtype=torch.float64)[:, None]
        ang = 2 * math.pi * k * n / 400.0
        basis = torch.zeros(416, 400, dtype=torch.float64)
        basis[:201] = torch.cos(ang)
        basis[208:409] = -torch.sin(ang)
        w.dft = basis.float().to(dev).contiguous()
        fb = torch.zeros(C, 208, dtype=torch.float32)
        fb[:, :201] = torch.from_numpy(mel_filterbank(C))
        w.melfb = fb.to(dev).contiguous()
        torch.cuda.synchronize(dev)
        return w


def mel_filterbank(n_mels: int):
    import numpy as np

    def hz_to_mel(f):
        f = np.asarray(f, dtype=np.float64)
        f_sp = 200.0 / 3
        min_log_hz, min_log_mel, logstep = 1000.0, 1000.0 / f_sp, np.log(6.4) / 27.0
        return np.where(f >= min_log_hz, min_log_mel + np.log(np.maximum(f, 1e-10) / min_log_hz) / logstep, f / f_sp)

    def mel_to_hz(m):
        m = np.asarray(m, dtype=np.float64)
        f_sp = 200.0 / 3
        min_log_hz, min_log_mel, logstep = 1000.0, 1000.0 / f_sp, np.log(6.4) / 27.0
        return np.where(m >= min_log_mel, min_log_hz * np.exp(logstep * (m - min_log_mel)), f_sp * m)

    fftfreqs = np.linspace(0, 8000.0, 201)
    mel_f = mel_to_hz(np.linspace(hz_to_mel(0.0), hz_to_mel(8000.0), n_mels + 2))
    fdiff = np.diff(mel_f)
    ramps = np.subtract.outer(mel_f, fftfreqs)
    weights = np.zeros((n_mels, 201))
    for i in range(n_mels):
        weights[i] = np.maximum(0, np.minimum(-ramps[i] / fdiff[i], ramps[i + 2] / fdiff[i + 1]))
    weights *= (2.0 / (mel_f[2:n_mels + 2] - mel_f[:n_mels]))[:, None]
    return weights.astype(np.float32)


def load_model(name, device=None, backend="openai-whisper", download_root=None, in_memory=False, *,
               synthetic_seed=1234, synthetic_kwargs=None):
    if backend not in ("openai-whisper", "openai"):
        raise ValueError(f"backend '{backend}' is not supported by the B200 drop-in (only 'openai-whisper')")
    if isinstance(name, str) and name.startswith("synthetic:"):
        base = name.split(":", 1)[1]
        if base not in zoo.DIMS:
            raise RuntimeError(f"Model {base} not found; available models = {sorted(zoo.DIMS)}")
        dims = zoo.DIMS[base]
        sd = zoo.synthetic_state_dict(dims, seed=synthetic_seed, **(synthetic_kwargs or {}))
        return WhisperB200(dims, sd, device, name=base, alignment_heads=zoo.ALIGNMENT_HEADS.get(base))
    path = None
    if os.path.isfile(name):
        path = name
    elif name in zoo.DIMS:
        root = download_root or os.path.join(os.path.expanduser("~"), ".cache", "whisper")
        cand = os.path.join(root, name + ".pt")
        if os.path.isfile(cand):
            path = cand
        else:
            raise RuntimeError(
                f"checkpoint for '{name}' not found at {cand} and this environment has no network; "
                f"put the openai-whisper checkpoint there or use load_model('synthetic:{name}')")
    else:
        raise RuntimeError(f"Model {name} not found; available models = {sorted(zoo.DIMS)}")
    ckpt = torch.load(path, map_location="cpu")
    dims = zoo.ModelDimensions(**ckpt["dims"])
    base = os.path.splitext(os.path.basename(path))[0]
    return WhisperB200(dims, ckpt["model_state_dict"], device, name=base,
                       alignment_heads=zoo.ALIGNMENT_HEADS.get(base))
```

Measured before the change: 1208.

## Fuse cross-attention K/V projection with fp16 packing and add 2-CTA paired GEMM kernel

Merges the cross-attention K and V weights into one GEMM and writes the results directly as head-major fp16 K/V, plus f32 alignment-head keys, from the GEMM epilogue. This removes the f32 temporary, the separate pack kernel and one GEMM launch per layer. It also adds a cluster-of-two persistent tcgen05 GEMM kernel using cta_group::2 MMA with 256-wide tiles, keeping the old kernel as a small variant. The risks are added complexity in cluster synchronisation and in tile selection between the two kernels.

```diff
diff --git a/include/wts.h b/include/wts.h
--- a/include/wts.h
+++ b/include/wts.h
@@ -7,7 +7,7 @@
 extern "C" {
 #endif
 
-#define WTS_VERSION 102
+#define WTS_VERSION 103
 #define WTS_SEG_NONPOSITIVE 1
 #define WTS_SEG_PITCH16 2
 
@@ -69,6 +69,8 @@
     int32_t backend;
     int32_t a_is_f32, b_is_f32;
     const int32_t* row_mask;
+    void* kv_k16; void* kv_v16; float* kv_k_align; const int32_t* kv_head_slot;
+    int32_t kv_ctx, kv_n_slots;
 } WtsGemm;
 
 int wts_gemm(const WtsGemm* g, void* stream);
@@ -109,8 +111,6 @@
                           float* d_qk_out, const int32_t* d_head_slot, int32_t n_slots, int32_t qk_rows,
                           const int32_t* d_qk_row, const int32_t* d_row_active, void* stream);
 
-int wts_cross_kv_pack(const float* d_src, void* d_dst16, float* d_dst_align, const int32_t* d_head_slot,
-                      int32_t n_slots, int32_t B, int32_t H, int32_t ctx, void* stream);
 int wts_cross_attention_f16(const float* d_q, int64_t ldq, const void* d_k16, const void* d_v16,
                             const float* d_k_align, const int32_t* d_head_slot, int32_t n_slots, int32_t ctx,
                             const int32_t* d_row_seq, int32_t rows, int32_t H, void* d_out_sb16, int64_t ldo,
diff --git a/whisper-timestamped_b200/csrc/gemm.cu b/whisper-timestamped_b200/csrc/gemm.cu
--- a/whisper-timestamped_b200/csrc/gemm.cu
+++ b/whisper-timestamped_b200/csrc/gemm.cu
@@ -1,4 +1,5 @@
 #include <cuda_bf16.h>
+#include <cuda_fp16.h>
 
 #include "common.cuh"
 
@@ -21,6 +22,17 @@
     if (g.bias) v += g.bias[g.bias_on_m ? m : n];
     if (g.act == 1) v = gelu_erf(v);
     if (g.residual) v += g.residual[(int64_t)zo * g.r_bo + (int64_t)zi * g.r_bi + (int64_t)m * g.ldr + n];
+    if (g.kv_k16) {
+        const int D = g.N >> 1, H = D >> 6;
+        const bool is_v = n >= D;
+        const int c = is_v ? n - D : n, h = c >> 6;
+        const int w = m / g.kv_ctx, pos = m - w * g.kv_ctx;
+        const int64_t off = (((int64_t)w * H + h) * g.kv_ctx + pos) * 64 + (c & 63);
+        reinterpret_cast<__half*>(is_v ? g.kv_v16 : g.kv_k16)[off] = __float2half_rn(v);
+        const int slot = (!is_v && g.kv_k_align) ? g.kv_head_slot[h] : -1;
+        if (slot >= 0) g.kv_k_align[(((int64_t)w * g.kv_n_slots + slot) * g.kv_ctx + pos) * 64 + (c & 63)] = v;
+        return;
+    }
     if (g.out_f32) {
         const int64_t off = g.head_dim > 0 ? (int64_t)(n / g.head_dim) * g.head_stride + (int64_t)m * g.ldc + (n % g.head_dim)
                                            : (int64_t)m * g.ldc + n;
@@ -88,7 +100,13 @@
     if (!gp) { set_error("wts_gemm: null descriptor"); return -2; }
     const WtsGemm g = *gp;
     if (g.M <= 0 || g.N <= 0 || g.batch_outer <= 0 || g.batch_inner <= 0) return 0;
-    if (!g.a || !g.b || (!g.out_f32 && !g.out_sb16)) { set_error("wts_gemm: null operand/output"); return -2; }
+    if (!g.a || !g.b || (!g.out_f32 && !g.out_sb16 && !g.kv_k16)) { set_error("wts_gemm: null operand/output"); return -2; }
+    if (g.kv_k16 && (!g.kv_v16 || g.N % 128 != 0 || g.kv_ctx <= 0 || g.batch_outer * g.batch_inner != 1 ||
+                     (g.kv_k_align && (!g.kv_head_slot || g.kv_n_slots <= 0)))) {
+        set_error("wts_gemm: K/V output needs kv_v16, N = 2 x (multiple of 64), kv_ctx > 0, one problem, and head slots "
+                  "with kv_k_align (N=%d kv_ctx=%d)", g.N, g.kv_ctx);
+        return -2;
+    }
     cudaStream_t st = (cudaStream_t)stream;
     if (g.backend == 0 && !g.a_is_f32 && !g.b_is_f32) return gemm_tc_launch(g, st);
     dim3 grid((g.N + ST - 1) / ST, (g.M + ST - 1) / ST, g.batch_outer * g.batch_inner);
diff --git a/whisper-timestamped_b200/csrc/gemm_tc.cu b/whisper-timestamped_b200/csrc/gemm_tc.cu
--- a/whisper-timestamped_b200/csrc/gemm_tc.cu
+++ b/whisper-timestamped_b200/csrc/gemm_tc.cu
@@ -1,5 +1,6 @@
 #include <cuda.h>
 #include <cuda_bf16.h>
+#include <cuda_fp16.h>
 #include <cudaTypedefs.h>
 
 #include <mutex>
@@ -90,6 +91,12 @@
     return d;
 }
 
+__device__ __forceinline__ void cluster_sync_all()
+{
+    asm volatile("barrier.cluster.arrive.release.aligned;" ::: "memory");
+    asm volatile("barrier.cluster.wait.acquire.aligned;" ::: "memory");
+}
+
 __device__ __forceinline__ float gelu_erf_tc(float v) { return 0.5f * v * (1.0f + erff(v * 0.70710678118654752440f)); }
 
 struct TcArgs {
@@ -97,6 +104,27 @@
     int a_has_bo, a_has_bi, b_has_bo, b_has_bi;
     int debug;
 };
+
+__device__ __forceinline__ void epilogue_kv_chunk(const WtsGemm& g, const float (&y)[32], int m, int nb)
+{
+    const int D = g.N >> 1, H = D >> 6;
+    const bool is_v = nb >= D;
+    const int c = is_v ? nb - D : nb, h = c >> 6;
+    const int w = m / g.kv_ctx, pos = m - w * g.kv_ctx;
+    const int64_t off = (((int64_t)w * H + h) * g.kv_ctx + pos) * 64 + (c & 63);
+    __align__(16) __half hv[32];
+#pragma unroll
+    for (int j = 0; j < 32; ++j) hv[j] = __float2half_rn(y[j]);
+    uint4* dst = reinterpret_cast<uint4*>(reinterpret_cast<__half*>(is_v ? g.kv_v16 : g.kv_k16) + off);
+#pragma unroll
+    for (int j = 0; j < 4; ++j) dst[j] = reinterpret_cast<const uint4*>(hv)[j];
+    const int slot = (!is_v && g.kv_k_align) ? g.kv_head_slot[h] : -1;
+    if (slot >= 0) {
+        float4* da = reinterpret_cast<float4*>(g.kv_k_align + (((int64_t)w * g.kv_n_slots + slot) * g.kv_ctx + pos) * 64 + (c & 63));
+#pragma unroll
+        for (int j = 0; j < 8; ++j) da[j] = make_float4(y[4 * j], y[4 * j + 1], y[4 * j + 2], y[4 * j + 3]);
+    }
+}
 
 __device__ __forceinline__ void epilogue_chunk(const WtsGemm& g, float (&y)[32], int m, int nb, float bias_m, const float* res,
                                                float* of, __nv_bfloat16* ob)
@@ -110,6 +138,7 @@
         if (res && n < g.N) t += res[n];
         y[j] = t;
     }
+    if (g.kv_k16) { epilogue_kv_chunk(g, y, m, nb); return; }
     const bool full = nb + 32 <= g.N;
     if (of) {
         const int64_t off = g.head_dim > 0 ? (int64_t)(nb / g.head_dim) * g.head_stride + (int64_t)m * g.ldc + (nb % g.head_dim)
@@ -261,9 +290,194 @@
 constexpr int P_STAGES = 3;
 constexpr int P_STAGE_BYTES = 4 * TILE_BYTES;
 constexpr int P_SMEM = P_STAGES * P_STAGE_BYTES + 256 + 1024;
+constexpr int P_TILE = 2 * BM;
+constexpr int P_TMEM_COLS = 2 * P_TILE;
+
+__device__ __forceinline__ uint32_t cluster_ctarank()
+{
+    uint32_t r;
+    asm volatile("mov.u32 %0, %%cluster_ctarank;" : "=r"(r));
+    return r;
+}
+__device__ __forceinline__ uint32_t map_to_rank(uint32_t saddr, uint32_t rank)
+{
+    uint32_t d;
+    asm volatile("mapa.shared::cluster.u32 %0, %1, %2;" : "=r"(d) : "r"(saddr), "r"(rank));
+    return d;
+}
+__device__ __forceinline__ void mbar_wait_cluster(uint32_t bar, uint32_t parity)
+{
+    asm volatile(
+        "{\n\t"
+        ".reg .pred p;\n\t"
+        "WAIT_LOOP:\n\t"
+        "mbarrier.try_wait.parity.acquire.cluster.shared::cta.b64 p, [%0], %1;\n\t"
+        "@p bra DONE;\n\t"
+        "bra WAIT_LOOP;\n\t"
+        "DONE:\n\t"
+        "}\n" ::"r"(bar), "r"(parity) : "memory");
+}
+__device__ __forceinline__ void mbar_arrive_cluster(uint32_t cluster_bar)
+{
+    asm volatile("mbarrier.arrive.release.cluster.shared::cluster.b64 _, [%0];" ::"r"(cluster_bar) : "memory");
+}
+__device__ __forceinline__ void tma_load_5d_pair(uint32_t dst, const CUtensorMap* tm, uint32_t cluster_bar, int c0, int c1,
+                                                 int c2, int c3, int c4)
+{
+    asm volatile(
+        "cp.async.bulk.tensor.5d.cta_group::2.shared::cluster.global.mbarrier::complete_tx::bytes [%0], [%1, {%3, %4, %5, %6, %7}], [%2];"
+        ::"r"(dst), "l"(tm), "r"(cluster_bar), "r"(c0), "r"(c1), "r"(c2), "r"(c3), "r"(c4) : "memory");
+}
+__device__ __forceinline__ void umma_bf16_pair(uint32_t tmem_c, uint64_t adesc, uint64_t bdesc, uint32_t idesc, uint32_t accumulate)
+{
+    asm volatile(
+        "{\n\t"
+        ".reg .pred p;\n\t"
+        "setp.ne.b32 p, %4, 0;\n\t"
+        "tcgen05.mma.cta_group::2.kind::f16 [%0], %1, %2, %3, p;\n\t"
+        "}\n" ::"r"(tmem_c), "l"(adesc), "l"(bdesc), "r"(idesc), "r"(accumulate) : "memory");
+}
+__device__ __forceinline__ void umma_commit_pair(uint32_t bar)
+{
+    asm volatile("tcgen05.commit.cta_group::2.mbarrier::arrive::one.shared::cluster.multicast::cluster.b64 [%0], %1;"
+                 ::"r"(bar), "h"((uint16_t)0x3) : "memory");
+}
+
+__global__ void __cluster_dims__(2, 1, 1) __launch_bounds__(P_THREADS, 1)
+gemm_tc_persist_kernel(const __grid_constant__ CUtensorMap tmA, const __grid_constant__ CUtensorMap tmB, const TcArgs args)
+{
+    extern __shared__ unsigned char smem_raw[];
+    const WtsGemm& g = args.g;
+    const uint32_t base = (smem_addr(smem_raw) + 1023u) & ~1023u;
+    const uint32_t bar_base = base + P_STAGES * P_STAGE_BYTES;
+    const int warp = threadIdx.x >> 5, lane = threadIdx.x & 31;
+    const uint32_t rank = cluster_ctarank();
+    const int cluster = blockIdx.x >> 1, n_clusters = gridDim.x >> 1;
+    const int tiles_n = (g.N + P_TILE - 1) / P_TILE, tiles_m = (g.M + P_TILE - 1) / P_TILE;
+    const int n_tiles = tiles_n * tiles_m * g.batch_outer * g.batch_inner;
+    const int nkb = (g.K + BK - 1) / BK;
+
+    if (warp == 0 && lane == 0) {
+        asm volatile("prefetch.tensormap [%0];" ::"l"(&tmA) : "memory");
+        asm volatile("prefetch.tensormap [%0];" ::"l"(&tmB) : "memory");
+    }
+    if (warp == 1) {
+        if (lane == 0) {
+            for (int s = 0; s < P_STAGES; ++s) { mbar_init(bar_base + 8 * s, 1); mbar_init(bar_base + 32 + 8 * s, 1); }
+            for (int b = 0; b < 2; ++b) { mbar_init(bar_base + 64 + 8 * b, 1); mbar_init(bar_base + 80 + 8 * b, 16); }
+            asm volatile("fence.mbarrier_init.release.cluster;" ::: "memory");
+        }
+        __syncwarp();
+        asm volatile("tcgen05.alloc.cta_group::2.sync.aligned.shared::cta.b32 [%0], %1;" ::"r"(bar_base + 96), "r"(P_TMEM_COLS) : "memory");
+        asm volatile("tcgen05.relinquish_alloc_permit.cta_group::2.sync.aligned;" ::: "memory");
+    }
+    tc_fence_before();
+    __syncthreads();
+    cluster_sync_all();
+    tc_fence_after();
+    uint32_t tmem_base;
+    asm volatile("ld.shared.u32 %0, [%1];" : "=r"(tmem_base) : "r"(bar_base + 96));
+
+    if (warp == 0) {
+        if (lane == 0) {
+            const uint32_t full_leader = map_to_rank(bar_base, 0);
+            int it = 0;
+            for (int t = cluster; t < n_tiles; t += n_clusters) {
+                const int nt = t % tiles_n, mt = (t / tiles_n) % tiles_m, z = t / (tiles_n * tiles_m);
+                const int zo = z / g.batch_inner, zi = z - zo * g.batch_inner;
+                const int azo = args.a_has_bo ? zo : 0, azi = args.a_has_bi ? zi : 0;
+                const int bzo = args.b_has_bo ? zo : 0, bzi = args.b_has_bi ? zi : 0;
+                const int m0 = mt * P_TILE + BM * (int)rank, n0 = nt * P_TILE + BM * (int)rank;
+                for (int kb = 0; kb < nkb; ++kb, ++it) {
+                    const int s = it % P_STAGES, u = it / P_STAGES;
+                    mbar_wait(bar_base + 32 + 8 * s, (u & 1) ^ 1);
+                    const uint32_t full = full_leader + 8 * s;
+                    if (rank == 0) mbar_expect_tx(bar_base + 8 * s, 2 * P_STAGE_BYTES);
+                    const uint32_t st = base + s * P_STAGE_BYTES;
+                    const int kc = kb * BK;
+                    tma_load_5d_pair(st, &tmA, full, kc, m0, azi, azo, 0);
+                    tma_load_5d_pair(st + TILE_BYTES, &tmA, full, kc, m0, azi, azo, 1);
+                    tma_load_5d_pair(st + 2 * TILE_BYTES, &tmB, full, kc, n0, bzi, bzo, 0);
+                    tma_load_5d_pair(st + 3 * TILE_BYTES, &tmB, full, kc, n0, bzi, bzo, 1);
+                }
+            }
+            for (int i = 0; i < P_STAGES; ++i, ++it) mbar_wait(bar_base + 32 + 8 * (it % P_STAGES), ((it / P_STAGES) & 1) ^ 1);
+        }
+    } else if (warp == 1) {
+        if (lane == 0 && rank == 0) {
+            const uint32_t idesc = (1u << 4) | (1u << 7) | (1u << 10) | ((uint32_t)(P_TILE >> 3) << 17) | ((uint32_t)(P_TILE >> 4) << 24);
+            int it = 0, lt = 0;
+            for (int t = cluster; t < n_tiles; t += n_clusters, ++lt) {
+                const int buf = lt & 1, ut = lt >> 1;
+                mbar_wait_cluster(bar_base + 80 + 8 * buf, (ut & 1) ^ 1);
+                tc_fence_after();
+                const uint32_t acc = tmem_base + (uint32_t)(buf * P_TILE);
+                for (int kb = 0; kb < nkb; ++kb, ++it) {
+                    const int s = it % P_STAGES, u = it / P_STAGES;
+                    mbar_wait(bar_base + 8 * s, u & 1);
+                    tc_fence_after();
+                    const uint32_t st = base + s * P_STAGE_BYTES;
+                    const uint64_t a_hi = umma_desc(st), a_lo = umma_desc(st + TILE_BYTES);
+                    const uint64_t b_hi = umma_desc(st + 2 * TILE_BYTES), b_lo = umma_desc(st + 3 * TILE_BYTES);
+#pragma unroll
+                    for (int k = 0; k < BK / 16; ++k) {
+                        const uint64_t adv = (uint64_t)(k * 2);
+                        umma_bf16_pair(acc, a_hi + adv, b_hi + adv, idesc, (kb | k) ? 1u : 0u);
+                        umma_bf16_pair(acc, a_lo + adv, b_hi + adv, idesc, 1u);
+                        umma_bf16_pair(acc, a_hi + adv, b_lo + adv, idesc, 1u);
+                    }
+                    umma_commit_pair(bar_base + 32 + 8 * s);
+                }
+                umma_commit_pair(bar_base + 64 + 8 * buf);
+            }
+        }
+    } else {
+        const int q = warp & 3, half = (warp - 2) >> 2;
+        const uint32_t empty_leader = map_to_rank(bar_base + 80, 0);
+        int lt = 0;
+        for (int t = cluster; t < n_tiles; t += n_clusters, ++lt) {
+            const int nt = t % tiles_n, mt = (t / tiles_n) % tiles_m, z = t / (tiles_n * tiles_m);
+            const int zo = z / g.batch_inner, zi = z - zo * g.batch_inner;
+            const int m0 = mt * P_TILE + BM * (int)rank, n0 = nt * P_TILE + BM * half;
+            const int buf = lt & 1, ut = lt >> 1;
+            const int m = m0 + 32 * q + lane;
+            const bool row_ok = m < g.M;
+            const float* res = g.residual ? g.residual + (int64_t)zo * g.r_bo + (int64_t)zi * g.r_bi + (int64_t)m * g.ldr : nullptr;
+            float* of = g.out_f32 ? g.out_f32 + (int64_t)zo * g.c_bo + (int64_t)zi * g.c_bi : nullptr;
+            __nv_bfloat16* ob = g.out_sb16 ? reinterpret_cast<__nv_bfloat16*>(g.out_sb16) + (int64_t)zo * g.o_bo + (int64_t)zi * g.o_bi : nullptr;
+            const float bias_m = (g.bias && g.bias_on_m && row_ok) ? g.bias[m] : 0.f;
+            mbar_wait(bar_base + 64 + 8 * buf, ut & 1);
+            tc_fence_after();
+            const uint32_t taddr = tmem_base + ((uint32_t)(32 * q) << 16) + (uint32_t)(buf * P_TILE + BM * half);
+#pragma unroll 1
+            for (int c = 0; c < BM / 32; ++c) {
+                uint32_t v[32];
+                tmem_ld32(taddr + 32 * c, v);
+                if (c == BM / 32 - 1) {
+                    tc_fence_before();
+                    __syncwarp();
+                    if (lane == 0) mbar_arrive_cluster(empty_leader + 8 * buf);
+                }
+                const int nb = n0 + 32 * c;
+                if (!row_ok || nb >= g.N) continue;
+                float y[32];
+#pragma unroll
+                for (int j = 0; j < 32; ++j) y[j] = g.alpha * __uint_as_float(v[j]);
+                epilogue_chunk(g, y, m, nb, bias_m, res, of, ob);
+            }
+        }
+    }
+    tc_fence_before();
+    __syncthreads();
+    cluster_sync_all();
+    if (warp == 1) {
+        tc_fence_after();
+        asm volatile("tcgen05.dealloc.cta_group::2.sync.aligned.b32 %0, %1;" ::"r"(tmem_base), "r"(P_TMEM_COLS) : "memory");
+    }
+}
 
 __global__ void __launch_bounds__(P_THREADS, 1)
-gemm_tc_persist_kernel(const __grid_constant__ CUtensorMap tmA, const __grid_constant__ CUtensorMap tmB, const TcArgs args)
+gemm_tc_persist_small_kernel(const __grid_constant__ CUtensorMap tmA, const __grid_constant__ CUtensorMap tmB, const TcArgs args)
 {
     extern __shared__ unsigned char smem_raw[];
     const WtsGemm& g = args.g;
@@ -415,12 +629,6 @@
     }
 }
 
-__device__ __forceinline__ void cluster_sync_all()
-{
-    asm volatile("barrier.cluster.arrive.release.aligned;" ::: "memory");
-    asm volatile("barrier.cluster.wait.acquire.aligned;" ::: "memory");
-}
-
 template <int SMAX, int RB>
 __device__ __forceinline__ void sk_reduce_rows(const WtsGemm& g, const uint32_t (&peer)[8], int S, const int* list, int rank,
                                                int n_rows, int n, float bias_n, float* of, __nv_bfloat16* ob)
@@ -660,6 +868,40 @@
     return 0;
 }
 
+static int pair_clusters(int* out, int* n_sm)
+{
+    constexpr int MAX_DEV = 64;
+    static std::mutex mu;
+    static int per_dev[MAX_DEV] = {}, sms[MAX_DEV] = {};
+    int dev = 0;
+    WTS_CUDA_CHECK(cudaGetDevice(&dev));
+    if (dev >= MAX_DEV) { set_error("wts_gemm: device index %d out of range", dev); return -1; }
+    std::lock_guard<std::mutex> lock(mu);
+    if (per_dev[dev] == 0) {
+        WTS_CUDA_CHECK(cudaFuncSetAttribute(gemm_tc_persist_kernel, cudaFuncAttributeMaxDynamicSharedMemorySize, P_SMEM));
+        WTS_CUDA_CHECK(cudaFuncSetAttribute(gemm_tc_persist_small_kernel, cudaFuncAttributeMaxDynamicSharedMemorySize, P_SMEM));
+        WTS_CUDA_CHECK(cudaDeviceGetAttribute(&sms[dev], cudaDevAttrMultiProcessorCount, dev));
+        cudaLaunchConfig_t cfg = {};
+        cfg.gridDim = dim3(2, 1, 1);
+        cfg.blockDim = dim3(P_THREADS, 1, 1);
+        cfg.dynamicSmemBytes = P_SMEM;
+        cudaLaunchAttribute attr;
+        attr.id = cudaLaunchAttributeClusterDimension;
+        attr.val.clusterDim.x = 2;
+        attr.val.clusterDim.y = 1;
+        attr.val.clusterDim.z = 1;
+        cfg.attrs = &attr;
+        cfg.numAttrs = 1;
+        int n = 0;
+        WTS_CUDA_CHECK(cudaOccupancyMaxActiveClusters(&n, gemm_tc_persist_kernel, &cfg));
+        if (n < 1) { set_error("wts_gemm: gemm_tc_persist_kernel cannot be resident on this device"); return -1; }
+        per_dev[dev] = n;
+    }
+    *out = per_dev[dev];
+    *n_sm = sms[dev];
+    return 0;
+}
+
 static int launch_big(const WtsGemm& g, cudaStream_t st)
 {
     constexpr int BN = 128;
@@ -681,18 +923,18 @@
     static const int persist = []{ const char* e = getenv("WTS_GEMM_PERSIST"); return e ? atoi(e) : 1; }();
     const int64_t n_tiles = (int64_t)((g.N + BN - 1) / BN) * ((g.M + BM - 1) / BM) * g.batch_outer * g.batch_inner;
     if (persist && args.debug == 0 && n_tiles > 1) {
-        static bool pattr = false;
-        static int n_sm = 148;
-        if (!pattr) {
-            WTS_CUDA_CHECK(cudaFuncSetAttribute(gemm_tc_persist_kernel, cudaFuncAttributeMaxDynamicSharedMemorySize, P_SMEM));
-            int dev = 0;
-            WTS_CUDA_CHECK(cudaGetDevice(&dev));
-            WTS_CUDA_CHECK(cudaDeviceGetAttribute(&n_sm, cudaDevAttrMultiProcessorCount, dev));
-            pattr = true;
-        }
-        const int64_t rounds = (n_tiles + n_sm - 1) / n_sm;
-        const int ctas = (int)((n_tiles + rounds - 1) / rounds);
-        gemm_tc_persist_kernel<<<ctas, P_THREADS, P_SMEM, st>>>(tmA, tmB, args);
+        int clusters = 0, n_sm = 0;
+        int rc2 = pair_clusters(&clusters, &n_sm);
+        if (rc2) return rc2;
+        if (n_tiles <= n_sm) {
+            gemm_tc_persist_small_kernel<<<(int)n_tiles, P_THREADS, P_SMEM, st>>>(tmA, tmB, args);
+            WTS_LAUNCH_CHECK();
+            return 0;
+        }
+        const int64_t pair_tiles = (int64_t)((g.N + P_TILE - 1) / P_TILE) * ((g.M + P_TILE - 1) / P_TILE) * g.batch_outer * g.batch_inner;
+        const int64_t rounds = (pair_tiles + clusters - 1) / clusters;
+        const int n_cl = (int)((pair_tiles + rounds - 1) / rounds);
+        gemm_tc_persist_kernel<<<2 * n_cl, P_THREADS, P_SMEM, st>>>(tmA, tmB, args);
         WTS_LAUNCH_CHECK();
         return 0;
     }
@@ -744,7 +986,7 @@
 {
     static const int skinny = []{ const char* e = getenv("WTS_SKINNY_GEMM"); return e ? atoi(e) : 1; }();
     static const int splitk = []{ const char* e = getenv("WTS_SPLITK"); return e ? atoi(e) : 1; }();
-    if (skinny && g.M <= BM && g.batch_outer * g.batch_inner == 1 && g.head_dim == 0) {
+    if (skinny && g.M <= BM && g.batch_outer * g.batch_inner == 1 && g.head_dim == 0 && !g.kv_k16) {
         const int tiles = (g.N + BM - 1) / BM, nkb = (g.K + BK - 1) / BK;
         int split = 1;
         if (splitk && tiles <= 74) {
diff --git a/whisper-timestamped_b200/csrc/ops.cu b/whisper-timestamped_b200/csrc/ops.cu
--- a/whisper-timestamped_b200/csrc/ops.cu
+++ b/whisper-timestamped_b200/csrc/ops.cu
@@ -265,23 +265,6 @@
 }
 
 
-__global__ void cross_kv_pack_kernel(const float* __restrict__ src, __half* __restrict__ dst16,
-                                     float* __restrict__ dst_align, const int32_t* __restrict__ head_slot,
-                                     int n_slots, int H, int ctx)
-{
-    const int bh = blockIdx.x;
-    const int b = bh / H, h = bh - b * H;
-    const float* s = src + (int64_t)bh * ctx * 64;
-    __half* d = dst16 + (int64_t)bh * ctx * 64;
-    const int slot = dst_align ? head_slot[h] : -1;
-    float* da = slot >= 0 ? dst_align + ((int64_t)b * n_slots + slot) * ctx * 64 : nullptr;
-    for (int i = threadIdx.x; i < ctx * 64; i += blockDim.x) {
-        const float v = s[i];
-        d[i] = __float2half_rn(v);
-        if (da) da[i] = v;
-    }
-}
-
 __global__ void __launch_bounds__(CA_THREADS)
 cross_attention_f16_kernel(const float* q, int64_t ldq, const __half* k16,
                            const __half* v16, const float* k_align,
@@ -535,16 +518,6 @@
 }
 
 
-extern "C" int wts_cross_kv_pack(const float* d_src, void* d_dst16, float* d_dst_align, const int32_t* d_head_slot,
-                                 int32_t n_slots, int32_t B, int32_t H, int32_t ctx, void* stream)
-{
-    if (B <= 0) return 0;
-    cross_kv_pack_kernel<<<B * H, 256, 0, (cudaStream_t)stream>>>(d_src, (__half*)d_dst16, d_dst_align, d_head_slot,
-                                                                 n_slots, H, ctx);
-    WTS_LAUNCH_CHECK();
-    return 0;
-}
-
 extern "C" int wts_cross_attention_f16(const float* d_q, int64_t ldq, const void* d_k16, const void* d_v16,
                                        const float* d_k_align, const int32_t* d_head_slot, int32_t n_slots,
                                        int32_t ctx, const int32_t* d_row_seq, int32_t rows, int32_t H,
diff --git a/whisper-timestamped_b200/whisper_timestamped/_native.py b/whisper-timestamped_b200/whisper_timestamped/_native.py
--- a/whisper-timestamped_b200/whisper_timestamped/_native.py
+++ b/whisper-timestamped_b200/whisper_timestamped/_native.py
@@ -42,6 +42,8 @@
         ("head_dim", ctypes.c_int32), ("head_stride", ctypes.c_int64),
         ("backend", ctypes.c_int32), ("a_is_f32", ctypes.c_int32), ("b_is_f32", ctypes.c_int32),
         ("row_mask", ctypes.c_void_p),
+        ("kv_k16", ctypes.c_void_p), ("kv_v16", ctypes.c_void_p), ("kv_k_align", ctypes.c_void_p), ("kv_head_slot", ctypes.c_void_p),
+        ("kv_ctx", ctypes.c_int32), ("kv_n_slots", ctypes.c_int32),
     ]
 
 
@@ -107,7 +109,6 @@
     lib.wts_gather_rows.argtypes = [vp, i64, vp, i32, i32, vp, vp]
     lib.wts_decoder_attention.argtypes = [i32, vp, i64, vp, vp, i64, i32, vp, vp, i32, i32, vp, i64, i64, vp, vp, i32,
                                           i32, vp, vp, vp]
-    lib.wts_cross_kv_pack.argtypes = [vp, vp, vp, vp, i32, i32, i32, i32, vp]
     lib.wts_cross_attention_f16.argtypes = [vp, i64, vp, vp, vp, vp, i32, i32, vp, i32, i32, vp, i64, i64, vp, i32, vp, vp, vp]
     lib.wts_enc_attention.argtypes = [vp, i64, i64, vp, i64, i64, i32, i32, i32, i32, vp, i64, i64, vp]
     lib.wts_enc_attention.restype = ctypes.c_int
@@ -124,7 +125,7 @@
     lib.wts_logprob_gather.argtypes = [vp, i64, i32, vp, vp, vp, i32, vp]
     for name in ("wts_to_sb16", "wts_layernorm", "wts_softmax_rows", "wts_frames", "wts_power", "wts_logmel_max",
                  "wts_logmel_finish", "wts_window_gather", "wts_embed", "wts_gather_rows", "wts_decoder_attention",
-                 "wts_kv_append", "wts_decode_select", "wts_step_inputs", "wts_softmax_pick", "wts_logprob_gather", "wts_cross_kv_pack",
+                 "wts_kv_append", "wts_decode_select", "wts_step_inputs", "wts_softmax_pick", "wts_logprob_gather",
                  "wts_cross_attention_f16"):
         getattr(lib, name).restype = ctypes.c_int
     return lib
@@ -137,7 +138,7 @@
     "wts_attn_prep_batch", "wts_dtw_batch", "wts_dtw_batch_sized", "wts_disfluency_starts", "wts_gemm", "wts_to_sb16", "wts_layernorm", "wts_softmax_rows",
     "wts_frames", "wts_power", "wts_logmel_max", "wts_logmel_finish", "wts_window_gather", "wts_embed",
     "wts_gather_rows", "wts_decoder_attention", "wts_kv_append", "wts_decode_select", "wts_filtered_logprobs", "wts_decode_steps", "wts_decode_step_kernels", "wts_step_inputs",
-    "wts_softmax_pick", "wts_logprob_gather", "wts_cross_kv_pack", "wts_cross_attention_f16", "wts_enc_attention",
+    "wts_softmax_pick", "wts_logprob_gather", "wts_cross_attention_f16", "wts_enc_attention",
 ]
 
 
diff --git a/whisper-timestamped_b200/whisper_timestamped/engine.py b/whisper-timestamped_b200/whisper_timestamped/engine.py
--- a/whisper-timestamped_b200/whisper_timestamped/engine.py
+++ b/whisper-timestamped_b200/whisper_timestamped/engine.py
@@ -80,7 +80,7 @@
              batch=(1, 1), a_b=(0, 0), b_b=(0, 0), alpha=1.0, bias=None, bias_on_m=False, act=0,
              residual=None, ldr=0, r_b=(0, 0), out_f32=None, ldc=0, c_b=(0, 0), c_off=0,
              out_sb=None, ldo=0, o_plane=0, o_b=(0, 0), o_off=0, head_dim=0, head_stride=0,
-             a_f32=False, b_f32=False, backend=None, row_mask=None):
+             a_f32=False, b_f32=False, backend=None, row_mask=None, kv=None):
         g = nat.Gemm()
         if a_f32:
             g.a, g.lda, g.a_plane = a.data_ptr() + 4 * a_off, lda, 0
@@ -111,6 +111,10 @@
         g.backend = self.backend if backend is None else backend
         g.a_is_f32, g.b_is_f32 = int(a_f32), int(b_f32)
         g.row_mask = row_mask.data_ptr() if row_mask is not None else None
+        if kv is not None:
+            k16, v16, k_align, head_slot, g.kv_ctx = kv
+            g.kv_k16, g.kv_v16 = k16.data_ptr(), v16.data_ptr()
+            g.kv_k_align, g.kv_head_slot, g.kv_n_slots = k_align.data_ptr(), head_slot.data_ptr(), k_align.shape[1]
         if a_f32 or b_f32:
             g.backend = 1
         nat.check(nat.lib.wts_gemm(ctypes.byref(g), self._st()), "wts_gemm")
@@ -269,23 +273,13 @@
             sv=[torch.zeros((B, H, d.n_text_ctx, 64), **f32) for _ in range(L)],
             ck=[torch.empty((B, H, N_CTX_AUDIO, 64), dtype=torch.float16, device=dev) for _ in range(L)],
             cv=[torch.empty((B, H, N_CTX_AUDIO, 64), dtype=torch.float16, device=dev) for _ in range(L)],
-            ckal=[torch.empty((B, max(1, len(self.m.heads)), N_CTX_AUDIO, 64), **f32) for _ in range(L)],
-            kvtmp=torch.empty((B, H, N_CTX_AUDIO, 64), **f32))
+            ckal=[torch.empty((B, max(1, len(self.m.heads)), N_CTX_AUDIO, 64), **f32) for _ in range(L)])
 
     def _cross_kv(self, xa, st8, B):
-        d = self.dims
-        D, H = d.n_text_state, d.n_text_head
+        D = self.dims.n_text_state
         for li, blk in enumerate(self.w.dec):
-            c = blk.cross
-            tmp = st8["kvtmp"]
-            n_slots = len(self.m.heads)
-            for (wt, bias, dst, al) in ((c.k, None, st8["ck"][li], st8["ckal"][li]), (c.v, c.v_b, st8["cv"][li], None)):
-                self.gemm(xa, wt, 1500, D, D, batch=(B, 1), a_b=(1500 * D, 0), bias=bias, out_f32=tmp, ldc=64,
-                          c_b=(H * 1500 * 64, 0), head_dim=64, head_stride=1500 * 64)
-                nat.check(nat.lib.wts_cross_kv_pack(tmp.data_ptr(), dst.data_ptr(), al.data_ptr() if al is not None else None,
-                                                    self.w.head_slot[li].data_ptr(), n_slots, B, H, N_CTX_AUDIO, self._st()),
-                          "wts_cross_kv_pack")
-                self.launches += 1
+            self.gemm(xa, blk.cross.kv, B * N_CTX_AUDIO, 2 * D, D, bias=blk.cross.kv_b,
+                      kv=(st8["ck"][li], st8["cv"][li], st8["ckal"][li], self.w.head_slot[li], N_CTX_AUDIO))
 
     def _final_logits(self, x_rows, n_rows, logits):
         d, w = self.dims, self.w
@@ -785,8 +779,7 @@
         return dict(
             ck=[torch.empty((B, H, N_CTX_AUDIO, 64), dtype=torch.float16, device=dev) for _ in range(L)],
             cv=[torch.empty((B, H, N_CTX_AUDIO, 64), dtype=torch.float16, device=dev) for _ in range(L)],
-            ckal=[torch.empty((B, max(1, len(self.m.heads)), N_CTX_AUDIO, 64), dtype=torch.float32, device=dev) for _ in range(L)],
-            kvtmp=torch.empty((B, H, N_CTX_AUDIO, 64), dtype=torch.float32, device=dev))
+            ckal=[torch.empty((B, max(1, len(self.m.heads)), N_CTX_AUDIO, 64), dtype=torch.float32, device=dev) for _ in range(L)])
 
     @torch.no_grad()
     def _decode_strategy(self, job, setup):
diff --git a/whisper-timestamped_b200/whisper_timestamped/model.py b/whisper-timestamped_b200/whisper_timestamped/model.py
--- a/whisper-timestamped_b200/whisper_timestamped/model.py
+++ b/whisper-timestamped_b200/whisper_timestamped/model.py
@@ -100,8 +100,8 @@
             out_w = g(prefix + ".out.weight")
             if cross:
                 b.q, b.q_b = lin(q), qb
-                b.k = lin(k)
-                b.v, b.v_b = lin(v), vb
+                b.kv = lin(torch.cat([k, v], 0))
+                b.kv_b = torch.cat([zeros, vb]).contiguous()
                 b.q_f32 = q.contiguous()
             else:
                 qkv = torch.cat([q, k, v], 0).contiguous()
```

Result: faster. 1263, median of 6 (+4.5%).
